# phcavelar/graph-odenet

Measured on AMD Instinct MI355X. Metric: full-graph ODE-GCN forward+backward steps/sec at 64 RK4 evals, higher is better.
Workload: dtype f32; 1 GPU; RMAT scale-20 / 10000000 edges (+self loops, dedup) row-normalised, d=128, ODEGCN3 rk4(3/8) 16 steps = 64 f-evals fwd, adjoint bwd, Adam; one graph per GPU; nodes=1048576, nnz=10758918, nfeat=128, hidden=128, nclass=16, parallelism=dp1 (one graph per rank, 1 gradient all-reduce/step)

## Files before the change

### graph_odenet_amd/csrc/api.hip

```cpp
#include "common.h"

extern "C" int gode_abi_version(void) { return GODE_ABI_VERSION; }

extern "C" const char* gode_error_string(int code) {
    switch (code) {
        case 0: return "success";
        case GODE_E_NULLPTR: return "graphode: required pointer is NULL";
        case GODE_E_SHAPE: return "graphode: invalid shape / leading dimension";
        case GODE_E_ALIGN: return "graphode: operand not 16-byte aligned";
        case GODE_E_RANGE: return "graphode: argument out of range";
        case GODE_E_UNSUPPORTED: return "graphode: unsupported configuration";
        default: break;
    }
    if (code > 0) return hipGetErrorString((hipError_t)code);
    return "graphode: unknown error";
}

#include "options.h"
#include <cstdlib>
#include <cstring>

namespace {
int env_int(const char* name, int dflt) { const char* e = getenv(name); return e ? atoi(e) : dflt; }
int g_gemm_split = -1, g_overlap = -1, g_wgrad_split = -1, g_wgrad_split_small = 0, g_bwd_pc = -1, g_fwd_pc = -1, g_small_fused = -1, g_bwd_wgrad = -1, g_y2_colsum = -1, g_rk_close_once = -1, g_spmm_pipe = -1;
}

int gode_opt_gemm_split() { if (g_gemm_split < 0) { const int v = env_int("GODE_GEMM_SPLIT", 2); g_gemm_split = (v == 1 || v == 2) ? v : 0; } return g_gemm_split; }
int gode_opt_wgrad_split() {
    if (g_wgrad_split < 0) { const int v = env_int("GODE_WGRAD_SPLIT", 8); g_wgrad_split = (v == 6 || v == 8) ? v : 0; }
    return g_wgrad_split;
}
int gode_opt_wgrad_split_small() { return g_wgrad_split_small; }
int gode_opt_bwd_pc() { if (g_bwd_pc < 0) g_bwd_pc = env_int("GODE_BWD_PC", 1) != 0; return g_bwd_pc; }
int gode_opt_fwd_pc() { if (g_fwd_pc < 0) g_fwd_pc = env_int("GODE_FWD_PC", 3) & 3; return g_fwd_pc; }
int gode_opt_small_fused() { if (g_small_fused < 0) g_small_fused = env_int("GODE_SMALL_FUSED", 1) != 0; return g_small_fused; }
int gode_opt_bwd_wgrad() { if (g_bwd_wgrad < 0) g_bwd_wgrad = env_int("GODE_BWD_WGRAD", 1) != 0; return g_bwd_wgrad; }
int gode_opt_y2_colsum() { if (g_y2_colsum < 0) g_y2_colsum = env_int("GODE_Y2_COLSUM", 1) != 0; return g_y2_colsum; }
int gode_opt_rk_close_once() { if (g_rk_close_once < 0) g_rk_close_once = env_int("GODE_RK_CLOSE_ONCE", 1) != 0; return g_rk_close_once; }
int gode_opt_spmm_pipe() { if (g_spmm_pipe < 0) { const int v = env_int("GODE_SPMM_PIPE", 1); g_spmm_pipe = (v < 0 || v > 64) ? 1 : v; } return g_spmm_pipe; }
int gode_opt_overlap() { if (g_overlap < 0) g_overlap = env_int("GODE_OVERLAP", 1) != 0; return g_overlap; }

extern "C" int gode_set_option(const char* name, int value) {
    if (!name) return GODE_E_NULLPTR;
    if (!strcmp(name, "gemm_split")) { if (value < 0 || value > 2) return GODE_E_UNSUPPORTED; g_gemm_split = value; return 0; }
    if (!strcmp(name, "overlap")) { g_overlap = value != 0; return 0; }
    if (!strcmp(name, "wgrad_split_small")) { g_wgrad_split_small = value != 0; return 0; }
    if (!strcmp(name, "bwd_pc")) { g_bwd_pc = value != 0; return 0; }
    if (!strcmp(name, "small_fused")) { g_small_fused = value != 0; return 0; }
    if (!strcmp(name, "bwd_wgrad")) { g_bwd_wgrad = value != 0; return 0; }
    if (!strcmp(name, "y2_colsum")) { g_y2_colsum = value != 0; return 0; }
    if (!strcmp(name, "rk_close_once")) { g_rk_close_once = value != 0; return 0; }
    if (!strcmp(name, "spmm_pipe")) { if (value < 0 || value > 64) return GODE_E_UNSUPPORTED; g_spmm_pipe = value; return 0; }
    if (!strcmp(name, "fwd_pc")) { if (value < 0 || value > 3) return GODE_E_UNSUPPORTED; g_fwd_pc = value; return 0; }
    if (!strcmp(name, "wgrad_split")) { if (value != 0 && value != 6 && value != 8) return GODE_E_UNSUPPORTED; g_wgrad_split = value; return 0; }
    return GODE_E_UNSUPPORTED;
}
extern "C" int gode_get_option(const char* name) {
    if (!name) return GODE_E_NULLPTR;
    if (!strcmp(name, "gemm_split")) return gode_opt_gemm_split();
    if (!strcmp(name, "overlap")) return gode_opt_overlap();
    if (!strcmp(name, "wgrad_split")) return gode_opt_wgrad_split();
    if (!strcmp(name, "wgrad_split_small")) return gode_opt_wgrad_split_small();
    if (!strcmp(name, "bwd_pc")) return gode_opt_bwd_pc();
    if (!strcmp(name, "small_fused")) return gode_opt_small_fused();
    if (!strcmp(name, "bwd_wgrad")) return gode_opt_bwd_wgrad();
    if (!strcmp(name, "y2_colsum")) return gode_opt_y2_colsum();
    if (!strcmp(name, "rk_close_once")) return gode_opt_rk_close_once();
    if (!strcmp(name, "spmm_pipe")) return gode_opt_spmm_pipe();
    if (!strcmp(name, "fwd_pc")) return gode_opt_fwd_pc();
    return GODE_E_UNSUPPORTED;
}
```

### graph_odenet_amd/csrc/dense_pc.h

```cpp
#pragma once
#include "common.h"

int gode_pc_fwd_launch(const LinComb& lc, int64_t n_rows, float eps, const float* gamma, const float* beta,
                       const float* W, int has_time, float t, float* S, float* xout, const float* aux_coef, float* aux,
                       int cg, hipStream_t s);
int gode_pc_bwd_launch(const LinComb& lc, int64_t n_rows, float eps, const float* gamma, const float* W, int has_time,
                       const float* dS, float out_scale, const LinComb& pre, float* dx, float* dgamma_part,
                       float* dbeta_part, int64_t n_part, int cg, hipStream_t s);
int64_t gode_pc_bwd_wgrad_parts(int64_t n_rows);
int gode_pc_bwd_wgrad_launch(const LinComb& lc, int64_t n_rows, float eps, const float* gamma, const float* beta, const float* W,
                             int has_time, const float* dS, float out_scale, const LinComb& pre, float* dx,
                             float* dgamma_part, float* dbeta_part, int64_t n_part, float* dW_part, int cg, hipStream_t s);
```

### graph_odenet_amd/csrc/gemm.hip

```cpp
#include <map>
#include <mutex>
#include <utility>
#include "common.h"
#include "dense_common.h"
#include "dense_pc.h"
#include "options.h"
#include "prof.h"

namespace {

constexpr int kMaxBlocks = 512;
constexpr int64_t kWgradSplitMinRows = 65536;

template <int D, int NTHREADS, bool TRANSPOSE>
__device__ __forceinline__ void fill_w_lds(float* Wl, const float* __restrict__ W, int has_time) {
    constexpr int LDW = D + 4;
    constexpr int N4 = D * D / 4;
    constexpr int IT = (N4 + NTHREADS - 1) / NTHREADS;
    float4 v[IT];
#pragma unroll
    for (int it = 0; it < IT; ++it) {
        const int idx = threadIdx.x + it * NTHREADS;
        v[it] = make_float4(0.f, 0.f, 0.f, 0.f);
        if (idx < N4) v[it] = ld4(W + (int64_t)has_time * D + (int64_t)idx * 4);
// ... 1127 lines not shown
                const float c3 = -c2 * m - bsum * rs * sc;
                dx[(int64_t)row * d_in + c] = out_scale * (rs * (gamma ? gamma[c] : 1.f) * dy[idx] + c2 * xs[idx] + c3) +
                                              (pre.n > 0 ? lc_load1(pre, (int64_t)row * d_in + c) : 0.f);
            }
            if (dgamma_part) {
                const bool first = blk == (int)blockIdx.x;
                for (int c = threadIdx.x; c < d_in; c += 256) {
                    const int gi = c / cg;
                    float sg = 0.f, sb = 0.f;
                    for (int rr = 0; rr < RB; ++rr) {
                        if (blk * RB + rr >= n_rows) break;
                        const float m = stat[(rr * groups + gi) * 2], rs = stat[(rr * groups + gi) * 2 + 1];
                        sg += dy[rr * d_in + c] * (xs[rr * d_in + c] - m) * rs;
                        sb += dy[rr * d_in + c];
                    }
                    float* pg = dgamma_part + (int64_t)blockIdx.x * d_in + c;
                    float* pb = dbeta_part + (int64_t)blockIdx.x * d_in + c;
                    *pg = first ? sg : *pg + sg;
                    *pb = first ? sb : *pb + sb;
                }
            }
        } else {
            for (int idx = threadIdx.x; idx < RB * d_in; idx += 256) {
                const int rr = idx / d_in, c = idx % d_in;
                const int row = blk * RB + rr;
                if (row < n_rows) dx[(int64_t)row * d_in + c] = out_scale * dy[idx] + (pre.n > 0 ? lc_load1(pre, (int64_t)row * d_in + c) : 0.f);
            }
        }
    }
    if (dgamma_part && groups > 0) {
        const int owned = n_blk < (int)gridDim.x ? n_blk : (int)gridDim.x;
        for (int p = owned + blockIdx.x; p < n_part; p += gridDim.x)
            for (int c = threadIdx.x; c < d_in; c += 256) { dgamma_part[(int64_t)p * d_in + c] = 0.f; dbeta_part[(int64_t)p * d_in + c] = 0.f; }
    }
}

__global__ __launch_bounds__(256) void wgrad_generic(LinComb xin, int n_rows, int d_in, int groups, float eps,
                                                     const float* gamma, const float* beta, const float* dS,
                                                     int d_out, int has_time, float* dW_part)
{
    extern __shared__ __attribute__((aligned(16))) float smem[];
    float* xs = smem;
    float* stat = smem + RB * d_in;
    const int n_blk = (n_rows + RB - 1) / RB;
    const int K = d_in + has_time;
    float* out = dW_part + (int64_t)blockIdx.x * K * d_out;
    for (int idx = threadIdx.x; idx < K * d_out; idx += 256) out[idx] = 0.f;
    for (int blk = blockIdx.x; blk < n_blk; blk += gridDim.x) {
        __syncthreads();
        stage_rows_gn(xs, stat, xin, blk * RB, n_rows, d_in, groups, eps, gamma, beta, true);
        const int nr = (n_rows - blk * RB) < RB ? (n_rows - blk * RB) : RB;
        for (int idx = threadIdx.x; idx < K * d_out; idx += 256) {
            const int i = idx / d_out, n = idx % d_out;
            float acc = 0.f;
            for (int rr = 0; rr < nr; ++rr) {
                const float a = (has_time && i == 0) ? 1.0f : xs[rr * d_in + (i - has_time)];
                acc = fmaf(a, dS[(int64_t)(blk * RB + rr) * d_out + n], acc);
            }
            out[idx] += acc;
        }
    }
}

template <typename K>
int set_lds(K kernel, size_t bytes) { return gode_set_lds_once(reinterpret_cast<const void*>(kernel), bytes); }

int fast_cg(int64_t d_in, int64_t d_out, int32_t groups) {
    if (d_in != d_out) return -1;
    if (d_in != 16 && d_in != 32 && d_in != 64 && d_in != 128) return -1;
    if (groups == 0) return 0;
    if (d_in % groups) return -1;
    const int64_t cg = d_in / groups;
    if (cg == 1 || cg == 2 || cg == 4) return (int)cg;
    return -1;
}

int narrow_cg(int64_t d_in, int64_t d_out, int32_t groups) {
    if (d_out != 2) return -1;
    if (d_in != 16 && d_in != 32 && d_in != 64 && d_in != 128) return -1;
    if (groups == 0) return 0;
    if (d_in % groups) return -1;
    const int64_t cg = d_in / groups;
    return (cg == 1 || cg == 2 || cg == 4) ? (int)cg : -1;
}

int64_t fwd_blocks(int64_t n_rows) {
    int64_t b = ((n_rows + 15) / 16 + 3) / 4;
    if (b < 1) b = 1;
    if (b > kMaxBlocks) b = kMaxBlocks;
    return b;
}
int64_t wgrad_blocks(int64_t n_rows) {
    int64_t b = (n_rows + 31) / 32;
    if (b < 1) b = 1;
    if (b > kMaxBlocks) b = kMaxBlocks;
    return b;
}

}

int gode_set_lds_once(const void* fn, size_t bytes) {
    if (bytes <= 64 * 1024) return 0;
    static std::mutex mu;
    static std::map<std::pair<int, const void*>, size_t> done;
    int dev = 0;
    hipError_t e = hipGetDevice(&dev);
    if (e != hipSuccess) return (int)e;
    std::lock_guard<std::mutex> lk(mu);
    auto key = std::make_pair(dev, fn);
    auto it = done.find(key);
    if (it != done.end() && it->second >= bytes) return 0;
    e = hipFuncSetAttribute(fn, hipFuncAttributeMaxDynamicSharedMemorySize, (int)bytes);
    if (e != hipSuccess) return (int)e;
    done[key] = bytes;
    return 0;
}

#define GODE_DISPATCH_NJ_CG(NJV, CGV, MACRO)                                        \
    if (nj == NJV && cg == CGV) { MACRO(NJV, CGV) }

#define GODE_DISPATCH_ALL(MACRO)                                                    \
    GODE_DISPATCH_NJ_CG(1, 0, MACRO) GODE_DISPATCH_NJ_CG(1, 1, MACRO)               \
    GODE_DISPATCH_NJ_CG(2, 0, MACRO) GODE_DISPATCH_NJ_CG(2, 1, MACRO)               \
    GODE_DISPATCH_NJ_CG(4, 0, MACRO) GODE_DISPATCH_NJ_CG(4, 2, MACRO)               \
    GODE_DISPATCH_NJ_CG(8, 0, MACRO) GODE_DISPATCH_NJ_CG(8, 4, MACRO)               \
    GODE_DISPATCH_NJ_CG(1, 2, MACRO) GODE_DISPATCH_NJ_CG(1, 4, MACRO)               \
    GODE_DISPATCH_NJ_CG(2, 2, MACRO) GODE_DISPATCH_NJ_CG(2, 4, MACRO)               \
    GODE_DISPATCH_NJ_CG(4, 1, MACRO) GODE_DISPATCH_NJ_CG(4, 4, MACRO)               \
    GODE_DISPATCH_NJ_CG(8, 1, MACRO) GODE_DISPATCH_NJ_CG(8, 2, MACRO)

static int check_common(const gode_lincomb_t* xin, int64_t n_rows, int64_t d_in, int32_t groups, int64_t d_out) {
    if (n_rows < 0 || d_in <= 0 || d_out <= 0 || groups < 0) return GODE_E_SHAPE;
    if (groups > 0 && d_in % groups) return GODE_E_SHAPE;
    if (n_rows > INT32_MAX || d_in > 2048 || d_out > 65536) return GODE_E_RANGE;
    return check_lincomb(xin, true);
}

extern "C" int gode_gn_time_gemm_f32(const gode_lincomb_t* xin, int64_t n_rows, int64_t d_in, int32_t groups,
                                     float eps, const float* gamma, const float* beta, const float* W,
                                     int64_t d_out, int has_time, float t, float* S, void* stream)
{
    return gode_gn_time_gemm_xout_f32(xin, n_rows, d_in, groups, eps, gamma, beta, W, d_out, has_time, t, S, nullptr,
                                      stream);
}

extern "C" int gode_gn_time_gemm_xout_f32(const gode_lincomb_t* xin, int64_t n_rows, int64_t d_in, int32_t groups,
                                          float eps, const float* gamma, const float* beta, const float* W,
                                          int64_t d_out, int has_time, float t, float* S, float* x_out, void* stream)
{
    return gode_gn_time_gemm_xout_aux_f32(xin, n_rows, d_in, groups, eps, gamma, beta, W, d_out, has_time, t, S, x_out,
                                          nullptr, nullptr, stream);
}

extern "C" int gode_gn_time_gemm_xout_aux_f32(const gode_lincomb_t* xin, int64_t n_rows, int64_t d_in, int32_t groups,
                                              float eps, const float* gamma, const float* beta, const float* W,
                                              int64_t d_out, int has_time, float t, float* S, float* x_out,
                                              const float* aux_coef, float* aux_out, void* stream)
{
    int rc = check_common(xin, n_rows, d_in, groups, d_out); if (rc) return rc;
    if (aux_out && !aux_coef) return GODE_E_NULLPTR;
    if (n_rows == 0) return 0;
    if (!W || !S) return GODE_E_NULLPTR;
    if (x_out && (((uintptr_t)x_out) & 15)) return GODE_E_ALIGN;
    if (aux_out && (((uintptr_t)aux_out) & 15)) return GODE_E_ALIGN;
    if (aux_out) {
        if (aux_out == S || aux_out == x_out) return GODE_E_RANGE;
        for (int j = 0; j < xin->n; ++j) if (aux_out == xin->ptr[j]) return GODE_E_RANGE;
    }
    has_time = has_time ? 1 : 0;
    hipStream_t s = (hipStream_t)stream;
    LinComb lc = make_lincomb(xin);
    AuxCoef ac;
    for (int j = 0; j < GODE_MAX_TERMS; ++j) ac.c[j] = (aux_out && j < lc.n) ? aux_coef[j] : 0.f;
    const int cg = fast_cg(d_in, d_out, groups);
    const bool al = lincomb_aligned16(xin) && !(((uintptr_t)S) & 15) && !(((uintptr_t)W) & 15) &&
                    (!gamma || !(((uintptr_t)gamma) & 15)) && (!beta || !(((uintptr_t)beta) & 15));
    if (aux_out && !(cg >= 0 && al && d_in == 128)) return GODE_E_UNSUPPORTED;
    if (cg >= 0 && al && d_in == 128 && (n_rows >= kWgradSplitMinRows || gode_opt_wgrad_split_small()) &&
        ((lc.n <= 2 && !x_out) ? (gode_opt_fwd_pc() & 1) : (gode_opt_fwd_pc() & 2))) {
        rc = gode_pc_fwd_launch(lc, n_rows, eps, gamma, beta, W, has_time, t, S, x_out, aux_coef, aux_out, cg, s);
        if (rc != GODE_E_UNSUPPORTED) return rc;
        if (aux_out && (cg == 0 || cg == 1 || cg == 2 || cg == 4)) return GODE_E_UNSUPPORTED;
    }
    if (cg >= 0 && al && d_in == 128 && !x_out && (gode_opt_gemm_split() == 1 || (gode_opt_gemm_split() == 2 && lc.n <= 2 && n_rows >= 65536))) {
        if (aux_out) return GODE_E_UNSUPPORTED;
        const size_t lds = (size_t)3 * 128 * (128 + 8) * sizeof(unsigned short) + 3 * 128 * sizeof(float);
        int64_t blocks = ((n_rows + 15) / 16 + 7) / 8; if (blocks < 1) blocks = 1; if (blocks > 256) blocks = 256;
#define GODE_FWDS2(CGV, NXV) { rc = set_lds(gn_gemm_fwd_split_kernel<CGV, NXV>, lds); if (rc) return rc;    \
          const int slot = gode_prof_begin(s, d_in, n_rows, (int64_t)lc.n - 1, GODE_PROF_GEMM_FWD | GODE_PROF_FORM_SPLIT); \
          hipLaunchKernelGGL((gn_gemm_fwd_split_kernel<CGV, NXV>), dim3((unsigned)blocks), dim3(512), lds, s, \
                             lc, (int)n_rows, eps, gamma, beta, W, has_time, t, S);                           \
          gode_prof_end(s, slot);                                                                             \
          GODE_LAUNCH_CHECK(); return 0; }
#define GODE_FWDS(CGV) { if (lc.n == 1) GODE_FWDS2(CGV, 1) else if (lc.n == 2) GODE_FWDS2(CGV, 2) else GODE_FWDS2(CGV, 0) }
        if (cg == 0) GODE_FWDS(0) else if (cg == 1) GODE_FWDS(1) else if (cg == 2) GODE_FWDS(2) else GODE_FWDS(4)
#undef GODE_FWDS
#undef GODE_FWDS2
    }
    if (cg >= 0 && al) {
        const int nj = (int)(d_in / 16);
        const size_t lds = ((size_t)d_in * (d_in + 4) + 3 * d_in) * sizeof(float);
        const int64_t blocks = fwd_blocks(n_rows);
#define GODE_FWD(NJV, CGV)                                                                          \
        { rc = set_lds(gn_gemm_fwd_kernel<NJV, CGV>, lds); if (rc) return rc;                       \
          const int slot = gode_prof_begin(s, d_in, n_rows, (int64_t)lc.n - 1 + (x_out ? 1 : 0), GODE_PROF_GEMM_FWD); \
          hipLaunchKernelGGL((gn_gemm_fwd_kernel<NJV, CGV>), dim3((unsigned)blocks), dim3(256), lds, s, \
                             lc, (int)n_rows, eps, gamma, beta, W, has_time, t, S, x_out,           \
                             (const float*)nullptr, (float*)nullptr, ac, (float*)nullptr);          \
          gode_prof_end(s, slot);                                                                   \
          GODE_LAUNCH_CHECK(); return 0; }
#define GODE_FWDA(NJV, CGV)                                                                         \
        { rc = set_lds(gn_gemm_fwd_kernel<NJV, CGV, true>, lds); if (rc) return rc;                 \
          const int slot = gode_prof_begin(s, d_in, n_rows, (int64_t)lc.n - 1 + (x_out ? 1 : 0) + 1, GODE_PROF_GEMM_FWD); \
          hipLaunchKernelGGL((gn_gemm_fwd_kernel<NJV, CGV, true>), dim3((unsigned)blocks), dim3(256), lds, s, \
                             lc, (int)n_rows, eps, gamma, beta, W, has_time, t, S, x_out,           \
                             (const float*)nullptr, (float*)nullptr, ac, aux_out);                  \
          gode_prof_end(s, slot);                                                                   \
          GODE_LAUNCH_CHECK(); return 0; }
        if (aux_out) {
            GODE_DISPATCH_NJ_CG(8, 0, GODE_FWDA) GODE_DISPATCH_NJ_CG(8, 1, GODE_FWDA)
            GODE_DISPATCH_NJ_CG(8, 2, GODE_FWDA) GODE_DISPATCH_NJ_CG(8, 4, GODE_FWDA)
            return GODE_E_UNSUPPORTED;
        }
        GODE_DISPATCH_ALL(GODE_FWD)
#undef GODE_FWDA
#undef GODE_FWD
    }
    {
        const int cg = narrow_cg(d_in, d_out, groups);
        if (cg >= 0 && al) {
            const int nj = (int)(d_in / 16);
            const int64_t blocks = fwd_blocks(n_rows);
#define GODE_NFWD(NJV, CGV)                                                                                 \
            { hipLaunchKernelGGL((gn_narrow_fwd_kernel<NJV, CGV, 2>), dim3((unsigned)blocks), dim3(256), 0, s, \
                                 lc, (int)n_rows, eps, gamma, beta, W, has_time, t, S, x_out);              \
              GODE_LAUNCH_CHECK(); return 0; }
            GODE_DISPATCH_ALL(GODE_NFWD)
#undef GODE_NFWD
        }
    }
    if (x_out) { rc = gode_lincomb_f32(x_out, xin, n_rows * d_in, stream); if (rc) return rc; }
    const size_t lds = ((size_t)RB * d_in + (size_t)RB * (groups > 0 ? groups : 1) * 2) * sizeof(float);
    rc = set_lds(gn_gemm_fwd_generic, lds); if (rc) return rc;
    int64_t blocks = (n_rows + RB - 1) / RB; if (blocks > 2048) blocks = 2048;
    hipLaunchKernelGGL(gn_gemm_fwd_generic, dim3((unsigned)blocks), dim3(256), lds, s, lc, (int)n_rows, (int)d_in,
                       (int)groups, eps, gamma, beta, W, (int)d_out, has_time, t, S);
    GODE_LAUNCH_CHECK();
    return 0;
}

extern "C" int gode_gn_time_gemm_pair_f32(const gode_lincomb_t* xin, int64_t n_rows, int64_t d, int32_t groups, float eps,
                                          const float* gamma, const float* beta, const float* Wa, const float* Wb,
                                          int has_time, float t, float* Sa, float* Sb, float* x_out, void* stream)
{
    int rc = check_common(xin, n_rows, d, groups, d); if (rc) return rc;
    if (n_rows == 0) return 0;
    if (!Wa || !Wb || !Sa || !Sb) return GODE_E_NULLPTR;
    has_time = has_time ? 1 : 0;
    hipStream_t s = (hipStream_t)stream;
    LinComb lc = make_lincomb(xin);
    const int cg = fast_cg(d, d, groups);
    const bool al = lincomb_aligned16(xin) && !((((uintptr_t)Sa) | ((uintptr_t)Sb) | ((uintptr_t)Wa) | ((uintptr_t)Wb)) & 15) &&
                    (!gamma || !(((uintptr_t)gamma) & 15)) && (!beta || !(((uintptr_t)beta) & 15)) &&
                    (!x_out || !(((uintptr_t)x_out) & 15));
    if (cg >= 0 && al) {
        const int nj = (int)(d / 16);
        const size_t lds = ((size_t)d * (d + 4) + 3 * d) * sizeof(float);
        const int64_t blocks = fwd_blocks(n_rows);
#define GODE_FWDP(NJV, CGV)                                                                         \
        { rc = set_lds(gn_gemm_fwd_kernel<NJV, CGV>, lds); if (rc) return rc;                       \
          hipLaunchKernelGGL((gn_gemm_fwd_kernel<NJV, CGV>), dim3((unsigned)blocks, 2), dim3(256), lds, s, \
                             lc, (int)n_rows, eps, gamma, beta, Wa, has_time, t, Sa, x_out, Wb, Sb, AuxCoef(), (float*)nullptr);  \
          GODE_LAUNCH_CHECK(); return 0; }
        GODE_DISPATCH_ALL(GODE_FWDP)
#undef GODE_FWDP
    }
    rc = gode_gn_time_gemm_xout_f32(xin, n_rows, d, groups, eps, gamma, beta, Wa, d, has_time, t, Sa, x_out, stream);
    if (rc) return rc;
    return gode_gn_time_gemm_f32(xin, n_rows, d, groups, eps, gamma, beta, Wb, d, has_time, t, Sb, stream);
}

extern "C" int64_t gode_gemm_bwd_parts(int64_t n_rows) {
    int64_t a = fwd_blocks(n_rows);
    int64_t b = (n_rows + RB - 1) / RB; if (b > 2048) b = 2048; if (b < 1) b = 1;
    return a > b ? a : b;
}

extern "C" int gode_gn_time_gemm_bwd_f32(const gode_lincomb_t* xin, int64_t n_rows, int64_t d_in, int32_t groups,
                                         float eps, const float* gamma, const float* W, int64_t d_out,
                                         int has_time, const float* dS, float out_scale,
                                         const gode_lincomb_t* pre, float* dx,
                                         float* dgamma_part, float* dbeta_part, void* stream)
{
    int rc = check_common(xin, n_rows, d_in, groups, d_out); if (rc) return rc;
    if (n_rows == 0) return 0;
    if (!W || !dS || !dx) return GODE_E_NULLPTR;
    if ((dgamma_part == nullptr) != (dbeta_part == nullptr)) return GODE_E_NULLPTR;
    if (pre && pre->n > 0) { rc = check_lincomb(pre, true); if (rc) return rc; } else pre = nullptr;
    has_time = has_time ? 1 : 0;
    hipStream_t s = (hipStream_t)stream;
    LinComb lc = make_lincomb(xin);
    LinComb lpre = make_lincomb(pre);
    const int64_t n_part = gode_gemm_bwd_parts(n_rows);
    const int cg = fast_cg(d_in, d_out, groups);
    const bool al = lincomb_aligned16(xin) && lincomb_aligned16(pre) && !(((uintptr_t)dS) & 15) && !(((uintptr_t)dx) & 15) &&
                    (!gamma || !(((uintptr_t)gamma) & 15)) &&
// ... 192 lines not shown
```

### graph_odenet_amd/csrc/gemm_pc.hip

```cpp
#include "common.h"
#include "dense_common.h"
#include "dense_pc.h"
#include "prof.h"

namespace {

constexpr int D = 128;
constexpr int LDK = D + 8;
constexpr int LDX = D + 4;
constexpr int kBlocks = 256;
template <int R> struct Img { static constexpr int PIECE_B = R * LDK * 2, BUF_B = 3 * PIECE_B; };

__device__ __forceinline__ bf16x8 pack8(const unsigned (&u)[8]) {
    const uint2 a = pack_hi16x4(u[0], u[1], u[2], u[3]), b = pack_hi16x4(u[4], u[5], u[6], u[7]);
    typedef unsigned u32x4 __attribute__((ext_vector_type(4)));
    const u32x4 v = {a.x, a.y, b.x, b.y};
    return __builtin_bit_cast(bf16x8, v);
}

template <typename F>
__device__ __forceinline__ void load_weight_pieces(bf16x8 (&A)[4][3], F element) {
    const int l = threadIdx.x & 63, m = l & 15, g = l >> 4;
#pragma unroll
    for (int kb = 0; kb < 4; ++kb) {
        unsigned h[8], md[8], lo[8];
#pragma unroll
        for (int e = 0; e < 8; ++e) split3_trunc(element(m, 32 * kb + 8 * g + e), h[e], md[e], lo[e]);
        A[kb][0] = pack8(h); A[kb][1] = pack8(md); A[kb][2] = pack8(lo);
    }
}

template <int R>
__device__ __forceinline__ void tile_product(const char* img , const bf16x8 (&A)[4][3], f32x4 (&acc)[R / 16]) {
    constexpr int PIECE_B = Img<R>::PIECE_B, NS = (R / 16) * 4;
    bf16x8 b[2][3];
#pragma unroll
    for (int pc = 0; pc < 3; ++pc) b[0][pc] = *reinterpret_cast<const bf16x8*>(img + pc * PIECE_B);
#pragma unroll
    for (int s = 0; s < NS; ++s) {
        const int rt = s >> 2, kb = s & 3;
        if (s + 1 < NS) {
            const int rt2 = (s + 1) >> 2, kb2 = (s + 1) & 3;
#pragma unroll
            for (int pc = 0; pc < 3; ++pc)
                b[(s + 1) & 1][pc] = *reinterpret_cast<const bf16x8*>(img + pc * PIECE_B + rt2 * 16 * LDK * 2 + kb2 * 64);
        }
        const bf16x8 bh = b[s & 1][0], bm = b[s & 1][1], bl = b[s & 1][2];
        f32x4 c = acc[rt];
        c = __builtin_amdgcn_mfma_f32_16x16x32_bf16(A[kb][2], bm, c, 0, 0, 0);
        c = __builtin_amdgcn_mfma_f32_16x16x32_bf16(A[kb][1], bl, c, 0, 0, 0);
        c = __builtin_amdgcn_mfma_f32_16x16x32_bf16(A[kb][2], bh, c, 0, 0, 0);
        c = __builtin_amdgcn_mfma_f32_16x16x32_bf16(A[kb][0], bl, c, 0, 0, 0);
        c = __builtin_amdgcn_mfma_f32_16x16x32_bf16(A[kb][1], bm, c, 0, 0, 0);
        c = __builtin_amdgcn_mfma_f32_16x16x32_bf16(A[kb][1], bh, c, 0, 0, 0);
        c = __builtin_amdgcn_mfma_f32_16x16x32_bf16(A[kb][0], bm, c, 0, 0, 0);
        c = __builtin_amdgcn_mfma_f32_16x16x32_bf16(A[kb][0], bh, c, 0, 0, 0);
        acc[rt] = c;
        __builtin_amdgcn_sched_barrier(0);
    }
}

template <int PIECE_B>
__device__ __forceinline__ void stage_row4(char* dst , const float4 v) {
    unsigned h0, m0, l0, h1, m1, l1, h2, m2, l2, h3, m3, l3;
    split3_trunc(v.x, h0, m0, l0); split3_trunc(v.y, h1, m1, l1); split3_trunc(v.z, h2, m2, l2); split3_trunc(v.w, h3, m3, l3);
    *reinterpret_cast<uint2*>(dst) = pack_hi16x4(h0, h1, h2, h3);
    *reinterpret_cast<uint2*>(dst + PIECE_B) = pack_hi16x4(m0, m1, m2, m3);
    *reinterpret_cast<uint2*>(dst + 2 * PIECE_B) = pack_hi16x4(l0, l1, l2, l3);
}

struct TileWalk {
    int n_tiles, stride, mine;
    __device__ TileWalk(int n_rows, int R) {
        n_tiles = (n_rows + R - 1) / R;
        stride = gridDim.x;
        mine = (int)blockIdx.x < n_tiles ? (n_tiles - 1 - (int)blockIdx.x) / stride + 1 : 0;
    }
    __device__ int tile(int k) const { return blockIdx.x + k * stride; }
    __device__ int clamped(int k) const { return blockIdx.x + (k < mine ? k : (mine > 0 ? mine - 1 : 0)) * stride; }
};

template <int CG, int NX, bool XOUT, int R, bool AUX = false>
__global__ __launch_bounds__(1024, 1) void gn_gemm_fwd_pc_kernel(LinComb xin, int n_rows, float eps,
                                                                const float* __restrict__ gamma,
                                                                const float* __restrict__ beta,
                                                                const float* __restrict__ W, int has_time, float t,
                                                                float* __restrict__ S, float* __restrict__ xout,
                                                                AuxCoef acoef, float* __restrict__ aux)
{
    static_assert(!AUX || NX > 0, "the second combination needs the raw terms");
    constexpr int PIECE_B = Img<R>::PIECE_B, BUF_B = Img<R>::BUF_B;
    constexpr int RPT = R / 8;
    extern __shared__ __attribute__((aligned(16))) float smem[];
    char* lds = reinterpret_cast<char*>(smem);
    const TileWalk tw(n_rows, R);
    if (threadIdx.x >= 512) {
        const int grp = (threadIdx.x - 512) >> 8, pt = (threadIdx.x - 512) & 255;
        const int trow = pt >> 5, tcol = 4 * (pt & 31);
        const float4 gmv = gamma ? ld4(gamma + tcol) : make_float4(1.f, 1.f, 1.f, 1.f);
        const float4 btv = beta ? ld4(beta + tcol) : make_float4(0.f, 0.f, 0.f, 0.f);
        constexpr int NXR = NX > 0 ? NX : 1;
        float4 xr[NXR][RPT];
        auto prefetch = [&](int k) {
            const int tile = tw.clamped(k);
#pragma unroll
            for (int p = 0; p < RPT; ++p) {
                const int row = tile * R + RPT * trow + p;
                const int64_t off = (int64_t)(row < n_rows ? row : n_rows - 1) * D + tcol;
                if (NX > 0) {
#pragma unroll
                    for (int j = 0; j < NXR; ++j) xr[j][p] = ld4(xin.ptr[j] + off);
                } else {
                    xr[0][p] = lc_load4(xin, off);
                }
            }
        };
        auto stage = [&](int k) {
            char* img = lds + (k & 1) * BUF_B + (RPT * trow) * LDK * 2 + tcol * 2;
            const int tile = tw.tile(k);
#pragma unroll
            for (int p = 0; p < RPT; ++p) {
                const int row = tile * R + RPT * trow + p;
                float4 x = xr[0][p];
                if (NX > 0) {
                    x = make_float4(0.f, 0.f, 0.f, 0.f);
#pragma unroll
                    for (int j = 0; j < NXR; ++j) {
                        const float c = xin.coef[j];
                        x.x = fmaf(c, xr[j][p].x, x.x); x.y = fmaf(c, xr[j][p].y, x.y);
                        x.z = fmaf(c, xr[j][p].z, x.z); x.w = fmaf(c, xr[j][p].w, x.w);
                    }
                }
                if (XOUT && row < n_rows) *reinterpret_cast<float4*>(xout + (int64_t)row * D + tcol) = x;
                if (AUX) {
                    float4 a = make_float4(0.f, 0.f, 0.f, 0.f);
#pragma unroll
                    for (int j = 0; j < NXR; ++j) {
                        const float c = acoef.c[j];
                        a.x = fmaf(c, xr[j][p].x, a.x); a.y = fmaf(c, xr[j][p].y, a.y);
                        a.z = fmaf(c, xr[j][p].z, a.z); a.w = fmaf(c, xr[j][p].w, a.w);
                    }
                    if (row < n_rows) *reinterpret_cast<float4*>(aux + (int64_t)row * D + tcol) = a;
                }
                float4 xn = gn_forward_v<CG>(x, eps, gmv, btv);
                if (row >= n_rows) xn = make_float4(0.f, 0.f, 0.f, 0.f);
                stage_row4<PIECE_B>(img + p * LDK * 2, xn);
            }
        };
        prefetch(grp);
        if (grp == 0 && tw.mine > 0) { stage(0); prefetch(2); }
        lds_barrier();
        for (int k = 0; k < tw.mine; ++k) {
            if (((k + 1) & 1) == grp && k + 1 < tw.mine) { stage(k + 1); prefetch(k + 3); }
            lds_barrier();
        }
        return;
    }
    const int wave = threadIdx.x >> 6, l = threadIdx.x & 63, r = l & 15, g = l >> 4;
    const int n0 = 16 * wave;
    bf16x8 A[4][3];
    load_weight_pieces(A, [&](int m, int k) { return W[(int64_t)(k + has_time) * D + n0 + m]; });
    f32x4 t0 = {0.f, 0.f, 0.f, 0.f};
    if (has_time) { const float4 w0 = ld4(W + n0 + 4 * g); t0 = (f32x4){t * w0.x, t * w0.y, t * w0.z, t * w0.w}; }
    const int rd_off = r * LDK * 2 + g * 16;
    lds_barrier();
    for (int k = 0; k < tw.mine; ++k) {
        f32x4 acc[R / 16];
#pragma unroll
        for (int rt = 0; rt < R / 16; ++rt) acc[rt] = t0;
        tile_product<R>(lds + (k & 1) * BUF_B + rd_off, A, acc);
        const int row0 = tw.tile(k) * R + r;
#pragma unroll
        for (int rt = 0; rt < R / 16; ++rt) {
            const int row = row0 + 16 * rt;
            if (row < n_rows)
                *reinterpret_cast<float4*>(S + (int64_t)row * D + n0 + 4 * g) = make_float4(acc[rt][0], acc[rt][1], acc[rt][2], acc[rt][3]);
        }
        lds_barrier();
    }
}

template <int CG, int NX, bool XLDS>
__global__ __launch_bounds__(1024, 1) void gn_gemm_bwd_pc_kernel(LinComb xin, int n_rows, float eps,
                                                                const float* __restrict__ gamma,
                                                                const float* __restrict__ W, int has_time,
                                                                const float* __restrict__ dS, float out_scale,
                                                                LinComb pre, float* __restrict__ dx,
                                                                float* __restrict__ dgamma_part,
                                                                float* __restrict__ dbeta_part, int n_part)
{
    constexpr int R = 32, PIECE_B = Img<R>::PIECE_B;
    constexpr int XT_B = (CG != 0 && XLDS) ? R * LDX * 4 : 0;
    constexpr int BUF_B = Img<R>::BUF_B + XT_B;
    extern __shared__ __attribute__((aligned(16))) float smem[];
    char* lds = reinterpret_cast<char*>(smem);
    const TileWalk tw(n_rows, R);
    if (threadIdx.x >= 512) {
        const int grp = (threadIdx.x - 512) >> 8, pt = (threadIdx.x - 512) & 255;
        const int trow = pt >> 5, tcol = 4 * (pt & 31);
        constexpr int NXR = NX > 0 ? NX : 1;
        float4 gr[4], xr[NXR][4];
        auto prefetch = [&](int k) {
            const int tile = tw.clamped(k);
#pragma unroll
            for (int p = 0; p < 4; ++p) {
                const int row = tile * R + 4 * trow + p;
                const int64_t off = (int64_t)(row < n_rows ? row : n_rows - 1) * D + tcol;
                gr[p] = ld4(dS + off);
                if (CG != 0 && XLDS) {
                    if (NX > 0) {
#pragma unroll
                        for (int j = 0; j < NXR; ++j) xr[j][p] = ld4(xin.ptr[j] + off);
                    } else {
                        xr[0][p] = lc_load4(xin, off);
                    }
                }
            }
        };
        auto stage = [&](int k) {
            char* buf = lds + (k & 1) * BUF_B;
            char* img = buf + (4 * trow) * LDK * 2 + tcol * 2;
            const int tile = tw.tile(k);
#pragma unroll
            for (int p = 0; p < 4; ++p) {
                float4 v = gr[p];
                if (tile * R + 4 * trow + p >= n_rows) v = make_float4(0.f, 0.f, 0.f, 0.f);
                stage_row4<PIECE_B>(img + p * LDK * 2, v);
                if (CG != 0 && XLDS) {
                    float4 x = xr[0][p];
                    if (NX > 0) {
                        x = make_float4(0.f, 0.f, 0.f, 0.f);
#pragma unroll
                        for (int j = 0; j < NXR; ++j) {
                            const float c = xin.coef[j];
                            x.x = fmaf(c, xr[j][p].x, x.x); x.y = fmaf(c, xr[j][p].y, x.y);
                            x.z = fmaf(c, xr[j][p].z, x.z); x.w = fmaf(c, xr[j][p].w, x.w);
                        }
                    }
                    *reinterpret_cast<float4*>(buf + Img<R>::BUF_B + ((4 * trow + p) * LDX + tcol) * 4) = x;
                }
            }
        };
        prefetch(grp);
        if (grp == 0 && tw.mine > 0) { stage(0); prefetch(2); }
        lds_barrier();
        for (int k = 0; k < tw.mine; ++k) {
            if (((k + 1) & 1) == grp && k + 1 < tw.mine) { stage(k + 1); prefetch(k + 3); }
            lds_barrier();
        }
        if (CG != 0 && dgamma_part)
            for (int p = gridDim.x + blockIdx.x; p < n_part; p += gridDim.x)
                for (int c = threadIdx.x - 512; c < D; c += 512) { dgamma_part[(int64_t)p * D + c] = 0.f; dbeta_part[(int64_t)p * D + c] = 0.f; }
        return;
    }
    const int wave = threadIdx.x >> 6, l = threadIdx.x & 63, r = l & 15, g = l >> 4;
    const int i0 = 16 * wave, c0 = i0 + 4 * g;
    bf16x8 A[4][3];
    load_weight_pieces(A, [&](int m, int k) { return W[(int64_t)(i0 + m + has_time) * D + k]; });
    const float4 gm = (CG != 0 && gamma) ? ld4(gamma + c0) : make_float4(1.f, 1.f, 1.f, 1.f);
    float4 dgs = make_float4(0.f, 0.f, 0.f, 0.f), dbs = make_float4(0.f, 0.f, 0.f, 0.f);
    const int rd_off = r * LDK * 2 + g * 16;
    const int xt_off = Img<R>::BUF_B + (r * LDX + c0) * 4;
    lds_barrier();
    for (int k = 0; k < tw.mine; ++k) {
        const char* buf = lds + (k & 1) * BUF_B;
        const int row0 = tw.tile(k) * R + r;
        constexpr int NXC = NX > 0 ? NX : 1;
        float4 xd[2][NXC];
        if (CG != 0 && !XLDS) {
#pragma unroll
            for (int rt = 0; rt < 2; ++rt) {
                const int row = row0 + 16 * rt;
                const int64_t off = (int64_t)(row < n_rows ? row : n_rows - 1) * D + c0;
                if (NX > 0) {
#pragma unroll
                    for (int j = 0; j < NXC; ++j) xd[rt][j] = ld4(xin.ptr[j] + off);
                } else {
                    xd[rt][0] = lc_load4(xin, off);
                }
            }
        }
        f32x4 acc[2] = {{0.f, 0.f, 0.f, 0.f}, {0.f, 0.f, 0.f, 0.f}};
        tile_product<R>(buf + rd_off, A, acc);
#pragma unroll
        for (int rt = 0; rt < 2; ++rt) {
            const int row = row0 + 16 * rt;
            const bool valid = row < n_rows;
            const float4 dy = make_float4(acc[rt][0], acc[rt][1], acc[rt][2], acc[rt][3]);
            float4 out = dy;
            if (CG != 0) {
                float4 x;
                if (XLDS) {
                    x = *reinterpret_cast<const float4*>(buf + xt_off + rt * 16 * LDX * 4);
                } else {
                    x = xd[rt][0];
                    if (NX > 0) {
                        x = make_float4(0.f, 0.f, 0.f, 0.f);
#pragma unroll
                        for (int j = 0; j < NXC; ++j) {
                            const float c = xin.coef[j];
                            x.x = fmaf(c, xd[rt][j].x, x.x); x.y = fmaf(c, xd[rt][j].y, x.y);
                            x.z = fmaf(c, xd[rt][j].z, x.z); x.w = fmaf(c, xd[rt][j].w, x.w);
                        }
                    }
                }
                float4 mean, rstd;
                gn_stats<CG>(x, eps, mean, rstd);
                const float4 xh = make_float4((x.x - mean.x) * rstd.x, (x.y - mean.y) * rstd.y,
                                              (x.z - mean.z) * rstd.z, (x.w - mean.w) * rstd.w);
                const float4 dh = make_float4(dy.x * gm.x, dy.y * gm.y, dy.z * gm.z, dy.w * gm.w);
                if (valid) {
                    dgs.x += dy.x * xh.x; dgs.y += dy.y * xh.y; dgs.z += dy.z * xh.z; dgs.w += dy.w * xh.w;
                    dbs.x += dy.x; dbs.y += dy.y; dbs.z += dy.z; dbs.w += dy.w;
                }
                const float m1 = ((dh.x + dh.y) + (dh.z + dh.w)) * 0.25f;
                const float m2 = ((dh.x * xh.x + dh.y * xh.y) + (dh.z * xh.z + dh.w * xh.w)) * 0.25f;
                const float rs = rstd.x;
                out = make_float4(rs * (dh.x - m1 - xh.x * m2), rs * (dh.y - m1 - xh.y * m2),
                                  rs * (dh.z - m1 - xh.z * m2), rs * (dh.w - m1 - xh.w * m2));
            }
            if (valid) {
                float4 o = make_float4(out_scale * out.x, out_scale * out.y, out_scale * out.z, out_scale * out.w);
                if (pre.n > 0) {
                    const float4 pv = lc_load4(pre, (int64_t)row * D + c0);
                    o.x += pv.x; o.y += pv.y; o.z += pv.z; o.w += pv.w;
                }
                *reinterpret_cast<float4*>(dx + (int64_t)row * D + c0) = o;
            }
        }
// ... 100 lines not shown
            stage(qb, k + 1);
            prefetch(qb, k + 3);
            lds_barrier();
            if (++k >= tw.mine) break;
            stage(qa, k + 1);
            prefetch(qa, k + 3);
            lds_barrier();
            ++k;
        }
        if (has_time) {
            float* red = smem;
            *reinterpret_cast<float4*>(red + trow * D + tcol) = csum;
        }
        __syncthreads();
        if (has_time && pt < D) {
            float sacc = 0.f;
            for (int p = 0; p < 8; ++p) sacc += smem[p * D + pt];
            out[pt] = sacc;
        }
        if (CG != 0 && dgamma_part)
            for (int p = gridDim.x + blockIdx.x; p < n_part; p += gridDim.x)
                for (int c = pt; c < D; c += 256) { dgamma_part[(int64_t)p * D + c] = 0.f; dbeta_part[(int64_t)p * D + c] = 0.f; }
        return;
    }
    const int wave = threadIdx.x >> 6, l = threadIdx.x & 63, r = l & 15, g = l >> 4;
    const int i0 = 16 * wave, c0 = i0 + 4 * g;
    bf16x8 A[4][3];
    load_weight_pieces(A, [&](int m, int k) { return W[(int64_t)(i0 + m + has_time) * D + k]; });
    const float4 gm = (CG != 0 && gamma) ? ld4(gamma + c0) : make_float4(1.f, 1.f, 1.f, 1.f);
    float4 dgs = make_float4(0.f, 0.f, 0.f, 0.f), dbs = make_float4(0.f, 0.f, 0.f, 0.f);
    const int rd_off = r * LDK * 2 + g * 16;
    const int xt_off = 2 * IMG_B + (r * LDX + c0) * 4;
    const int a0 = 4 * (wave >> 2), b0 = 2 * (wave & 3);
    const int tr_off = (8 * g + (r >> 2)) * LDK * 2 + 4 * (r & 3) * 2;
    f32x4 wacc[4][2];
#pragma unroll
    for (int a = 0; a < 4; ++a)
#pragma unroll
        for (int b = 0; b < 2; ++b) wacc[a][b] = (f32x4){0.f, 0.f, 0.f, 0.f};
    lds_barrier();
    for (int k = 0; k < tw.mine; ++k) {
        const char* buf = lds + (k & 1) * BUF_B;
        const int row0 = tw.tile(k) * R + r;
        f32x4 acc[2] = {{0.f, 0.f, 0.f, 0.f}, {0.f, 0.f, 0.f, 0.f}};
        tile_product<R>(buf + rd_off, A, acc);
#pragma unroll
        for (int rt = 0; rt < 2; ++rt) {
            const int row = row0 + 16 * rt;
            const bool valid = row < n_rows;
            const float4 dy = make_float4(acc[rt][0], acc[rt][1], acc[rt][2], acc[rt][3]);
            float4 o4 = dy;
            if (CG != 0) {
                const float4 x = *reinterpret_cast<const float4*>(buf + xt_off + rt * 16 * LDX * 4);
                float4 mean, rstd;
                gn_stats<CG>(x, eps, mean, rstd);
                const float4 xh = make_float4((x.x - mean.x) * rstd.x, (x.y - mean.y) * rstd.y,
                                              (x.z - mean.z) * rstd.z, (x.w - mean.w) * rstd.w);
                const float4 dh = make_float4(dy.x * gm.x, dy.y * gm.y, dy.z * gm.z, dy.w * gm.w);
                if (valid) {
                    dgs.x += dy.x * xh.x; dgs.y += dy.y * xh.y; dgs.z += dy.z * xh.z; dgs.w += dy.w * xh.w;
                    dbs.x += dy.x; dbs.y += dy.y; dbs.z += dy.z; dbs.w += dy.w;
                }
                const float m1 = ((dh.x + dh.y) + (dh.z + dh.w)) * 0.25f;
                const float m2 = ((dh.x * xh.x + dh.y * xh.y) + (dh.z * xh.z + dh.w * xh.w)) * 0.25f;
                const float rs = rstd.x;
                o4 = make_float4(rs * (dh.x - m1 - xh.x * m2), rs * (dh.y - m1 - xh.y * m2),
                                 rs * (dh.z - m1 - xh.z * m2), rs * (dh.w - m1 - xh.w * m2));
            }
            if (valid) {
                float4 o = make_float4(out_scale * o4.x, out_scale * o4.y, out_scale * o4.z, out_scale * o4.w);
                if (pre.n > 0) {
                    const float4 pv = lc_load4(pre, (int64_t)row * D + c0);
                    o.x += pv.x; o.y += pv.y; o.z += pv.z; o.w += pv.w;
                }
                *reinterpret_cast<float4*>(dx + (int64_t)row * D + c0) = o;
            }
        }
        const char* Gp = buf + tr_off;
        const char* Xp = buf + IMG_B + tr_off;
        bf16x8 Bf[2][3];
#pragma unroll
        for (int b = 0; b < 2; ++b)
#pragma unroll
            for (int pc = 0; pc < 3; ++pc) Bf[b][pc] = tr_frag(Gp + pc * PIECE_B, 16 * (b0 + b) * 2);
#pragma unroll
        for (int a = 0; a < 4; ++a) {
            bf16x8 Af[3];
#pragma unroll
            for (int pc = 0; pc < 3; ++pc) Af[pc] = tr_frag(Xp + pc * PIECE_B, 16 * (a0 + a) * 2);
#pragma unroll
            for (int b = 0; b < 2; ++b) {
                f32x4 c = wacc[a][b];
                c = __builtin_amdgcn_mfma_f32_16x16x32_bf16(Af[2], Bf[b][1], c, 0, 0, 0);
                c = __builtin_amdgcn_mfma_f32_16x16x32_bf16(Af[1], Bf[b][2], c, 0, 0, 0);
                c = __builtin_amdgcn_mfma_f32_16x16x32_bf16(Af[2], Bf[b][0], c, 0, 0, 0);
                c = __builtin_amdgcn_mfma_f32_16x16x32_bf16(Af[0], Bf[b][2], c, 0, 0, 0);
                c = __builtin_amdgcn_mfma_f32_16x16x32_bf16(Af[1], Bf[b][1], c, 0, 0, 0);
                c = __builtin_amdgcn_mfma_f32_16x16x32_bf16(Af[1], Bf[b][0], c, 0, 0, 0);
                c = __builtin_amdgcn_mfma_f32_16x16x32_bf16(Af[0], Bf[b][1], c, 0, 0, 0);
                c = __builtin_amdgcn_mfma_f32_16x16x32_bf16(Af[0], Bf[b][0], c, 0, 0, 0);
                wacc[a][b] = c;
            }
        }
        lds_barrier();
    }
#pragma unroll
    for (int a = 0; a < 4; ++a)
#pragma unroll
        for (int b = 0; b < 2; ++b)
#pragma unroll
            for (int q = 0; q < 4; ++q) {
                const int i = 16 * (a0 + a) + 4 * g + q;
                out[(int64_t)(i + has_time) * D + 16 * (b0 + b) + r] = wacc[a][b][q];
            }
    if (CG != 0 && dgamma_part) {
#pragma unroll
        for (int o = 1; o < 16; o <<= 1) {
            dgs.x += __shfl_xor(dgs.x, o, 64); dgs.y += __shfl_xor(dgs.y, o, 64); dgs.z += __shfl_xor(dgs.z, o, 64); dgs.w += __shfl_xor(dgs.w, o, 64);
            dbs.x += __shfl_xor(dbs.x, o, 64); dbs.y += __shfl_xor(dbs.y, o, 64); dbs.z += __shfl_xor(dbs.z, o, 64); dbs.w += __shfl_xor(dbs.w, o, 64);
        }
        if (r == 0) {
            *reinterpret_cast<float4*>(dgamma_part + (int64_t)blockIdx.x * D + c0) = dgs;
            *reinterpret_cast<float4*>(dbeta_part + (int64_t)blockIdx.x * D + c0) = dbs;
        }
    }
    __syncthreads();
}

int64_t pc_blocks(int64_t n_rows, int R) {
    int64_t b = (n_rows + R - 1) / R;
    if (b < 1) b = 1;
    if (b > kBlocks) b = kBlocks;
    return b;
}

template <typename K>
int set_lds_pc(K kernel, size_t bytes) { return gode_set_lds_once(reinterpret_cast<const void*>(kernel), bytes); }

}

int gode_pc_fwd_launch(const LinComb& lc, int64_t n_rows, float eps, const float* gamma, const float* beta,
                       const float* W, int has_time, float t, float* S, float* xout, const float* aux_coef, float* aux,
                       int cg, hipStream_t s)
{
    int rc = 0;
    AuxCoef ac;
    for (int j = 0; j < GODE_MAX_TERMS; ++j) ac.c[j] = (aux && j < lc.n) ? aux_coef[j] : 0.f;
#define GODE_FPC5(CGV, NXV, XO, RV, AX)                                                                           \
    { const size_t lds = 2 * (size_t)Img<RV>::BUF_B;                                                               \
      const int64_t blocks = pc_blocks(n_rows, RV);                                                                \
      rc = set_lds_pc(gn_gemm_fwd_pc_kernel<CGV, NXV, XO, RV, AX>, lds); if (rc) return rc;                        \
      const int slot = gode_prof_begin(s, D, n_rows, (int64_t)lc.n - 1 + (XO ? 1 : 0) + (AX ? 1 : 0), GODE_PROF_GEMM_FWD | GODE_PROF_FORM_PC); \
      hipLaunchKernelGGL((gn_gemm_fwd_pc_kernel<CGV, NXV, XO, RV, AX>), dim3((unsigned)blocks), dim3(1024), lds, s, \
                         lc, (int)n_rows, eps, gamma, beta, W, has_time, t, S, xout, ac, aux);                    \
      gode_prof_end(s, slot);                                                                                      \
      GODE_LAUNCH_CHECK(); return 0; }
#define GODE_FPC2(CGV, NXV, RV) { if (xout) GODE_FPC5(CGV, NXV, true, RV, false) else GODE_FPC5(CGV, NXV, false, RV, false) }
#define GODE_FPC(CGV) { switch (lc.n) { case 1: GODE_FPC2(CGV, 1, 32) case 2: GODE_FPC2(CGV, 2, 32) case 3: GODE_FPC2(CGV, 3, 32) \
                                        case 4: GODE_FPC2(CGV, 4, 32) default: GODE_FPC2(CGV, 0, 32) } }
#define GODE_FPCA(CGV) { if (xout) GODE_FPC5(CGV, 4, true, 32, true) else GODE_FPC5(CGV, 4, false, 32, true) }
    if (aux) {
        if (lc.n != 4) return GODE_E_UNSUPPORTED;
        if (cg == 0) GODE_FPCA(0) else if (cg == 1) GODE_FPCA(1) else if (cg == 2) GODE_FPCA(2) else if (cg == 4) GODE_FPCA(4)
        return GODE_E_UNSUPPORTED;
    }
    if (cg == 0) GODE_FPC(0) else if (cg == 1) GODE_FPC(1) else if (cg == 2) GODE_FPC(2) else if (cg == 4) GODE_FPC(4)
#undef GODE_FPCA
#undef GODE_FPC
#undef GODE_FPC2
#undef GODE_FPC5
    return GODE_E_UNSUPPORTED;
}

int gode_pc_bwd_launch(const LinComb& lc, int64_t n_rows, float eps, const float* gamma, const float* W, int has_time,
                       const float* dS, float out_scale, const LinComb& pre, float* dx, float* dgamma_part,
                       float* dbeta_part, int64_t n_part, int cg, hipStream_t s)
{
    const int64_t blocks = pc_blocks(n_rows, 32);
    int rc = 0;
#define GODE_BPC3(CGV, NXV, XL)                                                                                   \
    { const size_t lds = 2 * ((size_t)Img<32>::BUF_B + ((CGV != 0 && XL) ? 32 * LDX * 4 : 0));                     \
      rc = set_lds_pc(gn_gemm_bwd_pc_kernel<CGV, NXV, XL>, lds); if (rc) return rc;                                \
      const int slot = gode_prof_begin(s, D, n_rows, (int64_t)lc.n - 1 + pre.n, GODE_PROF_GEMM_BWD | GODE_PROF_FORM_PC); \
      hipLaunchKernelGGL((gn_gemm_bwd_pc_kernel<CGV, NXV, XL>), dim3((unsigned)blocks), dim3(1024), lds, s,        \
                         lc, (int)n_rows, eps, gamma, W, has_time, dS, out_scale, pre, dx, dgamma_part, dbeta_part, \
                         (int)n_part);                                                                             \
      gode_prof_end(s, slot);                                                                                      \
      GODE_LAUNCH_CHECK(); return 0; }
#define GODE_BPC(CGV) { if (lc.n == 1) GODE_BPC3(CGV, 1, false) else if (lc.n == 2) GODE_BPC3(CGV, 2, true) else GODE_BPC3(CGV, 0, true) }
    if (cg == 0) GODE_BPC3(0, 1, false) else if (cg == 4) GODE_BPC(4)
#undef GODE_BPC
#undef GODE_BPC3
    return GODE_E_UNSUPPORTED;
}

int64_t gode_pc_bwd_wgrad_parts(int64_t n_rows) { return pc_blocks(n_rows, 32); }

int gode_pc_bwd_wgrad_launch(const LinComb& lc, int64_t n_rows, float eps, const float* gamma, const float* beta, const float* W,
                             int has_time, const float* dS, float out_scale, const LinComb& pre, float* dx,
                             float* dgamma_part, float* dbeta_part, int64_t n_part, float* dW_part, int cg, hipStream_t s)
{
    const int64_t blocks = pc_blocks(n_rows, 32);
    int rc = 0;
#define GODE_BW(CGV, NXV)                                                                                          \
    { const size_t lds = 2 * ((size_t)2 * 3 * Img<32>::PIECE_B + (CGV != 0 ? 32 * LDX * 4 : 0));                     \
      rc = set_lds_pc(gn_gemm_bwd_wgrad_pc_kernel<CGV, NXV>, lds); if (rc) return rc;                               \
      const int slot = gode_prof_begin(s, D, n_rows, (int64_t)lc.n - 1 + pre.n, GODE_PROF_BWD_WGRAD | GODE_PROF_FORM_PC); \
      hipLaunchKernelGGL((gn_gemm_bwd_wgrad_pc_kernel<CGV, NXV>), dim3((unsigned)blocks), dim3(768), lds, s,         \
                         lc, (int)n_rows, eps, gamma, beta, W, has_time, dS, out_scale, pre, dx, dgamma_part,       \
                         dbeta_part, (int)n_part, dW_part);                                                        \
      gode_prof_end(s, slot);                                                                                       \
      GODE_LAUNCH_CHECK(); return 0; }
#define GODE_BWN(CGV) { if (lc.n == 1) GODE_BW(CGV, 1) else if (lc.n == 2) GODE_BW(CGV, 2) else GODE_BW(CGV, 0) }
    if (cg == 0) GODE_BWN(0) else if (cg == 4) GODE_BWN(4)
#undef GODE_BWN
#undef GODE_BW
    return GODE_E_UNSUPPORTED;
}
```

### graph_odenet_amd/csrc/ode_driver.hip

```cpp
#include <map>
#include <mutex>
#include <utility>
#include "rk_driver.h"
#include "options.h"

namespace {

int spmm(const gode_graph_t& g, const float* X, float* Y, int64_t d, const gode_spmm_epilogue_t* ep, void* s) {
    return gode_spmm_csr_f32(g.rowptr, g.col, g.val, g.items, g.n_items, g.long_rows, g.n_long, g.partial,
                             X, d, Y, d, g.n_rows, d, ep, s);
}
gode_spmm_epilogue_t relu_bias_epilogue(const gode_gcn_odefunc_t* f) {
    gode_spmm_epilogue_t ep = {};
    ep.bias = f->b; ep.relu = 1; ep.alpha = 1.f;
    return ep;
}

__global__ void theta_fixup_kernel(float* ktheta, const float* W, float t, int d, int64_t off_at) {
    __shared__ float sm[4];
    float s = 0.f;
    for (int c = threadIdx.x; c < d; c += blockDim.x) s += ktheta[c] * W[c];
    s = wave_sum(s);
    if ((threadIdx.x & 63) == 0) sm[threadIdx.x >> 6] = s;
    __syncthreads();
    if (threadIdx.x == 0) ktheta[off_at] = sm[0] + sm[1] + sm[2] + sm[3];
    __syncthreads();
    for (int c = threadIdx.x; c < d; c += blockDim.x) ktheta[c] *= t;
}

int close_bias(const gode_gcn_odefunc_t* f, const gode_rk4_workspace_t* ws, float* kt, const float* src, int64_t rows,
               void* stream) {
    return gode_colsum_f32(kt + (f->d + 1) * f->d, src, rows, f->d, 1.f, 0, ws->colsum_scratch, stream);
}
int close_weight(const gode_gcn_odefunc_t* f, const gode_rk4_workspace_t* ws, float* kt, int64_t parts, float ts,
                 void* stream) {
    const int64_t d = f->d;
    GODE_TRY(gode_reduce_parts_f32(kt, ws->wpart, parts, (d + 1) * d, 1.f, 0, stream));
    hipLaunchKernelGGL(theta_fixup_kernel, dim3(1), dim3(256), 0, (hipStream_t)stream, kt, f->W, ts, (int)d,
                       gode_gcn_ode_theta_len(d) - 1);
    GODE_LAUNCH_CHECK();
    return 0;
}
int close_affine(const gode_gcn_odefunc_t* f, const gode_rk4_workspace_t* ws, float* kt, void* stream) {
    const int64_t d = f->d;
    float* kg = kt + (d + 1) * d + d;
    if (f->groups <= 0) return gode_zero_f32(kg, 2 * d, stream);
    return gode_reduce_parts2_f32(kg, ws->gpart, kg + d, ws->bpart, gode_gemm_bwd_parts(f->n), d, 1.f, 0, stream);
}

int stage_finish_merged(const gode_gcn_odefunc_t* f, const gode_rk4_workspace_t* ws, float* kt, float ts, void* stream) {
    const int64_t n = f->n, d = f->d, nW = (d + 1) * d, P = gode_gcn_ode_theta_len(d);
    int64_t cparts = 0;
    GODE_TRY(gode_colsum_parts_f32(ws->dZ, n, d, (float*)ws->colsum_scratch, &cparts, stream));
    const int64_t gp = gode_gemm_bwd_parts(n);
    gode_reduce_seg_t sg[4] = {};
    sg[0] = {kt, ws->wpart, gode_wgrad_parts(n), nW, 0, 1, nW, f->W, d};
    sg[1] = {kt + nW, (const float*)ws->colsum_scratch, cparts, d, 0, 1, d, nullptr, 0};
    sg[2] = {kt + nW + d, ws->gpart, gp, d, 0, 1, d, nullptr, 0};
    sg[3] = {kt + nW + 2 * d, ws->bpart, gp, d, 0, 1, d, nullptr, 0};
    GODE_TRY(gode_reduce_segments_f32(sg, f->groups > 0 ? 4 : 2, ts, kt + (P - 1), stream));
    if (f->groups <= 0) GODE_TRY(gode_zero_f32(kt + nW + d, 2 * d, stream));
    return 0;
}

bool fused_small(const gode_gcn_odefunc_t* f) {
    return gode_opt_small_fused() && gode_gcn_small_supported(f->n, f->d, f->groups);
}

bool close_once_route(const gode_gcn_odefunc_t* f) {
    return gode_opt_rk_close_once() && !fused_small(f) && f->n > kMergedFinishMaxRows && f->d == 128;
}

int gf_last_stage(const gode_gcn_odefunc_t* f, const gode_lincomb_t& xin, const gode_lincomb_t& pre, float t, float* S,
                  float* x_out, float* p_out, bool* formed, void* stream) {
    *formed = false;
    bool distinct = p_out != S && p_out != x_out;
    for (int j = 0; j < xin.n; ++j) distinct = distinct && p_out != xin.ptr[j];
    if (distinct && xin.n == pre.n) {
        const int rc = gode_gn_time_gemm_xout_aux_f32(&xin, f->n, f->d, f->groups, f->eps, f->gamma, f->beta, f->W, f->d, 1, t, S,
                                                      x_out, pre.coef, p_out, stream);
        if (rc != GODE_E_UNSUPPORTED) { *formed = rc == 0; return rc; }
    }
    return gode_gn_time_gemm_xout_f32(&xin, f->n, f->d, f->groups, f->eps, f->gamma, f->beta, f->W, f->d, 1, t, S, x_out, stream);
}

struct StepClose { gode_lincomb_t pre; float alpha; bool once; };

int feval_large(const gode_gcn_odefunc_t* f, const gode_lincomb_t& xin, float t, float* S, float* out,
                const StepClose* close, float* k_save, void* stream) {
    const int64_t d = f->d;
    bool p_formed = false;
    if (close && close->once) {
        GODE_TRY(gf_last_stage(f, xin, close->pre, t, S, nullptr, out, &p_formed, stream));
    } else {
        GODE_TRY(gode_gn_time_gemm_f32(&xin, f->n, d, f->groups, f->eps, f->gamma, f->beta, f->W, d, 1, t, S, stream));
    }
    gode_spmm_epilogue_t ep = relu_bias_epilogue(f);
    if (close) { ep.pre = p_formed ? one_term(out) : close->pre; ep.alpha = close->alpha; }
    if (!k_save) return spmm(f->A, S, out, d, &ep, stream);
    const gode_graph_t& g = f->A;
    return gode_spmm_csr_save_f32(g.rowptr, g.col, g.val, g.items, g.n_items, g.long_rows, g.n_long, g.partial,
                                  S, d, out, d, g.n_rows, d, &ep, k_save, stream);
}

int rk4_forward_step(const gode_gcn_odefunc_t* f, const gode_rk4_workspace_t* ws, const float* y, float* const* k,
                     float* ynext, bool keep_k4, double t, double h, bool fused, bool close_once, void* stream) {
    for (int s = 0; s < 4; ++s) {
        const gode_lincomb_t xin = stage_terms(y, k, s, h);
        const float ts = (float)(t + C38[s] * h);
        if (s < 3) {
            if (fused) GODE_TRY(gode_gcn_feval_small_f32(f, &xin, ts, 1.f, nullptr, nullptr, nullptr, k[s], stream));
            else GODE_TRY(feval_large(f, xin, ts, ws->S, k[s], nullptr, nullptr, stream));
            continue;
        }
        const StepClose close = {combine_terms(y, k, h), (float)(h * B38[3]), close_once};
        if (!fused) GODE_TRY(feval_large(f, xin, ts, ws->S, ynext, &close, keep_k4 ? k[3] : nullptr, stream));
        else if (keep_k4) GODE_TRY(gode_gcn_feval_small_save_f32(f, &xin, ts, close.alpha, &close.pre, ynext, k[3], stream));
        else GODE_TRY(gode_gcn_feval_small_f32(f, &xin, ts, close.alpha, &close.pre, nullptr, nullptr, ynext, stream));
    }
    return 0;
}

}

extern "C" int64_t gode_gcn_ode_theta_len(int64_t d) { return (d + 1) * d + 3 * d + 1; }

extern "C" int gode_gcn_ode_rk4_forward(const gode_gcn_odefunc_t* f, float* y, float** result,
                                        const gode_rk4_workspace_t* ws, float t0, float t1, int32_t n_steps,
                                        void* stream)
{
    if (!f || !y || !ws || !result) return GODE_E_NULLPTR;
    if (n_steps <= 0 || f->n <= 0 || f->d <= 0) return GODE_E_SHAPE;
    if (!ws->S || !ws->ky[0] || !ws->ky[1] || !ws->ky[2] || !ws->ky[3]) return GODE_E_NULLPTR;
    const double h = ((double)t1 - (double)t0) / n_steps;
    float* cur = y;
    float* k[4] = {ws->ky[0], ws->ky[1], ws->ky[2], ws->ky[3]};
    const bool fused = fused_small(f);
    const bool close_once = close_once_route(f);
    for (int i = 0; i < n_steps; ++i) {
        GODE_TRY(rk4_forward_step(f, ws, cur, k, k[3], false, (double)t0 + i * h, h, fused, close_once, stream));
        float* tmp = cur; cur = k[3]; k[3] = tmp;
    }
    *result = cur;
    return 0;
}

namespace {

struct Overlap {
    hipStream_t side = nullptr;
    hipEvent_t sp = nullptr, gf = nullptr, spt = nullptr, wg = nullptr;
    bool ok = false;
};
Overlap* overlap_ctx(hipStream_t caller) {
    static std::mutex mu;
    static std::map<std::pair<int, hipStream_t>, Overlap*> ctxs;
    int dev = 0;
    if (hipGetDevice(&dev) != hipSuccess) return nullptr;
    std::lock_guard<std::mutex> lk(mu);
    auto key = std::make_pair(dev, caller);
    auto it = ctxs.find(key);
    if (it != ctxs.end()) return it->second;
    Overlap* c = new Overlap();
    if (hipStreamCreateWithFlags(&c->side, hipStreamNonBlocking) == hipSuccess) {
        bool ok = true;
        for (hipEvent_t* ev : {&c->sp, &c->gf, &c->spt, &c->wg})
            ok = ok && hipEventCreateWithFlags(ev, hipEventDisableTiming) == hipSuccess;
        c->ok = ok;
    }
    ctxs[key] = c;
    return c;
}

int rk4_adjoint_small(const gode_gcn_odefunc_t* f, const gode_rk4_workspace_t* ws, float* y, float* a, float* theta,
                      float** y_result, float** a_result, float t0, double h, int32_t n_steps, void* stream) {
    float* ycur = y; float* acur = a;
    float* ky[4] = {ws->ky[0], ws->ky[1], ws->ky[2], ws->ky[3]};
    float* ka[4] = {ws->ka[0], ws->ka[1], ws->ka[2], ws->ka[3]};
    const int64_t slot = gode_gcn_small_parts(f->n) * gode_gcn_small_part_len(f->d);
    const float hb3 = (float)(h * B38[3]);
    for (int i = 0; i < n_steps; ++i) {
        float stage_t[4];
        const gode_lincomb_t ypre = combine_terms(ycur, ky, h), apre = combine_terms(acur, ka, h);
        for (int s = 0; s < 4; ++s) {
            stage_t[s] = (float)((double)t0 + i * h + C38[s] * h);
            const gode_lincomb_t yin = stage_terms(ycur, ky, s, h);
            const gode_lincomb_t cot = negated(stage_terms(acur, ka, s, h));
            GODE_TRY(gode_gcn_feval_small_f32(f, &yin, stage_t[s], s == 3 ? hb3 : 1.f, s == 3 ? &ypre : nullptr,
                                              &cot, ws->dZ, ky[s], stream));
            GODE_TRY(gode_gcn_vjp_small_f32(f, &yin, ws->dZ, s == 3 ? hb3 : 1.f, s == 3 ? &apre : nullptr,
                                            ka[s], ws->small_part + s * slot, stream));
        }
        const float wb[4] = {(float)(h * B38[0]), (float)(h * B38[1]), (float)(h * B38[2]), hb3};
        GODE_TRY(gode_gcn_small_finish4_f32(f, ws->small_part, theta, wb, stage_t, stream));
        float* tmp = ycur; ycur = ky[3]; ky[3] = tmp;
        tmp = acur; acur = ka[3]; ka[3] = tmp;
    }
    *y_result = ycur;
    *a_result = acur;
    return 0;
}

}

extern "C" int gode_gcn_ode_rk4_adjoint(const gode_gcn_odefunc_t* f, float* y, float* a, float* theta,
                                        float** y_result, float** a_result,
                                        const gode_rk4_workspace_t* ws, float t0, float t1, int32_t n_steps,
                                        void* stream)
{
    if (!f || !y || !a || !theta || !ws || !y_result || !a_result) return GODE_E_NULLPTR;
    if (n_steps <= 0 || f->n <= 0 || f->d <= 0) return GODE_E_SHAPE;
    for (int s = 0; s < 4; ++s) if (!ws->ky[s] || !ws->ka[s] || !ws->ktheta[s]) return GODE_E_NULLPTR;
    if (!ws->S || !ws->dZ || !ws->dS || !ws->wpart || !ws->colsum_scratch) return GODE_E_NULLPTR;
    if (f->groups > 0 && (!ws->gpart || !ws->bpart)) return GODE_E_NULLPTR;
    const int64_t n = f->n, d = f->d;
    const double h = ((double)t1 - (double)t0) / n_steps;
    if (fused_small(f) && ws->small_part != nullptr)
        return rk4_adjoint_small(f, ws, y, a, theta, y_result, a_result, t0, h, n_steps, stream);
    hipStream_t hs = (hipStream_t)stream;
    const bool small = f->n <= kMergedFinishMaxRows;
    Overlap* ov = (!small && ws->S2 != nullptr && gode_opt_overlap()) ? overlap_ctx(hs) : nullptr;
    const bool two = ov != nullptr && ov->ok;
    void* side = two ? (void*)ov->side : stream;
    float* Sbuf[2] = {ws->S, two ? ws->S2 : ws->S};
    float* ycur = y; float* acur = a;
    float* ky[4] = {ws->ky[0], ws->ky[1], ws->ky[2], ws->ky[3]};
    float* ka[4] = {ws->ka[0], ws->ka[1], ws->ka[2], ws->ka[3]};
    const int64_t wparts = gode_wgrad_parts(n);
    const int total = 4 * n_steps;
    const bool bw = !small && gode_bwd_wgrad_supported(n, d, d, f->groups) && gode_bwd_wgrad_parts(n) <= wparts;
    const int64_t y2rows = (bw && ws->y2_colsum && gode_opt_y2_colsum())
        ? gode_spmm_y2_colsum_rows(f->A.items ? f->A.n_items : f->A.n_rows, f->A.items ? f->A.n_long : 0, d) : 0;

    const bool mat = ws->X[0] != nullptr && ws->X[1] != nullptr;
    auto x_out_of = [&](int g) -> float* { return (mat && (g % 4) >= 2) ? ws->X[g & 1] : nullptr; };
    auto stage_time = [&](int g) { return (float)((double)t0 + (g / 4) * h + C38[g % 4] * h); };

    const bool close_once = bw && close_once_route(f);
    bool py_formed = false;
    auto gf = [&](int g, void* st) -> int {
        const gode_lincomb_t yin = stage_terms(ycur, ky, g % 4, h);
        if (g % 4 == 3 && close_once)
            return gf_last_stage(f, yin, combine_terms(ycur, ky, h), stage_time(g), Sbuf[g & 1], x_out_of(g), ky[3], &py_formed, st);
        return gode_gn_time_gemm_xout_f32(&yin, n, d, f->groups, f->eps, f->gamma, f->beta, f->W, d, 1, stage_time(g),
                                          Sbuf[g & 1], x_out_of(g), st);
    };
    GODE_TRY(gf(0, stream));
    bool wg_pending = false;
    for (int g = 0; g < total; ++g) {
        const int s = g % 4;
        const float ts = stage_time(g);
        const gode_lincomb_t yin = x_out_of(g) ? one_term(x_out_of(g)) : stage_terms(ycur, ky, s, h);
        const gode_lincomb_t ain = stage_terms(acur, ka, s, h);
        gode_spmm_epilogue_t ep = relu_bias_epilogue(f);
        ep.cot = negated(ain);
        ep.Y2 = ws->dZ;
        if (y2rows > 0) ep.Y2_colsum = ws->y2_colsum;
        gode_lincomb_t apre; apre.n = 0;
        if (s == 3) {
            ep.pre = py_formed ? one_term(ky[3]) : combine_terms(ycur, ky, h);
            ep.alpha = (float)(h * B38[3]);
            apre = combine_terms(acur, ka, h);
            if (close_once && ain.n == apre.n) {
                ep.cot_out = ka[3];
                for (int j = 0; j < apre.n; ++j) ep.cot_out_coef[j] = apre.coef[j];
                apre = one_term(ka[3]);
            }
            py_formed = false;
        }
        if (two && g > 0) GODE_HIP(hipStreamWaitEvent(hs, ov->gf, 0));
        GODE_TRY(spmm(f->A, Sbuf[g & 1], ky[s], d, &ep, stream));
        if (s == 3) { float* tmp = ycur; ycur = ky[3]; ky[3] = tmp; }
        if (two && wg_pending) GODE_HIP(hipStreamWaitEvent(hs, ov->wg, 0));
        GODE_TRY(spmm(f->AT, ws->dZ, ws->dS, d, nullptr, stream));
        if (two) {
            GODE_HIP(hipEventRecord(ov->spt, hs));
            GODE_HIP(hipStreamWaitEvent(ov->side, ov->spt, 0));
        }
        float* kt = ws->ktheta[s];
        const float out_scale = s == 3 ? (float)(h * B38[3]) : 1.f;
        float* gpart = f->groups > 0 ? ws->gpart : nullptr;
        float* bpart = f->groups > 0 ? ws->bpart : nullptr;
        if (bw) {
            if (two) GODE_HIP(hipStreamWaitEvent(ov->side, ov->spt, 0));
            GODE_TRY(close_bias(f, ws, kt, y2rows > 0 ? ws->y2_colsum : ws->dZ, y2rows > 0 ? y2rows : n, side));
            GODE_TRY(gode_gn_time_gemm_bwd_wgrad_f32(&yin, n, d, f->groups, f->eps, f->gamma, f->beta, f->W, d, 1, ws->dS,
                                                     out_scale, s == 3 ? &apre : nullptr, ka[s], gpart, bpart, ws->wpart, stream));
            if (two) {
                GODE_HIP(hipEventRecord(ov->sp, hs));
                GODE_HIP(hipStreamWaitEvent(ov->side, ov->sp, 0));
            }
            GODE_TRY(close_weight(f, ws, kt, gode_bwd_wgrad_parts(n), ts, side));
            GODE_TRY(close_affine(f, ws, kt, side));
            if (two) { GODE_HIP(hipEventRecord(ov->wg, ov->side)); wg_pending = true; }
            if (g + 1 < total) {
                GODE_TRY(gf(g + 1, stream));
                if (two) GODE_HIP(hipEventRecord(ov->gf, hs));
            }
            if (two) { GODE_HIP(hipStreamWaitEvent(hs, ov->wg, 0)); wg_pending = false; }
        } else {
            GODE_TRY(gode_wgrad_f32(&yin, n, d, f->groups, f->eps, f->gamma, f->beta, ws->dS, d, 1, ws->wpart, side));
            if (!small) GODE_TRY(close_weight(f, ws, kt, wparts, ts, side));
            if (two) { GODE_HIP(hipEventRecord(ov->wg, ov->side)); wg_pending = true; }
            if (g + 1 < total) {
                GODE_TRY(gf(g + 1, side));
                if (two) GODE_HIP(hipEventRecord(ov->gf, ov->side));
            }
            GODE_TRY(gode_gn_time_gemm_bwd_f32(&yin, n, d, f->groups, f->eps, f->gamma, f->W, d, 1, ws->dS, out_scale,
                                               s == 3 ? &apre : nullptr, ka[s], gpart, bpart, stream));
            if (small) {
                GODE_TRY(stage_finish_merged(f, ws, kt, ts, stream));
            } else {
                GODE_TRY(close_bias(f, ws, kt, ws->dZ, n, stream));
                GODE_TRY(close_affine(f, ws, kt, stream));
            }
        }
        if (s == 3) {
            if (two) { GODE_HIP(hipStreamWaitEvent(hs, ov->wg, 0)); wg_pending = false; }
            gode_lincomb_t tc = one_term(theta);
            tc.n = 5;
            for (int q = 0; q < 4; ++q) { tc.coef[1 + q] = (float)(h * B38[q]); tc.ptr[1 + q] = ws->ktheta[q]; }
            GODE_TRY(gode_lincomb_f32(theta, &tc, gode_gcn_ode_theta_len(d), stream));
            float* tmp = acur; acur = ka[3]; ka[3] = tmp;
        }
    }
    if (two) {
        GODE_HIP(hipEventRecord(ov->gf, ov->side));
        GODE_HIP(hipStreamWaitEvent(hs, ov->gf, 0));
    }
    *y_result = ycur;
    *a_result = acur;
    return 0;
}

namespace {

int dp_eval_forward(const gode_gcn_odefunc_t* f, const gode_rk4_workspace_t* ws, const gode_lincomb_t* yin, float t,
                    float* k_out, const gode_lincomb_t* next, float* x_next, void* stream) {
    if (fused_small(f)) return gode_gcn_feval_small_next_f32(f, yin, t, 1.f, nullptr, nullptr, nullptr, k_out, next, x_next, stream);
    return feval_large(f, *yin, t, ws->S, k_out, nullptr, nullptr, stream);
}

int dp_eval_adjoint(const gode_gcn_odefunc_t* f, const gode_rk4_workspace_t* ws, gode_lincomb_t yin,
                    const gode_lincomb_t& ain, float t, float* ky, float* ka, float* kth, const gode_lincomb_t* next,
                    float* x_next, int part_slot, void* stream) {
    const int64_t n = f->n, d = f->d;
    if (fused_small(f) && ws->small_part) {
        const gode_lincomb_t cot = negated(ain);
        GODE_TRY(gode_gcn_feval_small_next_f32(f, &yin, t, 1.f, nullptr, &cot, ws->dZ, ky, next, x_next, stream));
        float* part = ws->small_part + (part_slot > 0 ? part_slot : 0) * gode_gcn_small_parts(n) * gode_gcn_small_part_len(d);
        GODE_TRY(gode_gcn_vjp_small_f32(f, &yin, ws->dZ, 1.f, nullptr, ka, part, stream));
        if (part_slot >= 0) return 0;
        return gode_gcn_small_finish_f32(f, part, kth, t, stream);
    }
    float* xo = (yin.n >= 3 && ws->X[0]) ? ws->X[0] : nullptr;
    GODE_TRY(gode_gn_time_gemm_xout_f32(&yin, n, d, f->groups, f->eps, f->gamma, f->beta, f->W, d, 1, t, ws->S, xo, stream));
    if (xo) yin = one_term(xo);
    gode_spmm_epilogue_t ep = relu_bias_epilogue(f);
    ep.cot = negated(ain);
    ep.Y2 = ws->dZ;
    GODE_TRY(spmm(f->A, ws->S, ky, d, &ep, stream));
    GODE_TRY(spmm(f->AT, ws->dZ, ws->dS, d, nullptr, stream));
    GODE_TRY(gode_gn_time_gemm_bwd_f32(&yin, n, d, f->groups, f->eps, f->gamma, f->W, d, 1, ws->dS, 1.f, nullptr, ka,
                                       f->groups > 0 ? ws->gpart : nullptr, f->groups > 0 ? ws->bpart : nullptr, stream));
    GODE_TRY(gode_wgrad_f32(&yin, n, d, f->groups, f->eps, f->gamma, f->beta, ws->dS, d, 1, ws->wpart, stream));
    if (n <= kMergedFinishMaxRows) return stage_finish_merged(f, ws, kth, t, stream);
    GODE_TRY(close_weight(f, ws, kth, gode_wgrad_parts(n), t, stream));
    GODE_TRY(close_bias(f, ws, kth, ws->dZ, n, stream));
    return close_affine(f, ws, kth, stream);
}

}

extern "C" int gode_gcn_ode_dopri5_step_forward(const gode_gcn_odefunc_t* f, const float* y, float* const* k, float* y1,
                                                const gode_rk4_workspace_t* ws, double t, double h, float rtol,
                                                float atol, double* sums, void* err_scratch, void* stream)
{
    if (!f || !y || !k || !y1 || !ws || !sums || !err_scratch) return GODE_E_NULLPTR;
    if (f->n <= 0 || f->d <= 0) return GODE_E_SHAPE;
    for (int s = 0; s < 7; ++s) if (!k[s]) return GODE_E_NULLPTR;
    if (!ws->S) return GODE_E_NULLPTR;
    const int64_t nd = f->n * f->d;
    const bool chain = fused_small(f) && ws->X[0] && ws->X[1];
    for (int s = 1; s < 7; ++s) {
        gode_lincomb_t yin = dp_terms(y, k, DPA[s], s, h, true);
        if (chain && s >= 2) yin = one_term(ws->X[s & 1]);
        gode_lincomb_t nxt; nxt.n = 0;
        if (chain && s < 6) nxt = dp_terms(y, k, DPA[s + 1], s + 1, h, true);
        GODE_TRY(dp_eval_forward(f, ws, &yin, (float)(t + DPC[s] * h), k[s], nxt.n > 0 ? &nxt : nullptr,
                                 nxt.n > 0 ? ws->X[(s + 1) & 1] : nullptr, stream));
    }
    gode_lincomb_t sol = dp_terms(y, k, DPB, 7, h, true);
    GODE_TRY(gode_lincomb_f32(y1, &sol, nd, stream));
    gode_lincomb_t err = dp_terms(nullptr, k, DPE, 7, h, false);
    return gode_rk_errnorm_f32(sums, y, y1, &err, rtol, atol, nd, err_scratch, stream);
}

extern "C" int gode_gcn_ode_dopri5_step_adjoint(const gode_gcn_odefunc_t* f, const float* y, const float* a,
                                                const float* theta, float* const* ky, float* const* ka,
                                                float* const* kth, float* y1, float* a1, float* theta1,
                                                const gode_rk4_workspace_t* ws, double t, double h, float rtol,
                                                float atol, double* sums , void* err_scratch, void* stream)
{
    if (!f || !y || !a || !theta || !ky || !ka || !kth || !y1 || !a1 || !theta1 || !ws || !sums || !err_scratch)
        return GODE_E_NULLPTR;
    if (f->n <= 0 || f->d <= 0) return GODE_E_SHAPE;
    for (int s = 0; s < 7; ++s) if (!ky[s] || !ka[s] || !kth[s]) return GODE_E_NULLPTR;
    if (!ws->S || !ws->dZ || !ws->dS || !ws->wpart || !ws->colsum_scratch) return GODE_E_NULLPTR;
    if (f->groups > 0 && (!ws->gpart || !ws->bpart)) return GODE_E_NULLPTR;
    const int64_t nd = f->n * f->d, P = gode_gcn_ode_theta_len(f->d);
    const bool fused = fused_small(f) && ws->small_part;
    const bool chain = fused && ws->X[0] && ws->X[1];
    for (int s = 1; s < 7; ++s) {
        gode_lincomb_t yin = dp_terms(y, ky, DPA[s], s, h, true);
        if (chain && s >= 2) yin = one_term(ws->X[s & 1]);
        gode_lincomb_t ain = dp_terms(a, ka, DPA[s], s, h, true);
        gode_lincomb_t nxt; nxt.n = 0;
        if (chain && s < 6) nxt = dp_terms(y, ky, DPA[s + 1], s + 1, h, true);
        GODE_TRY(dp_eval_adjoint(f, ws, yin, ain, (float)(t + DPC[s] * h), ky[s], ka[s], kth[s], nxt.n > 0 ? &nxt : nullptr,
                                 nxt.n > 0 ? ws->X[(s + 1) & 1] : nullptr, fused ? s - 1 : -1, stream));
    }
    if (fused) {
        float* kout[6]; float tsv[6];
        for (int s = 1; s < 7; ++s) { kout[s - 1] = kth[s]; tsv[s - 1] = (float)(t + DPC[s] * h); }
        GODE_TRY(gode_gcn_small_finish_multi_f32(f, ws->small_part, 6, kout, tsv, stream));
    }
// ... 228 lines not shown
```

### graph_odenet_amd/csrc/options.h

```cpp
#pragma once
int gode_opt_gemm_split();
int gode_opt_overlap();
int gode_opt_wgrad_split();
int gode_opt_wgrad_split_small();
int gode_opt_bwd_pc();
int gode_opt_fwd_pc();
int gode_opt_small_fused();
int gode_opt_bwd_wgrad();
int gode_opt_y2_colsum();
int gode_opt_rk_close_once();
int gode_opt_spmm_pipe();
```

### graph_odenet_amd/csrc/spmm.hip

```cpp
#include "common.h"
#include "prof.h"
#include "options.h"
#include <algorithm>

namespace {

constexpr int SPMM_PIPE_TILES = 4;
constexpr int SPMM_PIPE_MIN_BLOCKS = 4096;

struct Epilogue {
    const float* bias;
    int relu;
    float alpha;
    LinComb pre;
    LinComb cot;
    float* Y2;
    float* colpart;
    int64_t colpart_row0;
    float* K;
    float* Y3;
    float c3[GODE_MAX_TERMS];
};

template <int LPR, bool OUT3 = false, bool COT = true>
__device__ __forceinline__ float4 epilogue_store4(const Epilogue& ep, float4 z, int row, int lane,
                                                  int64_t d, float* Y, int64_t ldy) {
    if (ep.bias) {
        const float4 b = *reinterpret_cast<const float4*>(ep.bias + lane * 4);
        z.x += b.x; z.y += b.y; z.z += b.z; z.w += b.w;
    }
    float4 y = z;
    if (ep.relu) { y.x = fmaxf(z.x, 0.f); y.y = fmaxf(z.y, 0.f); y.z = fmaxf(z.z, 0.f); y.w = fmaxf(z.w, 0.f); }
    if (ep.K) *reinterpret_cast<float4*>(ep.K + (int64_t)row * d + lane * 4) = y;
    if (ep.pre.n > 0) {
        const float4 p = lc_load4(ep.pre, (int64_t)row * d + lane * 4);
        y.x = fmaf(ep.alpha, y.x, p.x); y.y = fmaf(ep.alpha, y.y, p.y);
        y.z = fmaf(ep.alpha, y.z, p.z); y.w = fmaf(ep.alpha, y.w, p.w);
    } else if (ep.alpha != 1.f) {
        y.x *= ep.alpha; y.y *= ep.alpha; y.z *= ep.alpha; y.w *= ep.alpha;
    }
    *reinterpret_cast<float4*>(Y + (int64_t)row * ldy + lane * 4) = y;
    if (COT && ep.Y2) {
        const int64_t o = (int64_t)row * d + lane * 4;
        float4 g;
        if (OUT3) {
            float4 g3;
            lc_load4_pair(ep.cot, ep.c3, o, g, g3);
            *reinterpret_cast<float4*>(ep.Y3 + o) = g3;
        } else {
            g = lc_load4(ep.cot, o);
        }
        g.x = z.x > 0.f ? g.x : 0.f; g.y = z.y > 0.f ? g.y : 0.f;
        g.z = z.z > 0.f ? g.z : 0.f; g.w = z.w > 0.f ? g.w : 0.f;
        *reinterpret_cast<float4*>(ep.Y2 + o) = g;
        return g;
    }
    return make_float4(0.f, 0.f, 0.f, 0.f);
}

template <int LPR>
__device__ __forceinline__ void block_colsum_store(const float4 g, float* __restrict__ colpart_row) {
    __shared__ float4 cs[256];
    cs[threadIdx.x] = g;
    __syncthreads();
    if (threadIdx.x < LPR) {
        float4 t = cs[threadIdx.x];
#pragma unroll
        for (int r = 1; r < 256 / LPR; ++r) {
            const float4 a = cs[r * LPR + threadIdx.x];
            t.x += a.x; t.y += a.y; t.z += a.z; t.w += a.w;
        }
        *reinterpret_cast<float4*>(colpart_row + 4 * threadIdx.x) = t;
    }
}

template <int LPR, bool OUT3 = false>
__global__ __launch_bounds__(256) void spmm_vec4_kernel(
    const int* __restrict__ rowptr, const int* __restrict__ col, const float* __restrict__ val,
    const int4* __restrict__ items, int n_items, float* __restrict__ partial,
    const float* __restrict__ X, int64_t ldx, float* __restrict__ Y, int64_t ldy, Epilogue ep)
{
    constexpr int U = 4;
    const int64_t tid = (int64_t)blockIdx.x * blockDim.x + threadIdx.x;
    const int gid = (int)(tid / LPR);
    const int lane = threadIdx.x & (LPR - 1);
    const bool active = gid < n_items;
    int row = 0, b = 0, e = 0, slot = -1;
    if (active) {
        if (items) { const int4 it = items[gid]; row = it.x; b = it.y; e = it.z; slot = it.w; }
        else { row = gid; b = rowptr[gid]; e = rowptr[gid + 1]; }
    }
    const int len = e - b;
    float4 acc = make_float4(0.f, 0.f, 0.f, 0.f);
    const float* Xl = X + lane * 4;

    for (int base = 0; __any(base < len); base += LPR) {
        int c = 0; float v = 0.f;
        if (base + lane < len) {
            c = col[b + base + lane];
            v = val ? val[b + base + lane] : 1.f;
        }
        const int cnt = len - base;
        for (int k = 0; k < LPR; k += U) {
            if (!__any(k < cnt)) break;
            int cc[U]; float vv[U]; float4 xv[U];
#pragma unroll
            for (int u = 0; u < U; ++u) {
                cc[u] = __shfl(c, k + u, LPR);
                vv[u] = __shfl(v, k + u, LPR);
            }
#pragma unroll
            for (int u = 0; u < U; ++u) {
                xv[u] = make_float4(0.f, 0.f, 0.f, 0.f);
                if (k + u < cnt && k + u < LPR)
                    xv[u] = *reinterpret_cast<const float4*>(Xl + (int64_t)cc[u] * ldx);
            }
#pragma unroll
            for (int u = 0; u < U; ++u) {
                acc.x = fmaf(vv[u], xv[u].x, acc.x); acc.y = fmaf(vv[u], xv[u].y, acc.y);
                acc.z = fmaf(vv[u], xv[u].z, acc.z); acc.w = fmaf(vv[u], xv[u].w, acc.w);
            }
        }
    }
    if (ep.colpart) {
        float4 g = make_float4(0.f, 0.f, 0.f, 0.f);
        if (active) {
            if (slot < 0) g = epilogue_store4<LPR, OUT3>(ep, acc, row, lane, (int64_t)LPR * 4, Y, ldy);
            else *reinterpret_cast<float4*>(partial + (int64_t)slot * (LPR * 4) + lane * 4) = acc;
        }
        block_colsum_store<LPR>(g, ep.colpart + (int64_t)blockIdx.x * (LPR * 4));
        return;
    }
    if (!active) return;
    if (slot < 0) epilogue_store4<LPR, OUT3>(ep, acc, row, lane, (int64_t)LPR * 4, Y, ldy);
    else *reinterpret_cast<float4*>(partial + (int64_t)slot * (LPR * 4) + lane * 4) = acc;
}

constexpr int SPMM_PIPE_RECS = 1024;
constexpr int spmm_pipe_max_tiles(int lpr) { return std::min(64, SPMM_PIPE_RECS / (256 / lpr)); }

template <bool REC>
__device__ __forceinline__ int4 pipe_load_rec(const int4* __restrict__ items, const int* __restrict__ rowptr, int gid, int n_items) {
    const int g = min(gid, n_items - 1);
    if (REC) return items[g];
    return make_int4(g, rowptr[g], rowptr[g + 1], -1);
}

__device__ __forceinline__ void pipe_load_chunk(const int* __restrict__ col, const float* __restrict__ val,
                                                const int* __restrict__ safe, int b, int len, int lane, int& c, float& v) {
    const int64_t i = (int64_t)b + min(lane, len - 1);
    const int* cp = len > 0 ? col + i : safe;
    const float* vp = (len > 0 && val) ? val + i : reinterpret_cast<const float*>(safe);
    const int cl = *cp;
    const float vl = *vp;
    c = lane < len ? cl : 0;
    v = lane < len ? (val ? vl : 1.f) : 0.f;
}

template <int LPR, bool REC>
__global__ __launch_bounds__(256) __attribute__((amdgpu_waves_per_eu((LPR == 4 || LPR == 64) ? 7 : 8, 8)))
void spmm_vec4_pipe_kernel(
    const int* __restrict__ rowptr, const int* __restrict__ col, const float* __restrict__ val,
    const int4* __restrict__ items, int n_items, float* __restrict__ partial,
    const float* __restrict__ X, int64_t ldx, float* __restrict__ Y, int64_t ldy, Epilogue ep,
    int tiles)
{
    constexpr int U = 4;
    constexpr int GPT = 256 / LPR;
    constexpr int NQ = (spmm_pipe_max_tiles(LPR) * GPT + 255) / 256;
    __shared__ int4 recs[SPMM_PIPE_RECS];
    const int lane = threadIdx.x & (LPR - 1);
    const int grp = threadIdx.x / LPR;
    const float* Xl = X + lane * 4;
    const int t0 = (int)blockIdx.x, step = (int)gridDim.x;
    const int n_here = (tiles - t0 + step - 1) / step;
    {
        const int cnt = n_here * GPT;
        int4 r[NQ]; int gid[NQ];
#pragma unroll
        for (int q = 0; q < NQ; ++q) {
            const int i = min((int)threadIdx.x + 256 * q, cnt - 1);
            gid[q] = (t0 + (i / GPT) * step) * GPT + (i % GPT);
            r[q] = pipe_load_rec<REC>(items, rowptr, gid[q], n_items);
        }
#pragma unroll
        for (int q = 0; q < NQ; ++q) {
            const bool in = gid[q] < n_items;
            if ((int)threadIdx.x + 256 * q < cnt)
                recs[threadIdx.x + 256 * q] = make_int4(r[q].w < 0 ? r[q].x : ~r[q].w, r[q].y, in ? r[q].z - r[q].y : 0, in ? 1 : 0);
        }
    }
    __syncthreads();

    int c; float v;
    pipe_load_chunk(col, val, rowptr, recs[grp].y, recs[grp].z, lane, c, v);
    for (int j = 0; j < n_here; ++j) {
        const int4 nx = recs[min(j + 1, n_here - 1) * GPT + grp];
        int nc; float nv;
        pipe_load_chunk(col, val, rowptr, nx.y, j + 1 < n_here ? nx.z : 0, lane, nc, nv);

        const int4 cur = recs[j * GPT + grp];
        const int dst = cur.x, b = cur.y, len = cur.z;
        float4 acc = make_float4(0.f, 0.f, 0.f, 0.f);
        for (int base = 0; __any(base < len); base += LPR) {
            if (base > 0) {
                c = 0; v = 0.f;
                if (base + lane < len) {
                    c = col[b + base + lane];
                    v = val ? val[b + base + lane] : 1.f;
                }
            }
            const int cnt = len - base;
            for (int k = 0; k < LPR; k += U) {
                if (!__any(k < cnt)) break;
                int cc[U]; float vv[U]; float4 xv[U];
#pragma unroll
                for (int u = 0; u < U; ++u) {
                    cc[u] = __shfl(c, k + u, LPR);
                    vv[u] = __shfl(v, k + u, LPR);
                }
#pragma unroll
                for (int u = 0; u < U; ++u) {
                    xv[u] = make_float4(0.f, 0.f, 0.f, 0.f);
                    if (k + u < cnt && k + u < LPR)
                        xv[u] = *reinterpret_cast<const float4*>(Xl + (int64_t)cc[u] * ldx);
                }
#pragma unroll
                for (int u = 0; u < U; ++u) {
                    acc.x = fmaf(vv[u], xv[u].x, acc.x); acc.y = fmaf(vv[u], xv[u].y, acc.y);
                    acc.z = fmaf(vv[u], xv[u].z, acc.z); acc.w = fmaf(vv[u], xv[u].w, acc.w);
                }
            }
        }
        asm volatile("" : "+v"(nc), "+v"(nv));
        if (cur.w) {
            if (dst >= 0) epilogue_store4<LPR, false, false>(ep, acc, dst, lane, (int64_t)LPR * 4, Y, ldy);
            else *reinterpret_cast<float4*>(partial + (int64_t)(~dst) * (LPR * 4) + lane * 4) = acc;
        }
        c = nc; v = nv;
    }
}

template <int LPR, bool OUT3 = false>
__global__ __launch_bounds__(256) void spmm_vec4_wave_kernel(
    const int* __restrict__ rowptr, const int* __restrict__ col, const float* __restrict__ val,
    const int4* __restrict__ items, int n_items, float* __restrict__ partial,
    const float* __restrict__ X, int64_t ldx, float* __restrict__ Y, int64_t ldy, Epilogue ep)
{
    const int gid = (int)(((int64_t)blockIdx.x * blockDim.x + threadIdx.x) >> 6);
    const int wl = threadIdx.x & 63;
    const int lane = wl & (LPR - 1), sub = wl / LPR;
    if (gid >= n_items) return;
    int row, b, e, slot = -1;
    if (items) { const int4 it = items[gid]; row = it.x; b = it.y; e = it.z; slot = it.w; }
    else { row = gid; b = rowptr[gid]; e = rowptr[gid + 1]; }
    const int len = e - b;
    float4 acc = make_float4(0.f, 0.f, 0.f, 0.f);
    const float* Xl = X + lane * 4;
    for (int base = sub * LPR; base - sub * LPR < len; base += 64) {
        int c = 0; float v = 0.f;
        if (base + lane < len) {
            c = col[b + base + lane];
            v = val ? val[b + base + lane] : 1.f;
        }
        const int cnt = len - base;
        constexpr int U = LPR < 4 ? LPR : 4;
        for (int k = 0; k < LPR; k += U) {
            if (!__any(k < cnt)) break;
            int cc[U]; float vv[U]; float4 xv[U];
#pragma unroll
            for (int u = 0; u < U; ++u) { cc[u] = __shfl(c, k + u, LPR); vv[u] = __shfl(v, k + u, LPR); }
#pragma unroll
            for (int u = 0; u < U; ++u) {
                xv[u] = make_float4(0.f, 0.f, 0.f, 0.f);
                if (k + u < cnt) xv[u] = *reinterpret_cast<const float4*>(Xl + (int64_t)cc[u] * ldx);
            }
#pragma unroll
            for (int u = 0; u < U; ++u) {
                acc.x = fmaf(vv[u], xv[u].x, acc.x); acc.y = fmaf(vv[u], xv[u].y, acc.y);
                acc.z = fmaf(vv[u], xv[u].z, acc.z); acc.w = fmaf(vv[u], xv[u].w, acc.w);
            }
        }
    }
#pragma unroll
    for (int off = LPR; off < 64; off <<= 1) {
        acc.x += __shfl_xor(acc.x, off, 64); acc.y += __shfl_xor(acc.y, off, 64);
        acc.z += __shfl_xor(acc.z, off, 64); acc.w += __shfl_xor(acc.w, off, 64);
    }
    if (sub != 0) return;
    if (slot < 0) epilogue_store4<LPR, OUT3>(ep, acc, row, lane, (int64_t)LPR * 4, Y, ldy);
    else *reinterpret_cast<float4*>(partial + (int64_t)slot * (LPR * 4) + lane * 4) = acc;
}

template <int LPR, bool OUT3 = false>
__global__ __launch_bounds__(256) void spmm_finish_vec4_kernel(
    const int4* __restrict__ long_rows, int n_long, const float* __restrict__ partial,
    float* __restrict__ Y, int64_t ldy, Epilogue ep)
{
    const int64_t tid = (int64_t)blockIdx.x * blockDim.x + threadIdx.x;
    const int gid = (int)(tid / LPR);
    const int lane = threadIdx.x & (LPR - 1);
    const bool active = gid < n_long;
    if (!active && !ep.colpart) return;
    const int4 lr = active ? long_rows[gid] : make_int4(0, 0, 0, 0);
    float4 acc = make_float4(0.f, 0.f, 0.f, 0.f);
    int s = lr.y;
    for (; s + 3 < lr.z; s += 4) {
        const float4 p0 = *reinterpret_cast<const float4*>(partial + (int64_t)s * (LPR * 4) + lane * 4);
        const float4 p1 = *reinterpret_cast<const float4*>(partial + (int64_t)(s + 1) * (LPR * 4) + lane * 4);
        const float4 p2 = *reinterpret_cast<const float4*>(partial + (int64_t)(s + 2) * (LPR * 4) + lane * 4);
        const float4 p3 = *reinterpret_cast<const float4*>(partial + (int64_t)(s + 3) * (LPR * 4) + lane * 4);
        acc.x += p0.x; acc.y += p0.y; acc.z += p0.z; acc.w += p0.w;
        acc.x += p1.x; acc.y += p1.y; acc.z += p1.z; acc.w += p1.w;
        acc.x += p2.x; acc.y += p2.y; acc.z += p2.z; acc.w += p2.w;
        acc.x += p3.x; acc.y += p3.y; acc.z += p3.z; acc.w += p3.w;
    }
    for (; s < lr.z; ++s) {
        const float4 p = *reinterpret_cast<const float4*>(partial + (int64_t)s * (LPR * 4) + lane * 4);
        acc.x += p.x; acc.y += p.y; acc.z += p.z; acc.w += p.w;
    }
    if (ep.colpart) {
        float4 g = make_float4(0.f, 0.f, 0.f, 0.f);
        if (active) g = epilogue_store4<LPR, OUT3>(ep, acc, lr.x, lane, (int64_t)LPR * 4, Y, ldy);
        block_colsum_store<LPR>(g, ep.colpart + (ep.colpart_row0 + blockIdx.x) * (LPR * 4));
        return;
    }
    epilogue_store4<LPR, OUT3>(ep, acc, lr.x, lane, (int64_t)LPR * 4, Y, ldy);
}

__device__ __forceinline__ void epilogue_store1(const Epilogue& ep, float z, int row, int c, int64_t d,
                                                float* Y, int64_t ldy) {
    if (ep.bias) z += ep.bias[c];
    float y = ep.relu ? fmaxf(z, 0.f) : z;
    if (ep.K) ep.K[(int64_t)row * d + c] = y;
    if (ep.pre.n > 0) y = fmaf(ep.alpha, y, lc_load1(ep.pre, (int64_t)row * d + c));
    else y *= ep.alpha;
    Y[(int64_t)row * ldy + c] = y;
    if (ep.Y2) {
        const int64_t o = (int64_t)row * d + c;
        const float g = lc_load1(ep.cot, o);
        ep.Y2[o] = z > 0.f ? g : 0.f;
        if (ep.Y3) {
            float g3 = 0.f;
#pragma unroll
            for (int j = 0; j < GODE_MAX_TERMS; ++j)
                if (j < ep.cot.n) g3 = fmaf(ep.c3[j], ep.cot.ptr[j][o], g3);
            ep.Y3[o] = g3;
        }
    }
}

__global__ __launch_bounds__(256) void spmm_generic_kernel(
    const int* __restrict__ rowptr, const int* __restrict__ col, const float* __restrict__ val,
    const int4* __restrict__ items, int n_items, float* __restrict__ partial,
    const float* __restrict__ X, int64_t ldx, float* __restrict__ Y, int64_t ldy, int d, int G, Epilogue ep)
{
    const int64_t tid = (int64_t)blockIdx.x * blockDim.x + threadIdx.x;
    const int gid = (int)(tid / G);
    const int lane = threadIdx.x & (G - 1);
    if (gid >= n_items) return;
    int row, b, e, slot = -1;
    if (items) { const int4 it = items[gid]; row = it.x; b = it.y; e = it.z; slot = it.w; }
    else { row = gid; b = rowptr[gid]; e = rowptr[gid + 1]; }
    for (int c = lane; c < d; c += G) {
        float acc = 0.f;
        int j = b;
        for (; j + 4 <= e; j += 4) {
            const int c0 = col[j], c1 = col[j + 1], c2 = col[j + 2], c3 = col[j + 3];
            const float x0 = X[(int64_t)c0 * ldx + c], x1 = X[(int64_t)c1 * ldx + c], x2 = X[(int64_t)c2 * ldx + c],
                        x3 = X[(int64_t)c3 * ldx + c];
            float v0 = 1.f, v1 = 1.f, v2 = 1.f, v3 = 1.f;
            if (val) { v0 = val[j]; v1 = val[j + 1]; v2 = val[j + 2]; v3 = val[j + 3]; }
            acc = fmaf(v0, x0, acc); acc = fmaf(v1, x1, acc); acc = fmaf(v2, x2, acc); acc = fmaf(v3, x3, acc);
        }
        for (; j < e; ++j) {
            const float v = val ? val[j] : 1.f;
            acc = fmaf(v, X[(int64_t)col[j] * ldx + c], acc);
        }
        if (slot < 0) epilogue_store1(ep, acc, row, c, d, Y, ldy);
        else partial[(int64_t)slot * d + c] = acc;
    }
}

__global__ __launch_bounds__(256) void spmv_wave_kernel(
    const int* __restrict__ rowptr, const int* __restrict__ col, const float* __restrict__ val,
    const int4* __restrict__ items, int n_items, float* __restrict__ partial,
    const float* __restrict__ X, int64_t ldx, float* __restrict__ Y, int64_t ldy, Epilogue ep)
{
    const int gid = (int)(((int64_t)blockIdx.x * blockDim.x + threadIdx.x) >> 6);
    const int lane = threadIdx.x & 63;
    if (gid >= n_items) return;
    int row, b, e, slot = -1;
    if (items) { const int4 it = items[gid]; row = it.x; b = it.y; e = it.z; slot = it.w; }
    else { row = gid; b = rowptr[gid]; e = rowptr[gid + 1]; }
    float acc = 0.f;
    for (int j = b + lane; j < e; j += 64) acc = fmaf(val ? val[j] : 1.f, X[(int64_t)col[j] * ldx], acc);
    acc = wave_sum(acc);
    if (lane == 0) {
        if (slot < 0) epilogue_store1(ep, acc, row, 0, 1, Y, ldy);
        else partial[slot] = acc;
    }
}

__global__ __launch_bounds__(256) void spmm_finish_generic_kernel(
    const int4* __restrict__ long_rows, int n_long, const float* __restrict__ partial,
    float* __restrict__ Y, int64_t ldy, int d, int G, Epilogue ep)
{
    const int64_t tid = (int64_t)blockIdx.x * blockDim.x + threadIdx.x;
    const int gid = (int)(tid / G);
    const int lane = threadIdx.x & (G - 1);
    if (gid >= n_long) return;
    const int4 lr = long_rows[gid];
    for (int c = lane; c < d; c += G) {
        float acc = 0.f;
        for (int s = lr.y; s < lr.z; ++s) acc += partial[(int64_t)s * d + c];
        epilogue_store1(ep, acc, lr.x, c, d, Y, ldy);
    }
}

template <int LPR, bool OUT3>
int launch_vec4(const int* rowptr, const int* col, const float* val, const int4* items, int n_items,
                const int4* long_rows, int n_long, float* partial, const float* X, int64_t ldx,
                float* Y, int64_t ldy, const Epilogue& ep, hipStream_t s) {
    if (LPR < 64 && n_items > 0 && n_items <= 65536) {
        if (ep.colpart) return GODE_E_UNSUPPORTED;
        const int64_t wb = ((int64_t)n_items * 64 + 255) / 256;
        const int slot = gode_prof_begin(s, (int64_t)LPR * 4, n_items, (int64_t)ep.pre.n + ep.cot.n + (ep.Y2 ? 1 : 0) + (ep.Y3 ? 1 : 0));
        hipLaunchKernelGGL((spmm_vec4_wave_kernel<LPR, OUT3>), dim3((unsigned)wb), dim3(256), 0, s,
                           rowptr, col, val, items, n_items, partial, X, ldx, Y, ldy, ep);
        gode_prof_end(s, slot);
        GODE_LAUNCH_CHECK();
        if (n_long > 0) {
            const int64_t b2 = ((int64_t)n_long * LPR + 255) / 256;
            hipLaunchKernelGGL((spmm_finish_vec4_kernel<LPR, OUT3>), dim3((unsigned)b2), dim3(256), 0, s,
                               long_rows, n_long, partial, Y, ldy, ep);
            GODE_LAUNCH_CHECK();
        }
        return 0;
    }
    const int64_t threads = (int64_t)n_items * LPR;
    const int64_t blocks = (threads + 255) / 256;
    if (blocks > 0) {
        const int slot = gode_prof_begin(s, (int64_t)LPR * 4, n_items, (int64_t)ep.pre.n + ep.cot.n + (ep.Y2 ? 1 : 0) + (ep.Y3 ? 1 : 0));
        const int pipe = gode_opt_spmm_pipe();
        if (pipe != 0 && !ep.Y2) {
            int64_t per = pipe == 1 ? std::max<int64_t>(1, std::min<int64_t>(SPMM_PIPE_TILES, blocks / SPMM_PIPE_MIN_BLOCKS)) : pipe;
            per = std::min<int64_t>(per, spmm_pipe_max_tiles(LPR));
            const int64_t grid = (blocks + per - 1) / per;
            if (items)
                hipLaunchKernelGGL((spmm_vec4_pipe_kernel<LPR, true>), dim3((unsigned)grid), dim3(256), 0, s,
                                   rowptr, col, val, items, n_items, partial, X, ldx, Y, ldy, ep, (int)blocks);
            else
                hipLaunchKernelGGL((spmm_vec4_pipe_kernel<LPR, false>), dim3((unsigned)grid), dim3(256), 0, s,
                                   rowptr, col, val, items, n_items, partial, X, ldx, Y, ldy, ep, (int)blocks);
        } else
        hipLaunchKernelGGL((spmm_vec4_kernel<LPR, OUT3>), dim3((unsigned)blocks), dim3(256), 0, s,
                           rowptr, col, val, items, n_items, partial, X, ldx, Y, ldy, ep);
        gode_prof_end(s, slot);
        GODE_LAUNCH_CHECK();
    }
    if (n_long > 0) {
        const int64_t b2 = ((int64_t)n_long * LPR + 255) / 256;
        Epilogue ep2 = ep;
        ep2.colpart_row0 = blocks;
        hipLaunchKernelGGL((spmm_finish_vec4_kernel<LPR, OUT3>), dim3((unsigned)b2), dim3(256), 0, s,
                           long_rows, n_long, partial, Y, ldy, ep2);
        GODE_LAUNCH_CHECK();
    }
    return 0;
}

}

extern "C" int64_t gode_spmm_y2_colsum_rows(int64_t n_items, int64_t n_long, int64_t d)
{
    if (n_items <= 0 || n_long < 0 || d <= 0 || d % 4) return 0;
    const int64_t lpr = d / 4;
    if (lpr > 64 || (lpr & (lpr - 1))) return 0;
    if (lpr < 64 && n_items <= 65536) return 0;
    return (n_items * lpr + 255) / 256 + (n_long * lpr + 255) / 256;
}

namespace {

int spmm_csr_impl(const int32_t* rowptr, const int32_t* col, const float* val,
                  const int32_t* items, int64_t n_items,
                  const int32_t* long_rows, int64_t n_long, float* partial,
                  const float* X, int64_t ldx, float* Y, int64_t ldy,
                  int64_t n_rows, int64_t d,
                  const gode_spmm_epilogue_t* epi, float* K, void* stream)
{
    if (n_rows < 0 || d <= 0 || ldx < d || ldy < d) return GODE_E_SHAPE;
    if (n_rows == 0) return 0;
    if (!rowptr || !col || !X || !Y) return GODE_E_NULLPTR;
    if (n_rows > INT32_MAX || d > (1 << 20)) return GODE_E_RANGE;
    if (!items) { n_items = n_rows; n_long = 0; }
    if (n_items < 0 || n_items > INT32_MAX || n_long < 0 || n_long > INT32_MAX) return GODE_E_RANGE;
    if (n_long > 0 && (!long_rows || !partial)) return GODE_E_NULLPTR;
    if (n_items * 64 >= ((int64_t)1 << 32)) return GODE_E_RANGE;
    const float* bias = epi ? epi->bias : nullptr;
    float* Y2 = epi ? epi->Y2 : nullptr;
    const gode_lincomb_t* cot = (epi && Y2) ? &epi->cot : nullptr;
    const gode_lincomb_t* pre = (epi && epi->pre.n > 0) ? &epi->pre : nullptr;
    if (Y2) { int rc = check_lincomb(cot, true); if (rc) return rc; }
    if (pre) { int rc = check_lincomb(pre, true); if (rc) return rc; }
    hipStream_t s = (hipStream_t)stream;

    Epilogue ep;
    ep.bias = bias; ep.relu = epi ? epi->relu : 0; ep.alpha = epi ? epi->alpha : 1.f;
    ep.pre = make_lincomb(pre); ep.cot = make_lincomb(cot); ep.Y2 = Y2;
    ep.colpart = (epi && Y2) ? epi->Y2_colsum : nullptr; ep.colpart_row0 = 0;
    ep.K = K;
    ep.Y3 = (epi && Y2) ? epi->cot_out : nullptr;
    for (int j = 0; j < GODE_MAX_TERMS; ++j) ep.c3[j] = (ep.Y3 && j < ep.cot.n) ? epi->cot_out_coef[j] : 0.f;
    if (ep.Y3) {
        if (ep.Y3 == Y || ep.Y3 == Y2 || ep.Y3 == K) return GODE_E_RANGE;
        for (int j = 0; j < ep.cot.n; ++j) if (ep.Y3 == ep.cot.ptr[j]) return GODE_E_RANGE;
    }
    if (ep.colpart && ((((uintptr_t)ep.colpart) & 15) || gode_spmm_y2_colsum_rows(n_items, n_long, d) == 0)) return GODE_E_UNSUPPORTED;

    const bool al = !(((uintptr_t)X) & 15) && !(((uintptr_t)Y) & 15) && (ldx % 4 == 0) && (ldy % 4 == 0) &&
                    (!bias || !(((uintptr_t)bias) & 15)) && (!partial || !(((uintptr_t)partial) & 15)) &&
                    (!Y2 || (!(((uintptr_t)Y2) & 15) && lincomb_aligned16(cot))) && lincomb_aligned16(pre) &&
                    !(((uintptr_t)K) & 15) && !(((uintptr_t)ep.Y3) & 15);
    const int4* it4 = reinterpret_cast<const int4*>(items);
    const int4* lr4 = reinterpret_cast<const int4*>(long_rows);
    if (al && d % 4 == 0) {
        switch (d / 4) {
#define GODE_CASE(L) case L: return ep.Y3 ? launch_vec4<L, true>(rowptr, col, val, it4, (int)n_items, lr4, (int)n_long, partial, X, ldx, Y, ldy, ep, s) \
                                        : launch_vec4<L, false>(rowptr, col, val, it4, (int)n_items, lr4, (int)n_long, partial, X, ldx, Y, ldy, ep, s);
            GODE_CASE(1) GODE_CASE(2) GODE_CASE(4) GODE_CASE(8) GODE_CASE(16) GODE_CASE(32) GODE_CASE(64)
#undef GODE_CASE
            default: break;
        }
    }
    if (ep.colpart) return GODE_E_UNSUPPORTED;
    int G = 1; while (G < d && G < 64) G <<= 1;
    if (d == 1 && it4 != nullptr) {
        const int64_t blocks = ((int64_t)n_items * 64 + 255) / 256;
        const int slot = gode_prof_begin(s, 1, n_items, (int64_t)ep.pre.n + ep.cot.n + (ep.Y2 ? 1 : 0) + (ep.Y3 ? 1 : 0));
        hipLaunchKernelGGL(spmv_wave_kernel, dim3((unsigned)blocks), dim3(256), 0, s,
                           rowptr, col, val, it4, (int)n_items, partial, X, ldx, Y, ldy, ep);
        gode_prof_end(s, slot);
        GODE_LAUNCH_CHECK();
    } else {
        const int64_t blocks = ((int64_t)n_items * G + 255) / 256;
        hipLaunchKernelGGL(spmm_generic_kernel, dim3((unsigned)blocks), dim3(256), 0, s,
                           rowptr, col, val, it4, (int)n_items, partial, X, ldx, Y, ldy, (int)d, G, ep);
        GODE_LAUNCH_CHECK();
    }
    if (n_long > 0) {
        const int64_t b2 = ((int64_t)n_long * G + 255) / 256;
        hipLaunchKernelGGL(spmm_finish_generic_kernel, dim3((unsigned)b2), dim3(256), 0, s,
                           lr4, (int)n_long, partial, Y, ldy, (int)d, G, ep);
        GODE_LAUNCH_CHECK();
    }
    return 0;
}

}

extern "C" int gode_spmm_csr_f32(const int32_t* rowptr, const int32_t* col, const float* val,
                                 const int32_t* items, int64_t n_items,
                                 const int32_t* long_rows, int64_t n_long, float* partial,
                                 const float* X, int64_t ldx, float* Y, int64_t ldy,
                                 int64_t n_rows, int64_t d,
                                 const gode_spmm_epilogue_t* epi, void* stream)
{
    return spmm_csr_impl(rowptr, col, val, items, n_items, long_rows, n_long, partial, X, ldx, Y, ldy, n_rows, d, epi,
                         nullptr, stream);
}

extern "C" int gode_spmm_csr_save_f32(const int32_t* rowptr, const int32_t* col, const float* val,
                                      const int32_t* items, int64_t n_items,
                                      const int32_t* long_rows, int64_t n_long, float* partial,
                                      const float* X, int64_t ldx, float* Y, int64_t ldy,
                                      int64_t n_rows, int64_t d,
                                      const gode_spmm_epilogue_t* epi, float* K, void* stream)
{
    if (n_rows < 0 || d <= 0 || ldx < d || ldy < d) return GODE_E_SHAPE;
    if (n_rows > 0 && !K) return GODE_E_NULLPTR;
    return spmm_csr_impl(rowptr, col, val, items, n_items, long_rows, n_long, partial, X, ldx, Y, ldy, n_rows, d, epi,
                         K, stream);
}
```

### graph_odenet_amd/gcn_ode.py

```python
import ctypes

import torch

from . import _lib, ops
from .graph import as_graph
from .solver import Field


def _graph_struct(g, d):
    gs = _lib.Graph()
    gs.rowptr, gs.col = g.rowptr.data_ptr(), g.col.data_ptr()
    gs.val = g.val.data_ptr() if g.val is not None else None
    gs.items, gs.n_items = (g.items.data_ptr() if g.items is not None else None), g.n_items
    gs.long_rows = g.long_rows.data_ptr() if g.long_rows is not None else None
    gs.n_long = g.n_long
    part = g.partial(d)
    gs.partial = part.data_ptr() if part is not None else None
    gs.n_rows, gs.nnz = g.n_rows, g.nnz
    return gs


class _Shared:

    def __init__(self, graph, d, device):
        n = graph.n_rows
        self.S = torch.empty(n, d, dtype=torch.float32, device=device)
        self.dZ = None
        self.dS = None
        self.n = n
        self.d = d
        self.device = device
        self._ky = self._ka = self._kt = None
        self._parts = None
        self.y2_rows = 0
        if not getattr(graph, "is_partitioned", False) and hasattr(graph, "n_items"):
            self.y2_rows = _lib.load().gode_spmm_y2_colsum_rows(graph.n_items if graph.items is not None else n, graph.n_long, d)
        self._y2_colsum = None
        self._X2 = None

    @property
    def X2(self):
        if self._X2 is None:
            self._X2 = [torch.empty_like(self.S), torch.empty_like(self.S)]
        return self._X2

    def bwd(self):
        if self.dZ is None:
            self.dZ = torch.empty_like(self.S)
            self.dS = torch.empty_like(self.S)
        return self.dZ, self.dS

    def stage_buffers(self, adjoint):
        if self._ky is None:
            self._ky = [torch.empty_like(self.S) for _ in range(4)]
        if adjoint and self._ka is None:
            lib = _lib.load()
            P = lib.gode_gcn_ode_theta_len(self.d)
            self._ka = [torch.empty_like(self.S) for _ in range(4)]
            self._kt = [torch.empty(P, dtype=torch.float32, device=self.device) for _ in range(4)]
            nW = (self.d + 1) * self.d
            self._parts = (torch.empty(lib.gode_wgrad_parts(self.n) * nW, dtype=torch.float32, device=self.device),
                           torch.empty(lib.gode_gemm_bwd_parts(self.n) * self.d, dtype=torch.float32, device=self.device),
                           torch.empty(lib.gode_gemm_bwd_parts(self.n) * self.d, dtype=torch.float32, device=self.device),
                           torch.empty(max(lib.gode_colsum_scratch_bytes(self.n, self.d), 16), dtype=torch.uint8,
                                       device=self.device))
        return self._ky, self._ka, self._kt, self._parts

    def workspace_struct(self, adjoint, groups=0):
        ky, ka, kt, parts = self.stage_buffers(adjoint)
        ws = _lib.Rk4Workspace()
        ws.S = self.S.data_ptr()
        for i in range(4):
            ws.ky[i] = ky[i].data_ptr()
        if not adjoint and _lib.load().gode_gcn_small_supported(self.n, self.d, int(groups)):
            ws.X[0], ws.X[1] = self.X2[0].data_ptr(), self.X2[1].data_ptr()
        if adjoint:
            dZ, dS = self.bwd()
            ws.dZ, ws.dS = dZ.data_ptr(), dS.data_ptr()
            if getattr(self, "S2", None) is None:
                self.S2 = torch.empty_like(self.S)
            ws.S2 = self.S2.data_ptr()
            for i in range(4):
                ws.ka[i] = ka[i].data_ptr()
                ws.ktheta[i] = kt[i].data_ptr()
            ws.wpart, ws.gpart, ws.bpart, ws.colsum_scratch = (p.data_ptr() for p in parts)
            ws.X[0], ws.X[1] = self.X2[0].data_ptr(), self.X2[1].data_ptr()
            sp = self.small_part(groups)
            ws.small_part = sp.data_ptr() if sp is not None else None
            if self.y2_rows > 0:
                if self._y2_colsum is None:
                    self._y2_colsum = torch.empty(self.y2_rows, self.d, dtype=torch.float32, device=self.device)
                ws.y2_colsum = self._y2_colsum.data_ptr()
        return ws

    def cot_colpart(self):
        rows = _lib.load().gode_masked_cot_parts(self.n, self.d)
        if rows <= 0:
            return None
        if getattr(self, "_cot_colpart", None) is None:
            self._cot_colpart = torch.empty(rows, self.d, dtype=torch.float32, device=self.device)
        return self._cot_colpart

    def small_part(self, groups):
        lib = _lib.load()
        if not lib.gode_gcn_small_supported(self.n, self.d, int(groups)):
            return None
        if getattr(self, "_small_part", None) is None:
            self._small_part = torch.empty(7 * lib.gode_gcn_small_parts(self.n) * lib.gode_gcn_small_part_len(self.d),
                                           dtype=torch.float32, device=self.device)
        return self._small_part


def _func_struct(spec):
    fs = _lib.GcnOdeFunc()
    fs.A = _graph_struct(spec.graph, spec.d)
    fs.AT = _graph_struct(spec.graph.transpose(), spec.d)
    fs.n, fs.d, fs.groups, fs.eps = spec.graph.n_rows, spec.d, spec.groups, spec.eps
    fs.W, fs.b = spec.W.data_ptr(), spec.b.data_ptr()
    fs.gamma, fs.beta = spec.gamma.data_ptr(), spec.beta.data_ptr()
    return fs


def _by_ptr(ptr_value, candidates):
    for t in candidates:
        if t.data_ptr() == ptr_value:
            return t
    raise RuntimeError("rk4 driver returned an unknown buffer")


RELABEL_MIN_OPERAND_BYTES = 64 << 20
RELABEL_MIN_NNZ = 1 << 21
RELABEL_MIN_IMBALANCE = 2.0
NODE_ORDERS = ("auto", "given", "degree")


def gather_imbalance(graph, d, inverse=None):
    m = max(8, min(4096, (32 << 10) // (4 * d)))
    col = graph.col.to(torch.int64)
    rp = graph.rowptr.to(torch.int64)
    deg = rp[1:] - rp[:-1]
    rows = torch.arange(graph.n_rows, device=col.device)
    if inverse is not None:
        col, rows = inverse[col], inverse
    h_a = torch.bincount(col % m, minlength=m)
    h_t = torch.zeros(m, dtype=torch.int64, device=col.device).index_add_(0, rows % m, deg)
    h = torch.stack([h_a, h_t]).tolist()
    return max(max(hh) * m / max(sum(hh), 1) for hh in h)


def tuned_graph(graph, d, node_order="auto"):
    if node_order not in NODE_ORDERS:
        raise ValueError("node_order must be one of %s, got %r" % (NODE_ORDERS, node_order))
    cache = graph.__dict__.setdefault("_tuned", {})
    hit = cache.get((d, node_order))
    if hit is not None:
        return hit
    res = (graph, None, None)
    info = {"node_order": node_order, "renumbered": False}
    square = graph.n_rows == graph.n_cols and not getattr(graph, "is_partitioned", False)
    big = graph.n_rows * d * 4 >= RELABEL_MIN_OPERAND_BYTES and graph.nnz >= RELABEL_MIN_NNZ
    if square and node_order != "given" and (node_order == "degree" or big) \
            and not torch.cuda.is_current_stream_capturing():
        order = graph.degree_order()
        inverse = torch.empty_like(order)
        inverse[order] = torch.arange(graph.n_rows, device=graph.device)
        take = node_order == "degree"
        if not take:
            given, hubs = gather_imbalance(graph, d), gather_imbalance(graph, d, inverse)
            info.update(imbalance_given=round(given, 4), imbalance_hubs_first=round(hubs, 4))
            take = given >= RELABEL_MIN_IMBALANCE and hubs <= 0.5 * given
        if take:
            res = (graph.relabel(order), order, inverse)
            info["renumbered"] = True
    graph.__dict__.setdefault("_tuned_info", {})[(d, node_order)] = info
    cache[(d, node_order)] = res
    return res


class GcnOdeSpec:

    def __init__(self, graph, W, b, gamma, beta, groups, eps):
        self.graph, self.W, self.b, self.gamma, self.beta = graph, W, b, gamma, beta
        self.groups, self.eps = int(groups), float(eps)
        self.d = W.shape[1]
        if W.shape[0] != self.d + 1:
            raise ValueError("GcnOdeSpec: weight must be (d+1) x d, got %s" % (tuple(W.shape),))
        if graph.n_rows != graph.n_cols:
            raise ValueError("GcnOdeSpec: adjacency must be square")


def small_fused(spec):
    lib = _lib.load()
    return bool(lib.gode_get_option(b"small_fused") == 1 and not getattr(spec.graph, "is_partitioned", False)
                and lib.gode_gcn_small_supported(spec.graph.n_rows, spec.d, spec.groups))


def _feval_small(spec, t, terms, out, pre=None, alpha=1.0, cot=None, out2=None, next_terms=None, x_next=None):
    lib = _lib.load()
    fs = _func_struct(spec)
    lx = _lib.lincomb(terms)
    lp = _lib.lincomb(pre) if pre is not None else None
    lc = _lib.lincomb(cot) if cot is not None else None
    ln = _lib.lincomb(next_terms) if next_terms is not None else None
    _lib.check(lib.gode_gcn_feval_small_next_f32(ctypes.byref(fs), ctypes.byref(lx), float(t), float(alpha),
                                                 ctypes.byref(lp) if lp is not None else None,
                                                 ctypes.byref(lc) if lc is not None else None,
                                                 _lib.ptr(out2) if cot is not None else None, _lib.ptr(out),
                                                 ctypes.byref(ln) if ln is not None else None,
                                                 _lib.ptr(x_next) if ln is not None else None, _lib.stream_ptr()),
               "gode_gcn_feval_small_next_f32")


def _byref(lc):
    return ctypes.byref(lc) if lc is not None else None


def _feval_small_save(spec, t, terms, out, k, pre=None, alpha=1.0):
    lib = _lib.load()
    fs = _func_struct(spec)
    lx = _lib.lincomb(terms)
    lp = _lib.lincomb(pre) if pre is not None else None
    _lib.check(lib.gode_gcn_feval_small_save_f32(ctypes.byref(fs), ctypes.byref(lx), float(t), float(alpha), _byref(lp),
                                                 _lib.ptr(out), _lib.ptr(k), _lib.stream_ptr()),
               "gode_gcn_feval_small_save_f32")


def _vjp_small(spec, terms, dZ, ka, part, pre=None, out_scale=1.0, fs=None):
    lib = _lib.load()
    fs = _func_struct(spec) if fs is None else fs
    lx = _lib.lincomb(terms)
    lp = _lib.lincomb(pre) if pre is not None else None
    _lib.check(lib.gode_gcn_vjp_small_f32(ctypes.byref(fs), ctypes.byref(lx), _lib.ptr(dZ), float(out_scale), _byref(lp),
                                          _lib.ptr(ka), _lib.ptr(part), _lib.stream_ptr()), "gode_gcn_vjp_small_f32")


def _vjp_small_next(spec, terms, dZ, ka, part, cot_next, k_next, dZ_next, pre=None, out_scale=1.0):
    lib = _lib.load()
    fs = _func_struct(spec)
    lx = _lib.lincomb(terms)
    lp = _lib.lincomb(pre) if pre is not None else None
    ln = _lib.lincomb(cot_next)
    _lib.check(lib.gode_gcn_vjp_small_next_f32(ctypes.byref(fs), ctypes.byref(lx), _lib.ptr(dZ), float(out_scale), _byref(lp),
                                               _lib.ptr(ka), _lib.ptr(part), ctypes.byref(ln), _lib.ptr(k_next),
                                               _lib.ptr(dZ_next), _lib.stream_ptr()), "gode_gcn_vjp_small_next_f32")


def _finish_small(spec, part, ktheta, t, fs=None):
    lib = _lib.load()
    fs = _func_struct(spec) if fs is None else fs
    _lib.check(lib.gode_gcn_small_finish_f32(ctypes.byref(fs), _lib.ptr(part), _lib.ptr(ktheta), float(t),
                                             _lib.stream_ptr()), "gode_gcn_small_finish_f32")


def _finish_small_multi(spec, part, kthetas, ts):
    lib = _lib.load()
    fs = _func_struct(spec)
    n = len(kthetas)
    _lib.check(lib.gode_gcn_small_finish_multi_f32(ctypes.byref(fs), _lib.ptr(part), n,
                                                   (ctypes.c_void_p * n)(*[k.data_ptr() for k in kthetas]),
                                                   (ctypes.c_float * n)(*[float(t) for t in ts]), _lib.stream_ptr()),
               "gode_gcn_small_finish_multi_f32")


def _finish_small4(spec, part, theta, wb, ts):
    lib = _lib.load()
    fs = _func_struct(spec)
    wbh, tsh = (ctypes.c_float * 4)(*[float(v) for v in wb]), (ctypes.c_float * 4)(*[float(v) for v in ts])
    _lib.check(lib.gode_gcn_small_finish4_f32(ctypes.byref(fs), _lib.ptr(part), _lib.ptr(theta), wbh, tsh, _lib.stream_ptr()),
               "gode_gcn_small_finish4_f32")


class _PackedParams:

    def _theta_len(self):
        return (self.s.d + 1) * self.s.d + 3 * self.s.d + 1

    def _packed_state(self, th, y, a):
        d = self.s.d
        nW = (d + 1) * d
        comps = [y, a, th[nW + 3 * d:], th[:nW].view(d + 1, d), th[nW:nW + d], th[nW + d:nW + 2 * d],
                 th[nW + 2 * d:nW + 3 * d]]
        comps[2]._gode_packed = th
        return comps

    def _in_params_order(self, comps):
        m = {"W": comps[3], "b": comps[4], "gamma": comps[5], "beta": comps[6]}
        return [m[k] for k in self.params_order]

    def packed_grads(self, device):
        return torch.zeros(self._theta_len(), dtype=torch.float32, device=device)

    def packed_param_grads(self, theta):
        return self._in_params_order(self._packed_state(theta, None, None))


class GcnOdeField(_PackedParams, Field):
    n_components = 1
    fused = True

    def __init__(self, spec, shared, params_order):
        self.s, self.w = spec, shared
        self.params_order = params_order
        self.token = ("gcn", id(spec.graph))

    def eval(self, t, terms, out):
        s, w = self.s, self.w
        if small_fused(s):
            return _feval_small(s, t, terms[0], out[0])
        ops.gn_time_gemm(terms[0], w.n, s.d, s.groups, s.eps, s.gamma, s.beta, s.W, True, t, out=w.S)
        ops.spmm(s.graph, w.S, bias=s.b, relu=True, out=out[0])

    def rk4_native(self, comps, t0, t1, n_steps):
        lib = _lib.load()
        s, w = self.s, self.w
        ky = w.stage_buffers(False)[0]
        fs, ws = _func_struct(s), w.workspace_struct(False, s.groups)
        res = ctypes.c_void_p()
        _lib.check(lib.gode_gcn_ode_rk4_forward(ctypes.byref(fs), _lib.ptr(comps[0]), ctypes.byref(res), ctypes.byref(ws),
                                                float(t0), float(t1), int(n_steps), _lib.stream_ptr()),
                   "gode_gcn_ode_rk4_forward")
        out = _by_ptr(res.value, [comps[0]] + ky)
        if out is not comps[0]:
            comps[0].copy_(out)
        return 4 * n_steps

    def rk4_forward_save(self, y0, y_end, save, t0, t1, n_steps, i0, i1):
# ... 267 lines not shown
```

### graph_odenet_amd/graph.py

```python
import weakref

import torch

DEFAULT_SPLIT = None


def auto_split(nnz):
    return 256 if nnz >= (1 << 20) else 1024


class CSRGraph:

    def __init__(self, rowptr, col, val, n_rows, n_cols, split=DEFAULT_SPLIT, records=True):
        self.rowptr = rowptr.to(torch.int32).contiguous()
        self.col = col.to(torch.int32).contiguous()
        self.val = None if val is None else val.to(torch.float32).contiguous()
        self.n_rows = int(n_rows)
        self.n_cols = int(n_cols)
        self.nnz = int(self.col.numel())
        self.device = self.col.device
        self.split = int(split) if split is not None else auto_split(self.nnz)
        if records:
            self._build_items()
        else:
            self.items, self.n_items, self.long_rows, self.n_long, self.n_slots = None, self.n_rows, None, 0, 0
        self._partial = {}
        self._T = None

    def _build_items(self):
        dev = self.device
        n = self.n_rows
        rp = self.rowptr.to(torch.int64)
        deg = rp[1:] - rp[:-1]
        L = self.split
        nseg = torch.clamp((deg + L - 1) // L, min=1)
        total = int(nseg.sum().item()) if n > 0 else 0
        rows = torch.repeat_interleave(torch.arange(n, device=dev, dtype=torch.int64), nseg)
        first = torch.cumsum(nseg, 0) - nseg
        k = torch.arange(total, device=dev, dtype=torch.int64) - first[rows]
        begin = rp[rows] + k * L
        end = torch.minimum(begin + L, rp[rows + 1])
        is_long = nseg[rows] > 1
        slot = torch.where(is_long, torch.cumsum(is_long.to(torch.int64), 0) - 1,
                           torch.full_like(rows, -1))
        self.n_slots = int(is_long.sum().item()) if total > 0 else 0
        items = torch.stack([rows, begin, end, slot], 1)
        order = torch.argsort(end - begin, descending=True, stable=True)
        self.items = items[order].to(torch.int32).contiguous()
        self.n_items = total
        long_rows = torch.nonzero(nseg > 1).flatten()
        self.n_long = int(long_rows.numel())
        if self.n_long:
            long_first = torch.cumsum(nseg[long_rows], 0) - nseg[long_rows]
            lr = torch.stack([long_rows, long_first, long_first + nseg[long_rows],
                              torch.zeros_like(long_rows)], 1)
            self.long_rows = lr.to(torch.int32).contiguous()
        else:
            self.long_rows = None

    def partial(self, d):
        if self.n_slots == 0:
            return None
        buf = self._partial.get(d)
        if buf is None:
            buf = torch.empty(self.n_slots * d, dtype=torch.float32, device=self.device)
            self._partial[d] = buf
        return buf

    def transpose(self):
        if self._T is None:
            rp = self.rowptr.to(torch.int64)
            rows = torch.repeat_interleave(torch.arange(self.n_rows, device=self.device), rp[1:] - rp[:-1])
            self._T = from_coo(self.col.to(torch.int64), rows, self.val, self.n_cols, self.n_rows,
                               split=self.split, coalesce=False)
            self._T._T = self
        return self._T

    def degree_order(self):
        rp = self.rowptr.to(torch.int64)
        deg = rp[1:] - rp[:-1]
        deg = deg + torch.bincount(self.col.to(torch.int64), minlength=self.n_cols)[: self.n_rows]
        return torch.argsort(deg, descending=True, stable=True)

    def relabel(self, order):
        if self.n_rows != self.n_cols:
            raise ValueError("relabel: square matrices only")
        order = order.to(torch.int64)
        new_id = torch.empty_like(order)
        new_id[order] = torch.arange(self.n_rows, device=self.device)

        def one(g):
            rp = g.rowptr.to(torch.int64)
            deg = (rp[1:] - rp[:-1])[order]
            rowptr = torch.zeros(g.n_rows + 1, dtype=torch.int64, device=g.device)
            rowptr[1:] = torch.cumsum(deg, 0)
            idx = torch.repeat_interleave(rp[order] - rowptr[:-1], deg) + torch.arange(g.nnz, device=g.device)
            return CSRGraph(rowptr, new_id[g.col.to(torch.int64)[idx]], None if g.val is None else g.val[idx],
                            g.n_rows, g.n_cols, split=g.split)
        out, out_t = one(self), one(self.transpose())
        out._T, out_t._T = out_t, out
        return out

    def to_dense(self):
        rp = self.rowptr.to(torch.int64)
        rows = torch.repeat_interleave(torch.arange(self.n_rows, device=self.device), rp[1:] - rp[:-1])
        out = torch.zeros(self.n_rows, self.n_cols, dtype=torch.float32, device=self.device)
        v = self.val if self.val is not None else torch.ones(self.nnz, device=self.device)
        out.index_put_((rows, self.col.to(torch.int64)), v, accumulate=True)
        return out

    def algorithmic_bytes(self, d):
        per = 4 + (4 if self.val is not None else 0) + 4 * d
        return self.nnz * per + (self.n_rows + 1) * 4 + self.n_rows * d * 4


def from_coo(rows, cols, vals, n_rows, n_cols, split=DEFAULT_SPLIT, coalesce=True):
    rows = rows.to(torch.int64)
    cols = cols.to(torch.int64)
    key = rows * n_cols + cols
    if coalesce:
        ukey, inv = torch.unique(key, sorted=True, return_inverse=True)
        if ukey.numel() != key.numel():
            if vals is None:
                vals = torch.ones(key.numel(), dtype=torch.float32, device=key.device)
            vals = torch.zeros(ukey.numel(), dtype=torch.float32, device=key.device).index_add_(0, inv, vals.float())
        elif vals is not None:
            vals = torch.empty_like(vals, dtype=torch.float32).index_copy_(0, inv, vals.float())
        key = ukey
    else:
        order = torch.argsort(key, stable=True)
        key = key[order]
        if vals is not None:
            vals = vals[order]
    r = key // n_cols
    c = key % n_cols
    counts = torch.bincount(r, minlength=n_rows)
    rowptr = torch.zeros(n_rows + 1, dtype=torch.int64, device=key.device)
    rowptr[1:] = torch.cumsum(counts, 0)
    return CSRGraph(rowptr, c, vals, n_rows, n_cols, split=split)


_cache = {}


def _evict(key):
    _cache.pop(key, None)


def as_graph(adj, split=DEFAULT_SPLIT):
    if isinstance(adj, CSRGraph) or getattr(adj, "is_partitioned", False):
        return adj
    if not torch.is_tensor(adj):
        raise TypeError("adjacency must be a torch tensor (sparse COO or dense) or CSRGraph")
    key = id(adj)
    hit = _cache.get(key)
    if hit is not None and hit[0]() is adj and hit[2] == adj._version:
        return hit[1]
    if adj.dim() != 2:
        raise ValueError("adjacency must be 2-D, got shape %s" % (tuple(adj.shape),))
    if adj.is_sparse:
        idx = adj._indices()
        vals = adj._values()
        g = from_coo(idx[0], idx[1], vals, adj.shape[0], adj.shape[1], split=split)
    elif adj.layout == torch.sparse_csr:
        g = CSRGraph(adj.crow_indices(), adj.col_indices(), adj.values(), adj.shape[0], adj.shape[1], split=split)
    else:
        nz = torch.nonzero(adj)
        g = from_coo(nz[:, 0], nz[:, 1], adj[nz[:, 0], nz[:, 1]], adj.shape[0], adj.shape[1], split=split)
    try:
        ref = weakref.ref(adj, lambda _r, k=key: _evict(k))
        _cache[key] = (ref, g, adj._version)
    except TypeError:
        pass
    return g


RECORDS_MIN_NNZ = 1 << 16


def csr_from_assignment(index, n_rows, vals=None, split=DEFAULT_SPLIT, records=None):
    idx = index.to(torch.int64)
    e = idx.numel()
    if records is None:
        records = e >= RECORDS_MIN_NNZ
    if idx.is_cuda and not records and n_rows > 0:
        from . import _lib
        lib = _lib.load()
        if lib.gode_assign_csr_supported(e, n_rows):
            idx = idx.contiguous()
            rowptr = torch.empty(n_rows + 1, dtype=torch.int32, device=idx.device)
            order = torch.empty(e, dtype=torch.int32, device=idx.device)
            v_in = None if vals is None else vals.to(torch.float32).contiguous()
            v = None if vals is None else torch.empty(e, dtype=torch.float32, device=idx.device)
            _lib.check(lib.gode_assign_csr_i32(_lib.ptr(idx), e, n_rows, _lib.ptr(rowptr), _lib.ptr(order), _lib.ptr(v_in),
                                               _lib.ptr(v), _lib.stream_ptr()), "gode_assign_csr_i32")
            return CSRGraph(rowptr, order, v, n_rows, e, split=split, records=False)
    order = torch.argsort(idx, stable=True)
    counts = torch.zeros(n_rows, dtype=torch.int64, device=idx.device).index_add_(
        0, idx, torch.ones(e, dtype=torch.int64, device=idx.device))
    rowptr = torch.zeros(n_rows + 1, dtype=torch.int64, device=idx.device)
    rowptr[1:] = torch.cumsum(counts, 0)
    v = None if vals is None else vals.to(torch.float32)[order]
    return CSRGraph(rowptr, order, v, n_rows, e, split=split, records=records)


def incidence_from_index(index, n_rows, split=DEFAULT_SPLIT):
    return csr_from_assignment(index, n_rows, None, split=split)
```

### include/graphode.h

```cpp
#ifndef GRAPHODE_H
#define GRAPHODE_H

#include <stdint.h>

#ifdef __cplusplus
extern "C" {
#endif

#define GODE_ABI_VERSION 1

#define GODE_E_NULLPTR  (-1)
#define GODE_E_SHAPE    (-2)
#define GODE_E_ALIGN    (-3)
#define GODE_E_RANGE    (-4)
#define GODE_E_UNSUPPORTED (-5)

#define GODE_MAX_TERMS 8

typedef struct gode_lincomb {
    int32_t      n;
    float        coef[GODE_MAX_TERMS];
    const float* ptr[GODE_MAX_TERMS];
} gode_lincomb_t;

int         gode_abi_version(void);
int         gode_set_option(const char* name, int value);
int         gode_get_option(const char* name);
const char* gode_error_string(int code);

typedef struct gode_spmm_epilogue {
    const float*   bias;
    int32_t        relu;
    float          alpha;
    gode_lincomb_t pre;
    gode_lincomb_t cot;
    float*         Y2;
    float*         Y2_colsum;
    float*         cot_out;
    float          cot_out_coef[GODE_MAX_TERMS];
} gode_spmm_epilogue_t;

int64_t gode_spmm_y2_colsum_rows(int64_t n_items, int64_t n_long, int64_t d);

int gode_spmm_csr_f32(const int32_t* rowptr, const int32_t* col, const float* val,
                      const int32_t* items, int64_t n_items,
                      const int32_t* long_rows, int64_t n_long, float* partial,
                      const float* X, int64_t ldx, float* Y, int64_t ldy,
                      int64_t n_rows, int64_t d,
                      const gode_spmm_epilogue_t* epi ,
                      void* stream);
int gode_spmm_csr_save_f32(const int32_t* rowptr, const int32_t* col, const float* val,
                           const int32_t* items, int64_t n_items,
                           const int32_t* long_rows, int64_t n_long, float* partial,
                           const float* X, int64_t ldx, float* Y, int64_t ldy,
                           int64_t n_rows, int64_t d,
                           const gode_spmm_epilogue_t* epi , float* K,
                           void* stream);

int64_t gode_masked_cot_parts(int64_t n_rows, int64_t d);
int gode_masked_cot_f32(const gode_lincomb_t* cot , const float* k, float* dZ, int64_t n_rows, int64_t d,
                        float* colpart , void* stream);

int gode_lincomb_f32(float* out, const gode_lincomb_t* lc , int64_t n, void* stream);
int gode_lincomb_multi_f32(float* const* outs , const gode_lincomb_t* lcs ,
                           const int64_t* ns , int32_t count, void* stream);

int64_t gode_rk_errnorm_scratch_bytes(void);
int gode_rk_errnorm_f32(double* out, const float* y0, const float* y1,
                        const gode_lincomb_t* elc , float rtol, float atol,
                        int64_t n, void* scratch, void* stream);
int gode_rk_errnorm_multi_f32(double* out, const float* const* y0 , const float* const* y1,
                              const gode_lincomb_t* elcs , const int64_t* ns, int32_t count, float rtol,
                              float atol, void* scratch, void* stream);

int gode_rk_scaled_sumsq_f32(double* out, const gode_lincomb_t* lc , const float* y,
                             float rtol, float atol, int64_t n, void* scratch, void* stream);

int gode_gn_time_gemm_f32(const gode_lincomb_t* xin , int64_t n_rows, int64_t d_in,
                          int32_t groups, float eps, const float* gamma, const float* beta,
                          const float* W, int64_t d_out, int has_time, float t,
                          float* S, void* stream);
int gode_gn_time_gemm_xout_f32(const gode_lincomb_t* xin , int64_t n_rows, int64_t d_in,
                               int32_t groups, float eps, const float* gamma, const float* beta,
                               const float* W, int64_t d_out, int has_time, float t,
                               float* S, float* x_out, void* stream);
int gode_gn_time_gemm_xout_aux_f32(const gode_lincomb_t* xin , int64_t n_rows, int64_t d_in,
                                   int32_t groups, float eps, const float* gamma, const float* beta,
                                   const float* W, int64_t d_out, int has_time, float t,
                                   float* S, float* x_out , const float* aux_coef ,
                                   float* aux_out, void* stream);

int gode_gn_time_gemm_pair_f32(const gode_lincomb_t* xin , int64_t n_rows, int64_t d, int32_t groups, float eps,
                               const float* gamma, const float* beta, const float* Wa, const float* Wb,
                               int has_time, float t, float* Sa, float* Sb, float* x_out, void* stream);

int64_t gode_gemm_bwd_parts(int64_t n_rows);
int gode_gn_time_gemm_bwd_f32(const gode_lincomb_t* xin , int64_t n_rows, int64_t d_in,
                              int32_t groups, float eps, const float* gamma,
                              const float* W, int64_t d_out, int has_time,
                              const float* dS, float out_scale,
                              const gode_lincomb_t* pre , float* dx,
                              float* dgamma_part, float* dbeta_part, void* stream);

int gode_bwd_wgrad_supported(int64_t n_rows, int64_t d_in, int64_t d_out, int32_t groups);
int64_t gode_bwd_wgrad_parts(int64_t n_rows);
int gode_gn_time_gemm_bwd_wgrad_f32(const gode_lincomb_t* xin , int64_t n_rows, int64_t d_in, int32_t groups,
                                    float eps, const float* gamma, const float* beta, const float* W, int64_t d_out,
                                    int has_time, const float* dS, float out_scale, const gode_lincomb_t* pre ,
                                    float* dx, float* dgamma_part, float* dbeta_part, float* dW_part, void* stream);

#define GODE_MAX_REDUCE_SEGS 8
typedef struct gode_reduce_seg {
    float* out; const float* part;
    int64_t n_part, ld, col0, col_stride, len;
    const float* w_row0; int64_t time_len;
} gode_reduce_seg_t;
int gode_reduce_segments_f32(const gode_reduce_seg_t* segs, int32_t n_segs, float t, float* at , void* stream);
int gode_colsum_parts_f32(const float* X, int64_t n_rows, int64_t d, float* scratch, int64_t* n_parts , void* stream);

int64_t gode_group_norm_parts(int64_t n_rows);
int gode_group_norm_f32_fwd(const float* x, int64_t n_rows, int64_t d, int32_t groups, float eps,
                            const float* gamma , const float* beta , float* y, void* stream);
int gode_group_norm_f32_bwd(const float* x, int64_t n_rows, int64_t d, int32_t groups, float eps,
                            const float* gamma , const float* dy, float* dx,
                            float* dgamma_part , float* dbeta_part , void* stream);

int64_t gode_wgrad_parts(int64_t n_rows);
int gode_wgrad_f32(const gode_lincomb_t* xin , int64_t n_rows, int64_t d_in,
                   int32_t groups, float eps, const float* gamma, const float* beta,
                   const float* dS, int64_t d_out, int has_time,
                   float* dW_part, void* stream);

int gode_rect_gemm_f32(const float* X, int64_t ldx, int64_t n_rows, int64_t K, const float* W, int64_t M,
                       float* S, int64_t lds, void* stream);
int gode_rect_gemm_nt_f32(const float* dS, int64_t ldds, int64_t n_rows, int64_t M, const float* W, int64_t K,
                          float* dX, int64_t lddx, void* stream);
int64_t gode_rect_wgrad_parts(int64_t n_rows);
int gode_rect_wgrad_f32(const float* X, int64_t ldx, int64_t n_rows, int64_t K, const float* dS, int64_t ldds,
                        int64_t M, float* part, void* stream);
int gode_rect_wgrad_sum_f32(const float* X, int64_t ldx, int64_t n_rows, int64_t K, const float* dS, int64_t ldds, int64_t M,
                            float* part, float* dW, void* stream);

int gode_gemm_f32(int trans_a, int trans_b, int64_t M, int64_t N, int64_t K, const float* A, int64_t lda,
                  const float* B, int64_t ldb, float* C, int64_t ldc, const float* bias, int relu,
                  const float* mask, int64_t ldmask, void* stream);
int64_t gode_gemm_splitk_parts(int64_t M, int64_t N, int64_t K);
int gode_gemm_splitk_f32(int trans_a, int trans_b, int64_t M, int64_t N, int64_t K, const float* A, int64_t lda,
                         const float* B, int64_t ldb, float* part, float* C , void* stream);

int64_t gode_cut_pad(int64_t n);
int gode_cut_bf16x3_f32(const float* X, int64_t ld, int64_t R, int64_t C, void* planes, void* stream);
int64_t gode_pgemm_workspace_bytes(int64_t M, int64_t N, int64_t K);
int gode_pgemm_bf16x3(int trans_a, int trans_b, int64_t M, int64_t N, int64_t K, const void* A_planes,
                      const void* B_planes, float* C, int64_t ldc, const float* bias, int relu,
                      const float* mask, int64_t ldmask, int products, void* workspace, void* stream);

#define GODE_ADAM_MAX_TENSORS 64
typedef struct gode_adam_args {
    float*       param[GODE_ADAM_MAX_TENSORS];
    const float* grad[GODE_ADAM_MAX_TENSORS];
    float*       exp_avg[GODE_ADAM_MAX_TENSORS];
    float*       exp_avg_sq[GODE_ADAM_MAX_TENSORS];
    int64_t      len[GODE_ADAM_MAX_TENSORS];
} gode_adam_args_t;
int64_t gode_adam_chunk(void);
int gode_adam_tick_f32(float* state, float beta1, float beta2, void* stream);
int gode_adam_f32(const gode_adam_args_t* args , int32_t n_tensors, const void* chunks, int64_t n_chunks,
                  const float* state, float lr, float beta1, float beta2, float eps, float weight_decay, void* stream);

int gode_reduce_parts_f32(float* out, const float* part, int64_t n_part, int64_t len,
                          float scale, int accumulate, void* stream);
int gode_reduce_parts2_f32(float* out_a, const float* part_a, float* out_b, const float* part_b,
                           int64_t n_part, int64_t len, float scale, int accumulate, void* stream);

int gode_colsum_f32(float* out, const float* X, int64_t n_rows, int64_t d, float scale,
                    int accumulate, float* scratch , void* stream);
int64_t gode_colsum_scratch_bytes(int64_t n_rows, int64_t d);

int64_t gode_gat_logits_scratch_bytes(int64_t n_edges);

typedef struct gode_graph {
    const int32_t* rowptr; const int32_t* col; const float* val;
    const int32_t* items;  int64_t n_items;
    const int32_t* long_rows; int64_t n_long; float* partial;
    int64_t n_rows; int64_t nnz;
} gode_graph_t;

typedef struct gode_gat_proj {
    const float* ps; int64_t ld_s;
    const float* pt; int64_t ld_t;
    const float* as; const float* at;
    int64_t ld_a;
} gode_gat_proj_t;
int gode_gat_logits_f32(const gode_gat_proj_t* proj, const float* bw, const int32_t* src, const int32_t* tgt,
                        int64_t n_edges, float* a, float* amax, float* scratch, void* stream);
int gode_gat_agg_f32_fwd(const gode_graph_t* mt, const int32_t* src, const int32_t* tgt,
                         const gode_gat_proj_t* proj, int64_t o, const float* bf, const float* a, const float* amax,
                         float eps, float* out, float* w_out, float* den_out, void* stream);
int gode_gat_agg_f32_bwd(const gode_graph_t* mt, const int32_t* src, const int32_t* tgt,
                         const gode_gat_proj_t* proj, int64_t o, const float* bf, const float* w, const float* den,
                         const float* out, const float* dout, const gode_lincomb_t* cot, float cot_scale,
                         float* dz, float* da, float* dpt, int64_t ld_dpt, float* dat, int64_t ld_dat,
                         int32_t* did_target_sums, void* stream);
int64_t gode_gat_maxpath_scratch_bytes(int64_t n_edges);
int gode_gat_maxpath_f32(const float* a, const float* amax, float* da, int64_t n_edges, const int32_t* tgt,
                         float* dat, int64_t ld_dat, void* scratch, void* stream);
int64_t gode_gat_heads_scratch_bytes(int64_t n_edges, int64_t heads);
int gode_gat_logits_heads_f32(const gode_gat_proj_t* proj, const float* bw ,
                              const int32_t* src, const int32_t* tgt, int64_t n_edges, int64_t heads, float* a,
                              float* hmax, void* scratch, void* stream);
int gode_gat_maxpath_heads_f32(const float* a, float* da, int64_t n_edges, int64_t heads, const int32_t* tgt,
                               float* dat, int64_t ld_dat, void* scratch, void* stream);
int64_t gode_gat_heads_parts(int64_t n_edges);
int gode_gat_logits_heads_raw_f32(const gode_gat_proj_t* proj, const float* bw, const int32_t* src, const int32_t* tgt,
                                  int64_t n_edges, int64_t heads, float* a, void* scratch, void* stream);
int gode_gat_agg_heads_f32_fwd(const gode_graph_t* mt, const int32_t* src, const int32_t* tgt, const gode_gat_proj_t* proj,
                               int64_t o, const float* bf, const float* a, const void* scratch, int64_t n_edges,
                               int64_t heads, float eps, float* out, float* w_out, float* den_out, void* stream);
int gode_gat_maxpath_heads_raw_f32(const float* a, float* da, int64_t n_edges, int64_t heads, const int32_t* tgt,
                                   float* dat, int64_t ld_dat, void* scratch, void* stream);
int gode_gat_maxpath_heads_part_f32(const float* a, const float* da, int64_t n_edges, int64_t heads, const int32_t* tgt,
                                    void* scratch, void* stream);
int64_t gode_gat_heads_block_cap(void);
int gode_gat_scatter_f32(const int32_t* rowptr_src, const int32_t* eid_src, const int32_t* rowptr_tgt,
                         const int32_t* eid_tgt, const float* dz, const float* da, int64_t o, int64_t n_rows,
                         float* dps, int64_t ld_s, float* dpt, int64_t ld_t, float* das, float* dat, int64_t ld_a,
                         void* stream);
int gode_time_row_fixup_f32(float* g_row0, const float* w_row0, int64_t len, float t, float* at, int accumulate,
                            void* stream);
int gode_time_row_fixup3_f32(float* g0, const float* w0, int64_t l0, float* g1, const float* w1, int64_t l1,
                             float* g2, const float* w2, int64_t l2, float t, float* at, void* stream);

int gode_edge_matvec_f32_fwd(const int32_t* rowptr, const int32_t* eid, const float* val,
                             const int32_t* src, const float* A, const float* X, int64_t ldx,
                             int64_t h, int64_t n_rows, float* out, int64_t ldo, void* stream);
int gode_edge_matvec_msg_f32(const int32_t* src, const float* A, const float* X, int64_t ldx, int64_t h,
                             int64_t n_edges, float* msg, void* stream);
int gode_edge_matvec_f32_bwd(const int32_t* edge_row, const float* edge_val, const int32_t* src,
                             const float* A, const float* X, int64_t ldx, const float* dM, int64_t ldm,
                             int64_t h, int64_t n_edges, float* dA, float* dxe, void* stream);
int gode_edge_outer_sum_f32(const int32_t* edge_row, const float* edge_val , const int32_t* src, int32_t n_terms,
                            const float* const* dM , const float* const* X , int64_t ldx, int64_t ldm,
                            int64_t h, int64_t n_edges, float* dA, void* stream);

int gode_segment_attention_f32_fwd(const int32_t* segptr, const int32_t* perm, const float* x, int64_t ldx,
                                   const float* q, int64_t n_seg, int64_t h, float* a, float* r, void* stream);
int gode_segment_attention_f32_bwd(const int32_t* segptr, const int32_t* perm, const float* x, int64_t ldx,
                                   const float* q, const float* a, const float* dr, int64_t n_seg, int64_t h,
                                   float* dx, float* dq, void* stream);
int gode_assign_csr_supported(int64_t n_entries, int64_t n_rows);
int gode_dense_first_nonzero_f32(const float* M, int64_t ld, int64_t n_rows, int64_t n_cols, int64_t* index, void* stream);
int gode_assign_csr_i32(const int64_t* index, int64_t n_entries, int64_t n_rows, int32_t* rowptr, int32_t* order,
                        const float* vals, float* vals_out, void* stream);

int gode_set2set_supported(int64_t H);
int gode_set2set_f32_fwd(const int32_t* segptr, const int32_t* perm, const float* x, int64_t ldx, const float* Wt,
                         const float* b_ih, const float* b_hh, int64_t n_graphs, int64_t H, int64_t steps, int64_t n_nodes,
                         float* qs, float* cs, float* gates, float* att, void* stream);
int gode_set2set_f32_bwd(const int32_t* segptr, const int32_t* perm, const float* x, int64_t ldx, const float* w_ih,
                         const float* w_hh, int64_t n_graphs, int64_t H, int64_t steps, int64_t n_nodes, const float* qs,
                         const float* cs, const float* gates, const float* att, const float* dq_final, float* dx,
                         float* DG, void* stream);


typedef struct gode_gcn_odefunc {
    gode_graph_t A, AT;
    int64_t n, d;
    int32_t groups; float eps;
    const float* W;
    const float* b; const float* gamma; const float* beta;
} gode_gcn_odefunc_t;

typedef struct gode_rk4_workspace {
    float* S; float* dZ; float* dS;
    float* S2;
    float* ky[4]; float* ka[4];
    float* ktheta[4];
    float* wpart;
    float* gpart; float* bpart;
    float* colsum_scratch;
    float* X[2];
    float* small_part;
    float* y2_colsum;
} gode_rk4_workspace_t;

int     gode_gcn_small_supported(int64_t n_rows, int64_t d, int32_t groups);
int64_t gode_gcn_small_parts(int64_t n_rows);
int64_t gode_gcn_small_part_len(int64_t d);
int gode_gcn_feval_small_f32(const gode_gcn_odefunc_t* f, const gode_lincomb_t* xin , float t, float alpha,
                             const gode_lincomb_t* pre , const gode_lincomb_t* cot ,
                             float* Y2 , float* out, void* stream);
int gode_gcn_feval_small_next_f32(const gode_gcn_odefunc_t* f, const gode_lincomb_t* xin , float t, float alpha,
                                  const gode_lincomb_t* pre , const gode_lincomb_t* cot ,
                                  float* Y2 , float* out, const gode_lincomb_t* next , float* x_next,
                                  void* stream);
int gode_gcn_vjp_small_f32(const gode_gcn_odefunc_t* f, const gode_lincomb_t* xin , const float* dZ,
                           float out_scale, const gode_lincomb_t* pre , float* ka, float* part,
                           void* stream);
int gode_gcn_vjp_small_next_f32(const gode_gcn_odefunc_t* f, const gode_lincomb_t* xin , const float* dZ,
                                float out_scale, const gode_lincomb_t* pre , float* ka, float* part,
                                const gode_lincomb_t* cot_next , const float* k_next, float* dZ_next,
                                void* stream);
int gode_gcn_feval_small_save_f32(const gode_gcn_odefunc_t* f, const gode_lincomb_t* xin , float t, float alpha,
                                  const gode_lincomb_t* pre , float* out, float* k, void* stream);
int gode_gcn_small_finish_f32(const gode_gcn_odefunc_t* f, const float* part, float* ktheta, float t, void* stream);
int gode_gcn_small_finish_multi_f32(const gode_gcn_odefunc_t* f, const float* part, int32_t n_stages,
                                    float* const* ktheta , const float* ts , void* stream);
int gode_gcn_small_finish4_f32(const gode_gcn_odefunc_t* f, const float* part, float* theta, const float* wb ,
                               const float* ts , void* stream);

int64_t gode_gcn_ode_theta_len(int64_t d);
int gode_gcn_ode_rk4_forward(const gode_gcn_odefunc_t* f, float* y, float** result,
                             const gode_rk4_workspace_t* ws, float t0, float t1, int32_t n_steps, void* stream);
int gode_gcn_ode_rk4_adjoint(const gode_gcn_odefunc_t* f, float* y, float* a, float* theta,
                             float** y_result, float** a_result,
                             const gode_rk4_workspace_t* ws, float t0, float t1, int32_t n_steps, void* stream);

int gode_gcn_ode_rk4_forward_save(const gode_gcn_odefunc_t* f, const float* y0, float* y_end, float* save,
                                  const gode_rk4_workspace_t* ws, float t0, float t1, int32_t n_steps,
                                  int32_t step_begin, int32_t step_end, void* stream);
int gode_gcn_ode_rk4_backprop(const gode_gcn_odefunc_t* f, const float* save, float* a, float* theta, float** a_result,
                              const gode_rk4_workspace_t* ws, float* cot_colpart , float t0, float t1,
                              int32_t n_steps, int32_t step_begin, int32_t step_end, void* stream);

int gode_gcn_ode_dopri5_step_forward(const gode_gcn_odefunc_t* f, const float* y, float* const* k , float* y1,
                                     const gode_rk4_workspace_t* ws, double t, double h, float rtol, float atol,
                                     double* sums, void* err_scratch, void* stream);
int gode_gcn_ode_dopri5_step_adjoint(const gode_gcn_odefunc_t* f, const float* y, const float* a, const float* theta,
                                     float* const* ky , float* const* ka , float* const* ktheta ,
                                     float* y1, float* a1, float* theta1, const gode_rk4_workspace_t* ws,
                                     double t, double h, float rtol, float atol, double* sums ,
                                     void* err_scratch, void* stream);

int gode_gcn_ode_dopri5_step_backprop(const gode_gcn_odefunc_t* f, const float* y, float* const* k ,
                                      const float* g, const float* kbar7 , double wy,
                                      const double* wk , double t, double h, int32_t first,
                                      float* const* ybar , float* ybar_n, float* kbar1, float* theta,
                                      float* const* ktheta , const gode_rk4_workspace_t* ws,
                                      float* cot_colpart , void* stream);

typedef struct gode_gat_odefunc {
    gode_graph_t mt;
    gode_graph_t ms_inc, mt_inc;
    const int32_t* src; const int32_t* tgt; int64_t n_edges;
    int64_t n, d; int32_t groups; float eps_gn; float eps;
    const float* Wsrc; const float* Wtgt; const float* Wlog;
    const float* bf; const float* bw; const float* gamma; const float* beta;
    int32_t heads;
    const float* Wpacked;
} gode_gat_odefunc_t;

typedef struct gode_gat_workspace {
    float* X; float* Ps; float* Pt; float* A2;
    float* a; float* amax; float* wgt; float* den;
    void* logits_scratch;
    float* dz; float* da;
    float* dPs; float* dPt; float* dA2; float* pair;
    float* gp; float* bp;
    float* wp[3];
    void* maxpath_scratch; void* colsum_scratch;
    const float* zeros; void* heads_scratch;
    void* colsum_scratch2;
    float* small_part;
} gode_gat_workspace_t;

int     gode_gat_small_supported(int64_t n_rows, int64_t d, int32_t groups, int64_t heads);
int64_t gode_gat_small_parts(int64_t n_rows, int64_t d);
int64_t gode_gat_small_part_len(int64_t d, int64_t heads);
int gode_gat_project_small_f32(const gode_lincomb_t* xin, int64_t n_rows, int64_t d, int32_t groups, float eps,
                               const float* gamma, const float* beta, const float* Wsrc, const float* Wtgt,
                               const float* Wlog, int64_t heads, const float* pt_bias, float t, float* Ps, float* Pt,
                               float* A2, float* x_out, const float* packed , void* stream);
int gode_gat_dense_vjp_small_f32(const gode_lincomb_t* xin, int64_t n_rows, int64_t d, int32_t groups, float eps,
                                 const float* gamma, const float* beta, const float* Wsrc, const float* Wtgt,
                                 const float* Wlog, int64_t heads, const float* dPs, const float* dPt, const float* dA2,
                                 float out_scale, const gode_lincomb_t* pre, float* ka, float* part,
                                 const void* maxpath_scratch , const int32_t* esrc, const int32_t* etgt, int64_t n_edges,
                                 const float* packed , void* stream);
int gode_gat_small_finish_f32(const float* part, int64_t n_rows, int64_t d, int64_t heads, float t, float* ktheta,
                              float* kat, void* stream);
int gode_gat_small_finish_step_f32(const float* part, int64_t n_rows, int64_t d, int64_t heads, int32_t n_slots,
                                   const float* ts , const float* w , float* theta, float* at,
                                   void* stream);
int64_t gode_gat_small_pack_len(int64_t d, int64_t heads);
int gode_gat_small_pack_f32(const float* Wsrc, const float* Wtgt, const float* Wlog, int64_t d, int64_t heads, float* packed,
                            void* stream);

int64_t gode_gat_ode_theta_len(int64_t d);
int64_t gode_gat_ode_theta_len_heads(int64_t d, int64_t heads);
int gode_gat_ode_dopri5_step_forward(const gode_gat_odefunc_t* f, const float* y, float* const* k , float* y1,
                                     const gode_gat_workspace_t* ws, double t, double h, float rtol, float atol,
                                     double* sums, void* err_scratch, void* stream);
int gode_gat_ode_dopri5_step_adjoint(const gode_gat_odefunc_t* f, const float* y, const float* a, const float* a_t,
                                     const float* theta, float* const* ky, float* const* ka, float* const* ka_t,
                                     float* const* ktheta, float* y1, float* a1, float* a_t1, float* theta1,
                                     const gode_gat_workspace_t* ws, double t, double h, float rtol, float atol,
                                     double* sums , void* err_scratch, void* stream);

int gode_lstm_cell_supported(int64_t B, int64_t I, int64_t H);
int gode_lstm_cell_f32_fwd(const float* x, const float* h, const float* c, const float* w_ih, const float* w_hh,
                           const float* b_ih, const float* b_hh, int64_t B, int64_t I, int64_t H, float* h_out,
                           float* c_out, float* gates, void* stream);
int gode_lstm_cell_f32_bwd(const float* x, const float* h, const float* c, const float* w_ih, const float* w_hh,
                           const float* gates, const float* c_out, const float* dh_out, const float* dc_out, int64_t B,
                           int64_t I, int64_t H, float* dx, float* dh, float* dc, float* dw_ih, float* dw_hh,
                           float* db_ih, float* db_hh, void* stream);
int64_t gode_gru_wgrad_parts(int64_t n);
int gode_gru_cell_f32_fwd(const float* x, const float* m, const float* w_ih, const float* w_hh, const float* b_ih,
                          const float* b_hh, int64_t n, int64_t h, float* out, float* gates, void* stream);
int gode_gru_cell_f32_bwd(const float* x, const float* m, const float* w_ih, const float* w_hh, const float* gates,
                          const float* dout, int64_t n, int64_t h, float* dx, float* dm, float* dgi, float* dgh,
                          float* part, float* dw_ih, float* dw_hh, float* db_ih, float* db_hh, void* stream);
int gode_gru_wreduce_f32(const float* part, int64_t n_part, int64_t h, float* dw_ih, float* dw_hh, float* db_ih,
                         float* db_hh, void* stream);

int gode_edge_ode_supported(int64_t h);
int gode_edge_ode_feval_f32(const int32_t* rowptr, const int32_t* eid, const float* val, const int32_t* src,
                            const float* A, const float* S, int64_t h, int64_t n_rows, const float* bias,
                            const gode_lincomb_t* pre , float alpha, float* out, void* stream);
int gode_edge_ode_vjp_f32(const int32_t* ms_rowptr, const int32_t* ms_eid, const int32_t* edge_row,
                          const float* edge_val, const float* A, const gode_lincomb_t* cot , float cot_scale,
                          const float* fout, int64_t h, int64_t n_rows, int64_t n_edges, float* dM, float* dS,
                          float* dxe, void* stream);
// ... 49 lines not shown
```

Baseline: 4.240 steps/s.

## Handle self-loop-only rows in GEMM epilogue and skip them in SpMM

Finds rows whose only nonzero is the diagonal (isolated nodes after adding self loops) and builds reduced SpMM item lists without them. In the forward pass the GEMM kernel writes relu(diag*S+b) straight into the output for these rows, and skips storing S for rows that A^T never reads. In the backward pass the A^T SpMM runs over the core list only, and the A SpMM epilogue writes the scaled diagonal rows. This removes SpMM traffic for many isolated RMAT rows, but adds extra per-row loads in the GEMM, new epilogue paths and a one-time host-side preprocessing step.

```diff
diff --git a/graph_odenet_amd/csrc/api.hip b/graph_odenet_amd/csrc/api.hip
--- a/graph_odenet_amd/csrc/api.hip
+++ b/graph_odenet_amd/csrc/api.hip
@@ -22,7 +22,7 @@
 
 namespace {
 int env_int(const char* name, int dflt) { const char* e = getenv(name); return e ? atoi(e) : dflt; }
-int g_gemm_split = -1, g_overlap = -1, g_wgrad_split = -1, g_wgrad_split_small = 0, g_bwd_pc = -1, g_fwd_pc = -1, g_small_fused = -1, g_bwd_wgrad = -1, g_y2_colsum = -1, g_rk_close_once = -1, g_spmm_pipe = -1;
+int g_gemm_split = -1, g_overlap = -1, g_wgrad_split = -1, g_wgrad_split_small = 0, g_bwd_pc = -1, g_fwd_pc = -1, g_small_fused = -1, g_bwd_wgrad = -1, g_y2_colsum = -1, g_rk_close_once = -1, g_spmm_pipe = -1, g_diag_rows = -1;
 }
 
 int gode_opt_gemm_split() { if (g_gemm_split < 0) { const int v = env_int("GODE_GEMM_SPLIT", 2); g_gemm_split = (v == 1 || v == 2) ? v : 0; } return g_gemm_split; }
@@ -38,6 +38,7 @@
 int gode_opt_y2_colsum() { if (g_y2_colsum < 0) g_y2_colsum = env_int("GODE_Y2_COLSUM", 1) != 0; return g_y2_colsum; }
 int gode_opt_rk_close_once() { if (g_rk_close_once < 0) g_rk_close_once = env_int("GODE_RK_CLOSE_ONCE", 1) != 0; return g_rk_close_once; }
 int gode_opt_spmm_pipe() { if (g_spmm_pipe < 0) { const int v = env_int("GODE_SPMM_PIPE", 1); g_spmm_pipe = (v < 0 || v > 64) ? 1 : v; } return g_spmm_pipe; }
+int gode_opt_diag_rows() { if (g_diag_rows < 0) g_diag_rows = env_int("GODE_DIAG_ROWS", 1) != 0; return g_diag_rows; }
 int gode_opt_overlap() { if (g_overlap < 0) g_overlap = env_int("GODE_OVERLAP", 1) != 0; return g_overlap; }
 
 extern "C" int gode_set_option(const char* name, int value) {
@@ -51,6 +52,7 @@
     if (!strcmp(name, "y2_colsum")) { g_y2_colsum = value != 0; return 0; }
     if (!strcmp(name, "rk_close_once")) { g_rk_close_once = value != 0; return 0; }
     if (!strcmp(name, "spmm_pipe")) { if (value < 0 || value > 64) return GODE_E_UNSUPPORTED; g_spmm_pipe = value; return 0; }
+    if (!strcmp(name, "diag_rows")) { g_diag_rows = value != 0; return 0; }
     if (!strcmp(name, "fwd_pc")) { if (value < 0 || value > 3) return GODE_E_UNSUPPORTED; g_fwd_pc = value; return 0; }
     if (!strcmp(name, "wgrad_split")) { if (value != 0 && value != 6 && value != 8) return GODE_E_UNSUPPORTED; g_wgrad_split = value; return 0; }
     return GODE_E_UNSUPPORTED;
@@ -67,6 +69,7 @@
     if (!strcmp(name, "y2_colsum")) return gode_opt_y2_colsum();
     if (!strcmp(name, "rk_close_once")) return gode_opt_rk_close_once();
     if (!strcmp(name, "spmm_pipe")) return gode_opt_spmm_pipe();
+    if (!strcmp(name, "diag_rows")) return gode_opt_diag_rows();
     if (!strcmp(name, "fwd_pc")) return gode_opt_fwd_pc();
     return GODE_E_UNSUPPORTED;
 }
diff --git a/graph_odenet_amd/csrc/dense_pc.h b/graph_odenet_amd/csrc/dense_pc.h
--- a/graph_odenet_amd/csrc/dense_pc.h
+++ b/graph_odenet_amd/csrc/dense_pc.h
@@ -4,6 +4,9 @@
 int gode_pc_fwd_launch(const LinComb& lc, int64_t n_rows, float eps, const float* gamma, const float* beta,
                        const float* W, int has_time, float t, float* S, float* xout, const float* aux_coef, float* aux,
                        int cg, hipStream_t s);
+struct FwdDiag { const float* diag; const float* skip; const float* bias; float* K; };
+int gode_pc_fwd_diag_launch(const LinComb& lc, int64_t n_rows, float eps, const float* gamma, const float* beta,
+                            const float* W, int has_time, float t, float* S, const FwdDiag& dg, int cg, hipStream_t s);
 int gode_pc_bwd_launch(const LinComb& lc, int64_t n_rows, float eps, const float* gamma, const float* W, int has_time,
                        const float* dS, float out_scale, const LinComb& pre, float* dx, float* dgamma_part,
                        float* dbeta_part, int64_t n_part, int cg, hipStream_t s);
diff --git a/graph_odenet_amd/csrc/gemm.hip b/graph_odenet_amd/csrc/gemm.hip
--- a/graph_odenet_amd/csrc/gemm.hip
+++ b/graph_odenet_amd/csrc/gemm.hip
@@ -1303,6 +1303,33 @@
                                           nullptr, nullptr, stream);
 }
 
+extern "C" int gode_gn_time_gemm_diag_f32(const gode_lincomb_t* xin, int64_t n_rows, int64_t d_in, int32_t groups,
+                                          float eps, const float* gamma, const float* beta, const float* W,
+                                          int64_t d_out, int has_time, float t, float* S, const float* diag,
+                                          const float* skip, const float* bias, float* K, int32_t* taken, void* stream)
+{
+    if (!taken) return GODE_E_NULLPTR;
+    *taken = 0;
+    int rc = check_common(xin, n_rows, d_in, groups, d_out); if (rc) return rc;
+    if (n_rows == 0) return 0;
+    if (!W || !S) return GODE_E_NULLPTR;
+    const int cg = fast_cg(d_in, d_out, groups);
+    const bool al = lincomb_aligned16(xin) && !(((uintptr_t)S) & 15) && !(((uintptr_t)W) & 15) &&
+                    (!gamma || !(((uintptr_t)gamma) & 15)) && (!beta || !(((uintptr_t)beta) & 15)) &&
+                    !(((uintptr_t)bias) & 15) && !(((uintptr_t)K) & 15);
+    bool distinct = diag && skip && bias && K && K != S;
+    for (int j = 0; distinct && j < xin->n; ++j) distinct = K != xin->ptr[j];
+    if (distinct && cg >= 0 && al && d_in == 128 && xin->n <= 3 && (n_rows >= kWgradSplitMinRows || gode_opt_wgrad_split_small()) &&
+        (xin->n <= 2 ? (gode_opt_fwd_pc() & 1) : (gode_opt_fwd_pc() & 2))) {
+        const FwdDiag dg = {diag, skip, bias, K};
+        rc = gode_pc_fwd_diag_launch(make_lincomb(xin), n_rows, eps, gamma, beta, W, has_time ? 1 : 0, t, S, dg, cg,
+                                     (hipStream_t)stream);
+        if (rc == 0) *taken = 1;
+        if (rc != GODE_E_UNSUPPORTED) return rc;
+    }
+    return gode_gn_time_gemm_f32(xin, n_rows, d_in, groups, eps, gamma, beta, W, d_out, has_time, t, S, stream);
+}
+
 extern "C" int gode_gn_time_gemm_xout_aux_f32(const gode_lincomb_t* xin, int64_t n_rows, int64_t d_in, int32_t groups,
                                               float eps, const float* gamma, const float* beta, const float* W,
                                               int64_t d_out, int has_time, float t, float* S, float* x_out,
diff --git a/graph_odenet_amd/csrc/gemm_pc.hip b/graph_odenet_amd/csrc/gemm_pc.hip
--- a/graph_odenet_amd/csrc/gemm_pc.hip
+++ b/graph_odenet_amd/csrc/gemm_pc.hip
@@ -80,13 +80,13 @@
     __device__ int clamped(int k) const { return blockIdx.x + (k < mine ? k : (mine > 0 ? mine - 1 : 0)) * stride; }
 };
 
-template <int CG, int NX, bool XOUT, int R, bool AUX = false>
+template <int CG, int NX, bool XOUT, int R, bool AUX = false, bool DIAG = false>
 __global__ __launch_bounds__(1024, 1) void gn_gemm_fwd_pc_kernel(LinComb xin, int n_rows, float eps,
                                                                 const float* __restrict__ gamma,
                                                                 const float* __restrict__ beta,
                                                                 const float* __restrict__ W, int has_time, float t,
                                                                 float* __restrict__ S, float* __restrict__ xout,
-                                                                AuxCoef acoef, float* __restrict__ aux)
+                                                                AuxCoef acoef, float* __restrict__ aux, FwdDiag dg)
 {
     static_assert(!AUX || NX > 0, "the second combination needs the raw terms");
     constexpr int PIECE_B = Img<R>::PIECE_B, BUF_B = Img<R>::BUF_B;
@@ -163,18 +163,41 @@
     f32x4 t0 = {0.f, 0.f, 0.f, 0.f};
     if (has_time) { const float4 w0 = ld4(W + n0 + 4 * g); t0 = (f32x4){t * w0.x, t * w0.y, t * w0.z, t * w0.w}; }
     const int rd_off = r * LDK * 2 + g * 16;
+    float4 bv = make_float4(0.f, 0.f, 0.f, 0.f);
+    if (DIAG) bv = ld4(dg.bias + n0 + 4 * g);
     lds_barrier();
     for (int k = 0; k < tw.mine; ++k) {
         f32x4 acc[R / 16];
 #pragma unroll
         for (int rt = 0; rt < R / 16; ++rt) acc[rt] = t0;
+        const int row0 = tw.tile(k) * R + r;
+        float dsc[R / 16], skp[R / 16];
+        if (DIAG) {
+#pragma unroll
+            for (int rt = 0; rt < R / 16; ++rt) {
+                const int rc = min(row0 + 16 * rt, n_rows - 1);
+                dsc[rt] = dg.diag[rc];
+                skp[rt] = dg.skip[rc];
+            }
+        }
         tile_product<R>(lds + (k & 1) * BUF_B + rd_off, A, acc);
-        const int row0 = tw.tile(k) * R + r;
 #pragma unroll
         for (int rt = 0; rt < R / 16; ++rt) {
             const int row = row0 + 16 * rt;
-            if (row < n_rows)
-                *reinterpret_cast<float4*>(S + (int64_t)row * D + n0 + 4 * g) = make_float4(acc[rt][0], acc[rt][1], acc[rt][2], acc[rt][3]);
+            if (row < n_rows) {
+                if (!DIAG || skp[rt] == 0.f)
+                    *reinterpret_cast<float4*>(S + (int64_t)row * D + n0 + 4 * g) = make_float4(acc[rt][0], acc[rt][1], acc[rt][2], acc[rt][3]);
+                if (DIAG && dsc[rt] != 0.f) {
+                    float m[4];
+#pragma unroll
+                    for (int c = 0; c < 4; ++c) {
+                        m[c] = fmaf(dsc[rt], acc[rt][c], 0.f);
+                        asm volatile("" : "+v"(m[c]));
+                    }
+                    *reinterpret_cast<float4*>(dg.K + (int64_t)row * D + n0 + 4 * g) =
+                        make_float4(fmaxf(m[0] + bv.x, 0.f), fmaxf(m[1] + bv.y, 0.f), fmaxf(m[2] + bv.z, 0.f), fmaxf(m[3] + bv.w, 0.f));
+                }
+            }
         }
         lds_barrier();
     }
@@ -581,7 +604,7 @@
       rc = set_lds_pc(gn_gemm_fwd_pc_kernel<CGV, NXV, XO, RV, AX>, lds); if (rc) return rc;                        \
       const int slot = gode_prof_begin(s, D, n_rows, (int64_t)lc.n - 1 + (XO ? 1 : 0) + (AX ? 1 : 0), GODE_PROF_GEMM_FWD | GODE_PROF_FORM_PC); \
       hipLaunchKernelGGL((gn_gemm_fwd_pc_kernel<CGV, NXV, XO, RV, AX>), dim3((unsigned)blocks), dim3(1024), lds, s, \
-                         lc, (int)n_rows, eps, gamma, beta, W, has_time, t, S, xout, ac, aux);                    \
+                         lc, (int)n_rows, eps, gamma, beta, W, has_time, t, S, xout, ac, aux, FwdDiag{});         \
       gode_prof_end(s, slot);                                                                                      \
       GODE_LAUNCH_CHECK(); return 0; }
 #define GODE_FPC2(CGV, NXV, RV) { if (xout) GODE_FPC5(CGV, NXV, true, RV, false) else GODE_FPC5(CGV, NXV, false, RV, false) }
@@ -598,6 +621,29 @@
 #undef GODE_FPC
 #undef GODE_FPC2
 #undef GODE_FPC5
+    return GODE_E_UNSUPPORTED;
+}
+
+int gode_pc_fwd_diag_launch(const LinComb& lc, int64_t n_rows, float eps, const float* gamma, const float* beta,
+                            const float* W, int has_time, float t, float* S, const FwdDiag& dg, int cg, hipStream_t s)
+{
+    int rc = 0;
+    AuxCoef ac;
+    for (int j = 0; j < GODE_MAX_TERMS; ++j) ac.c[j] = 0.f;
+#define GODE_FPCD(CGV, NXV)                                                                                        \
+    { const size_t lds = 2 * (size_t)Img<32>::BUF_B;                                                               \
+      const int64_t blocks = pc_blocks(n_rows, 32);                                                                \
+      rc = set_lds_pc(gn_gemm_fwd_pc_kernel<CGV, NXV, false, 32, false, true>, lds); if (rc) return rc;            \
+      const int slot = gode_prof_begin(s, D, n_rows, (int64_t)lc.n - 1, GODE_PROF_GEMM_FWD | GODE_PROF_FORM_PC);   \
+      hipLaunchKernelGGL((gn_gemm_fwd_pc_kernel<CGV, NXV, false, 32, false, true>), dim3((unsigned)blocks), dim3(1024), lds, s, \
+                         lc, (int)n_rows, eps, gamma, beta, W, has_time, t, S, (float*)nullptr, ac, (float*)nullptr, dg); \
+      gode_prof_end(s, slot);                                                                                      \
+      GODE_LAUNCH_CHECK(); return 0; }
+#define GODE_FPCDN(CGV) { if (lc.n == 1) GODE_FPCD(CGV, 1) else if (lc.n == 2) GODE_FPCD(CGV, 2) else if (lc.n == 3) GODE_FPCD(CGV, 3) }
+    if (!dg.diag || !dg.skip || !dg.bias || !dg.K) return GODE_E_UNSUPPORTED;
+    if (cg == 0) GODE_FPCDN(0) else if (cg == 4) GODE_FPCDN(4)
+#undef GODE_FPCDN
+#undef GODE_FPCD
     return GODE_E_UNSUPPORTED;
 }
 
diff --git a/graph_odenet_amd/csrc/ode_driver.hip b/graph_odenet_amd/csrc/ode_driver.hip
--- a/graph_odenet_amd/csrc/ode_driver.hip
+++ b/graph_odenet_amd/csrc/ode_driver.hip
@@ -87,9 +87,20 @@
 struct StepClose { gode_lincomb_t pre; float alpha; bool once; };
 
 int feval_large(const gode_gcn_odefunc_t* f, const gode_lincomb_t& xin, float t, float* S, float* out,
-                const StepClose* close, float* k_save, void* stream) {
+                const StepClose* close, float* k_save, void* stream, bool diag_ok = false) {
     const int64_t d = f->d;
     bool p_formed = false;
+    if (diag_ok && !close && !k_save) {
+        int32_t taken = 0;
+        GODE_TRY(gode_gn_time_gemm_diag_f32(&xin, f->n, d, f->groups, f->eps, f->gamma, f->beta, f->W, d, 1, t, S, f->a_diag,
+                                            f->at_diag, f->b, out, &taken, stream));
+        gode_spmm_epilogue_t ep = relu_bias_epilogue(f);
+        if (!taken) return spmm(f->A, S, out, d, &ep, stream);
+        ep.n_items_full = f->A.n_items;
+        const gode_graph_t& g = f->A;
+        return gode_spmm_csr_f32(g.rowptr, g.col, g.val, f->a_core_items, f->a_n_core, g.long_rows, g.n_long, g.partial,
+                                 S, d, out, d, g.n_rows, d, &ep, stream);
+    }
     if (close && close->once) {
         GODE_TRY(gf_last_stage(f, xin, close->pre, t, S, nullptr, out, &p_formed, stream));
     } else {
@@ -104,13 +115,14 @@
 }
 
 int rk4_forward_step(const gode_gcn_odefunc_t* f, const gode_rk4_workspace_t* ws, const float* y, float* const* k,
-                     float* ynext, bool keep_k4, double t, double h, bool fused, bool close_once, void* stream) {
+                     float* ynext, bool keep_k4, double t, double h, bool fused, bool close_once, void* stream,
+                     bool diag_ok = false) {
     for (int s = 0; s < 4; ++s) {
         const gode_lincomb_t xin = stage_terms(y, k, s, h);
         const float ts = (float)(t + C38[s] * h);
         if (s < 3) {
             if (fused) GODE_TRY(gode_gcn_feval_small_f32(f, &xin, ts, 1.f, nullptr, nullptr, nullptr, k[s], stream));
-            else GODE_TRY(feval_large(f, xin, ts, ws->S, k[s], nullptr, nullptr, stream));
+            else GODE_TRY(feval_large(f, xin, ts, ws->S, k[s], nullptr, nullptr, stream, diag_ok));
             continue;
         }
         const StepClose close = {combine_terms(y, k, h), (float)(h * B38[3]), close_once};
@@ -137,8 +149,10 @@
     float* k[4] = {ws->ky[0], ws->ky[1], ws->ky[2], ws->ky[3]};
     const bool fused = fused_small(f);
     const bool close_once = close_once_route(f);
+    const bool diag_ok = gode_opt_diag_rows() && !fused && f->n > kMergedFinishMaxRows && f->d == 128 && f->a_core_items &&
+                         f->a_diag && f->at_diag && f->A.items && f->a_n_core > 0 && f->a_n_core <= f->A.n_items;
     for (int i = 0; i < n_steps; ++i) {
-        GODE_TRY(rk4_forward_step(f, ws, cur, k, k[3], false, (double)t0 + i * h, h, fused, close_once, stream));
+        GODE_TRY(rk4_forward_step(f, ws, cur, k, k[3], false, (double)t0 + i * h, h, fused, close_once, stream, diag_ok));
         float* tmp = cur; cur = k[3]; k[3] = tmp;
     }
     *result = cur;
@@ -238,6 +252,8 @@
 
     const bool close_once = bw && close_once_route(f);
     bool py_formed = false;
+    const bool at_core = bw && y2rows > 0 && gode_opt_diag_rows() && f->at_core_items && f->at_diag && f->AT.items &&
+                         f->at_n_core > 0 && f->at_n_core <= f->AT.n_items;
     auto gf = [&](int g, void* st) -> int {
         const gode_lincomb_t yin = stage_terms(ycur, ky, g % 4, h);
         if (g % 4 == 3 && close_once)
@@ -268,10 +284,21 @@
             }
             py_formed = false;
         }
+        if (at_core) {
+            ep.Y2_scale = f->at_diag;
+            ep.Y2_scaled = ws->dS;
+        }
         if (two && g > 0) GODE_HIP(hipStreamWaitEvent(hs, ov->gf, 0));
         GODE_TRY(spmm(f->A, Sbuf[g & 1], ky[s], d, &ep, stream));
         if (s == 3) { float* tmp = ycur; ycur = ky[3]; ky[3] = tmp; }
         if (two && wg_pending) GODE_HIP(hipStreamWaitEvent(hs, ov->wg, 0));
+        if (at_core) {
+            gode_spmm_epilogue_t pt = {};
+            pt.alpha = 1.f;
+            pt.n_items_full = f->AT.n_items;
+            GODE_TRY(gode_spmm_csr_f32(f->AT.rowptr, f->AT.col, f->AT.val, f->at_core_items, f->at_n_core, f->AT.long_rows,
+                                       f->AT.n_long, f->AT.partial, ws->dZ, d, ws->dS, d, f->AT.n_rows, d, &pt, stream));
+        } else
         GODE_TRY(spmm(f->AT, ws->dZ, ws->dS, d, nullptr, stream));
         if (two) {
             GODE_HIP(hipEventRecord(ov->spt, hs));
diff --git a/graph_odenet_amd/csrc/options.h b/graph_odenet_amd/csrc/options.h
--- a/graph_odenet_amd/csrc/options.h
+++ b/graph_odenet_amd/csrc/options.h
@@ -10,3 +10,4 @@
 int gode_opt_y2_colsum();
 int gode_opt_rk_close_once();
 int gode_opt_spmm_pipe();
+int gode_opt_diag_rows();
diff --git a/graph_odenet_amd/csrc/spmm.hip b/graph_odenet_amd/csrc/spmm.hip
--- a/graph_odenet_amd/csrc/spmm.hip
+++ b/graph_odenet_amd/csrc/spmm.hip
@@ -20,9 +20,11 @@
     float* K;
     float* Y3;
     float c3[GODE_MAX_TERMS];
+    const float* y2_scale;
+    float* y2_dst;
 };
 
-template <int LPR, bool OUT3 = false, bool COT = true>
+template <int LPR, bool OUT3 = false, bool COT = true, bool SCALE = false>
 __device__ __forceinline__ float4 epilogue_store4(const Epilogue& ep, float4 z, int row, int lane,
                                                   int64_t d, float* Y, int64_t ldy) {
     if (ep.bias) {
@@ -42,6 +44,7 @@
     *reinterpret_cast<float4*>(Y + (int64_t)row * ldy + lane * 4) = y;
     if (COT && ep.Y2) {
         const int64_t o = (int64_t)row * d + lane * 4;
+        const float sc = (SCALE && ep.y2_scale) ? ep.y2_scale[row] : 0.f;
         float4 g;
         if (OUT3) {
             float4 g3;
@@ -52,7 +55,9 @@
         }
         g.x = z.x > 0.f ? g.x : 0.f; g.y = z.y > 0.f ? g.y : 0.f;
         g.z = z.z > 0.f ? g.z : 0.f; g.w = z.w > 0.f ? g.w : 0.f;
-        *reinterpret_cast<float4*>(ep.Y2 + o) = g;
+        const bool scaled = SCALE && sc != 0.f;
+        const float4 st = scaled ? make_float4(fmaf(sc, g.x, 0.f), fmaf(sc, g.y, 0.f), fmaf(sc, g.z, 0.f), fmaf(sc, g.w, 0.f)) : g;
+        *reinterpret_cast<float4*>((scaled ? ep.y2_dst : ep.Y2) + o) = st;
         return g;
     }
     return make_float4(0.f, 0.f, 0.f, 0.f);
@@ -125,14 +130,14 @@
     if (ep.colpart) {
         float4 g = make_float4(0.f, 0.f, 0.f, 0.f);
         if (active) {
-            if (slot < 0) g = epilogue_store4<LPR, OUT3>(ep, acc, row, lane, (int64_t)LPR * 4, Y, ldy);
+            if (slot < 0) g = epilogue_store4<LPR, OUT3, true, true>(ep, acc, row, lane, (int64_t)LPR * 4, Y, ldy);
             else *reinterpret_cast<float4*>(partial + (int64_t)slot * (LPR * 4) + lane * 4) = acc;
         }
         block_colsum_store<LPR>(g, ep.colpart + (int64_t)blockIdx.x * (LPR * 4));
         return;
     }
     if (!active) return;
-    if (slot < 0) epilogue_store4<LPR, OUT3>(ep, acc, row, lane, (int64_t)LPR * 4, Y, ldy);
+    if (slot < 0) epilogue_store4<LPR, OUT3, true, true>(ep, acc, row, lane, (int64_t)LPR * 4, Y, ldy);
     else *reinterpret_cast<float4*>(partial + (int64_t)slot * (LPR * 4) + lane * 4) = acc;
 }
 
@@ -421,11 +426,11 @@
 template <int LPR, bool OUT3>
 int launch_vec4(const int* rowptr, const int* col, const float* val, const int4* items, int n_items,
                 const int4* long_rows, int n_long, float* partial, const float* X, int64_t ldx,
-                float* Y, int64_t ldy, const Epilogue& ep, hipStream_t s) {
-    if (LPR < 64 && n_items > 0 && n_items <= 65536) {
-        if (ep.colpart) return GODE_E_UNSUPPORTED;
+                float* Y, int64_t ldy, const Epilogue& ep, int64_t full_items, hipStream_t s) {
+    if (LPR < 64 && n_items > 0 && full_items <= 65536) {
+        if (ep.colpart || ep.y2_scale) return GODE_E_UNSUPPORTED;
         const int64_t wb = ((int64_t)n_items * 64 + 255) / 256;
-        const int slot = gode_prof_begin(s, (int64_t)LPR * 4, n_items, (int64_t)ep.pre.n + ep.cot.n + (ep.Y2 ? 1 : 0) + (ep.Y3 ? 1 : 0));
+        const int slot = gode_prof_begin(s, (int64_t)LPR * 4, full_items, (int64_t)ep.pre.n + ep.cot.n + (ep.Y2 ? 1 : 0) + (ep.Y3 ? 1 : 0));
         hipLaunchKernelGGL((spmm_vec4_wave_kernel<LPR, OUT3>), dim3((unsigned)wb), dim3(256), 0, s,
                            rowptr, col, val, items, n_items, partial, X, ldx, Y, ldy, ep);
         gode_prof_end(s, slot);
@@ -441,7 +446,7 @@
     const int64_t threads = (int64_t)n_items * LPR;
     const int64_t blocks = (threads + 255) / 256;
     if (blocks > 0) {
-        const int slot = gode_prof_begin(s, (int64_t)LPR * 4, n_items, (int64_t)ep.pre.n + ep.cot.n + (ep.Y2 ? 1 : 0) + (ep.Y3 ? 1 : 0));
+        const int slot = gode_prof_begin(s, (int64_t)LPR * 4, full_items, (int64_t)ep.pre.n + ep.cot.n + (ep.Y2 ? 1 : 0) + (ep.Y3 ? 1 : 0));
         const int pipe = gode_opt_spmm_pipe();
         if (pipe != 0 && !ep.Y2) {
             int64_t per = pipe == 1 ? std::max<int64_t>(1, std::min<int64_t>(SPMM_PIPE_TILES, blocks / SPMM_PIPE_MIN_BLOCKS)) : pipe;
@@ -517,24 +522,34 @@
         if (ep.Y3 == Y || ep.Y3 == Y2 || ep.Y3 == K) return GODE_E_RANGE;
         for (int j = 0; j < ep.cot.n; ++j) if (ep.Y3 == ep.cot.ptr[j]) return GODE_E_RANGE;
     }
+    ep.y2_scale = (epi && Y2) ? epi->Y2_scale : nullptr;
+    ep.y2_dst = ep.y2_scale ? epi->Y2_scaled : nullptr;
+    if (epi && !Y2 && (epi->Y2_scale || epi->Y2_scaled)) return GODE_E_NULLPTR;
+    if (ep.y2_scale) {
+        if (!ep.y2_dst) return GODE_E_NULLPTR;
+        if (ep.y2_dst == Y || ep.y2_dst == Y2 || ep.y2_dst == K || ep.y2_dst == ep.Y3 || ep.y2_dst == X) return GODE_E_RANGE;
+        for (int j = 0; j < ep.cot.n; ++j) if (ep.y2_dst == ep.cot.ptr[j]) return GODE_E_RANGE;
+        for (int j = 0; j < ep.pre.n; ++j) if (ep.y2_dst == ep.pre.ptr[j]) return GODE_E_RANGE;
+    }
+    const int64_t full_items = (epi && epi->n_items_full > n_items) ? epi->n_items_full : n_items;
     if (ep.colpart && ((((uintptr_t)ep.colpart) & 15) || gode_spmm_y2_colsum_rows(n_items, n_long, d) == 0)) return GODE_E_UNSUPPORTED;
 
     const bool al = !(((uintptr_t)X) & 15) && !(((uintptr_t)Y) & 15) && (ldx % 4 == 0) && (ldy % 4 == 0) &&
                     (!bias || !(((uintptr_t)bias) & 15)) && (!partial || !(((uintptr_t)partial) & 15)) &&
                     (!Y2 || (!(((uintptr_t)Y2) & 15) && lincomb_aligned16(cot))) && lincomb_aligned16(pre) &&
-                    !(((uintptr_t)K) & 15) && !(((uintptr_t)ep.Y3) & 15);
+                    !(((uintptr_t)K) & 15) && !(((uintptr_t)ep.Y3) & 15) && !(((uintptr_t)ep.y2_dst) & 15);
     const int4* it4 = reinterpret_cast<const int4*>(items);
     const int4* lr4 = reinterpret_cast<const int4*>(long_rows);
     if (al && d % 4 == 0) {
         switch (d / 4) {
-#define GODE_CASE(L) case L: return ep.Y3 ? launch_vec4<L, true>(rowptr, col, val, it4, (int)n_items, lr4, (int)n_long, partial, X, ldx, Y, ldy, ep, s) \
-                                        : launch_vec4<L, false>(rowptr, col, val, it4, (int)n_items, lr4, (int)n_long, partial, X, ldx, Y, ldy, ep, s);
+#define GODE_CASE(L) case L: return ep.Y3 ? launch_vec4<L, true>(rowptr, col, val, it4, (int)n_items, lr4, (int)n_long, partial, X, ldx, Y, ldy, ep, full_items, s) \
+                                        : launch_vec4<L, false>(rowptr, col, val, it4, (int)n_items, lr4, (int)n_long, partial, X, ldx, Y, ldy, ep, full_items, s);
             GODE_CASE(1) GODE_CASE(2) GODE_CASE(4) GODE_CASE(8) GODE_CASE(16) GODE_CASE(32) GODE_CASE(64)
 #undef GODE_CASE
             default: break;
         }
     }
-    if (ep.colpart) return GODE_E_UNSUPPORTED;
+    if (ep.colpart || ep.y2_scale) return GODE_E_UNSUPPORTED;
     int G = 1; while (G < d && G < 64) G <<= 1;
     if (d == 1 && it4 != nullptr) {
         const int64_t blocks = ((int64_t)n_items * 64 + 255) / 256;
diff --git a/graph_odenet_amd/gcn_ode.py b/graph_odenet_amd/gcn_ode.py
--- a/graph_odenet_amd/gcn_ode.py
+++ b/graph_odenet_amd/gcn_ode.py
@@ -118,6 +118,11 @@
     fs.n, fs.d, fs.groups, fs.eps = spec.graph.n_rows, spec.d, spec.groups, spec.eps
     fs.W, fs.b = spec.W.data_ptr(), spec.b.data_ptr()
     fs.gamma, fs.beta = spec.gamma.data_ptr(), spec.beta.data_ptr()
+    core = getattr(spec.graph, "_at_core", None)
+    if core is not None:
+        fs.at_core_items, fs.at_n_core, fs.at_diag = core.items.data_ptr(), core.n_items, core.diag.data_ptr()
+        a = spec.graph.__dict__["_a_core"]
+        fs.a_core_items, fs.a_n_core, fs.a_diag = a.items.data_ptr(), a.n_items, a.diag.data_ptr()
     return fs
 
 
@@ -146,6 +151,25 @@
     h_t = torch.zeros(m, dtype=torch.int64, device=col.device).index_add_(0, rows % m, deg)
     h = torch.stack([h_a, h_t]).tolist()
     return max(max(hh) * m / max(sum(hh), 1) for hh in h)
+
+
+CORE_LIST_MIN_ROWS = 65536
+CORE_LIST_MIN_SHARE_INV = 8
+
+
+def _hand_core_list(g, info):
+    if getattr(g, "items", None) is None or g.n_rows <= CORE_LIST_MIN_ROWS or g.transpose().items is None:
+        return
+    if "_at_core" not in g.__dict__:
+        iso = g.transpose().isolated_rows()
+        take = CORE_LIST_MIN_SHARE_INV * iso.n_flagged >= g.n_rows and iso.n_items > 0
+        if take:
+            iso.items
+            g.diag_rows().items
+        g.__dict__["_at_core"] = iso if take else None
+        g.__dict__["_a_core"] = g.diag_rows() if take else None
+        g.__dict__["_isolated_count"] = iso.n_flagged
+    info.update(isolated_rows=g.__dict__["_isolated_count"], core_lists=g.__dict__["_at_core"] is not None)
 
 
 def tuned_graph(graph, d, node_order="auto"):
@@ -172,6 +196,8 @@
         if take:
             res = (graph.relabel(order), order, inverse)
             info["renumbered"] = True
+    if square and not (res[0].device.type == "cuda" and torch.cuda.is_current_stream_capturing()):
+        _hand_core_list(res[0], info)
     graph.__dict__.setdefault("_tuned_info", {})[(d, node_order)] = info
     cache[(d, node_order)] = res
     return res
diff --git a/graph_odenet_amd/graph.py b/graph_odenet_amd/graph.py
--- a/graph_odenet_amd/graph.py
+++ b/graph_odenet_amd/graph.py
@@ -26,6 +26,8 @@
             self.items, self.n_items, self.long_rows, self.n_long, self.n_slots = None, self.n_rows, None, 0, 0
         self._partial = {}
         self._T = None
+        self._diag_rows = None
+        self._isolated_rows = None
 
     def _build_items(self):
         dev = self.device
@@ -67,6 +69,20 @@
             self._partial[d] = buf
         return buf
 
+    def diag_rows(self):
+        if self._diag_rows is None:
+            if self.items is None:
+                raise ValueError("diag_rows: the graph has no record list")
+            self._diag_rows = DiagRows(self)
+        return self._diag_rows
+
+    def isolated_rows(self):
+        if self._isolated_rows is None:
+            if self.n_rows != self.n_cols or self.items is None:
+                raise ValueError("isolated_rows: square matrices with a record list only")
+            self._isolated_rows = DiagRows(self, among=self.transpose().diag_rows().diag)
+        return self._isolated_rows
+
     def transpose(self):
         if self._T is None:
             rp = self.rowptr.to(torch.int64)
@@ -112,6 +128,35 @@
     def algorithmic_bytes(self, d):
         per = 4 + (4 if self.val is not None else 0) + 4 * d
         return self.nnz * per + (self.n_rows + 1) * 4 + self.n_rows * d * 4
+
+
+class DiagRows:
+
+    def __init__(self, g, among=None):
+        n = g.n_rows
+        rp = g.rowptr.to(torch.int64)
+        self.diag = torch.zeros(n, dtype=torch.float32, device=g.device)
+        if n > 0 and g.nnz > 0:
+            first = torch.clamp(rp[:-1], max=g.nnz - 1)
+            rows = torch.arange(n, device=g.device, dtype=torch.int64)
+            v = g.val[first] if g.val is not None else torch.ones(n, dtype=torch.float32, device=g.device)
+            flag = ((rp[1:] - rp[:-1]) == 1) & (g.col.to(torch.int64)[first] == rows) & (v != 0)
+            if among is not None:
+                flag = flag & (among != 0)
+            self.diag = torch.where(flag, v, self.diag)
+        self.n_flagged = int((self.diag != 0).sum())
+        self.n_items = g.n_items - self.n_flagged
+        self._g, self._items = g, None
+
+    @property
+    def items(self):
+        if self._items is None:
+            g = self._g
+            keep = self.diag[g.items[:, 0].to(torch.int64)] == 0
+            self._items = g.items[keep].contiguous()
+            assert self._items.shape[0] == self.n_items
+            self._g = None
+        return self._items
 
 
 def from_coo(rows, cols, vals, n_rows, n_cols, split=DEFAULT_SPLIT, coalesce=True):
diff --git a/include/graphode.h b/include/graphode.h
--- a/include/graphode.h
+++ b/include/graphode.h
@@ -38,6 +38,9 @@
     float*         Y2_colsum;
     float*         cot_out;
     float          cot_out_coef[GODE_MAX_TERMS];
+    const float*   Y2_scale;
+    float*         Y2_scaled;
+    int64_t        n_items_full;
 } gode_spmm_epilogue_t;
 
 int64_t gode_spmm_y2_colsum_rows(int64_t n_items, int64_t n_long, int64_t d);
@@ -84,6 +87,11 @@
                                int32_t groups, float eps, const float* gamma, const float* beta,
                                const float* W, int64_t d_out, int has_time, float t,
                                float* S, float* x_out, void* stream);
+int gode_gn_time_gemm_diag_f32(const gode_lincomb_t* xin , int64_t n_rows, int64_t d_in,
+                               int32_t groups, float eps, const float* gamma, const float* beta,
+                               const float* W, int64_t d_out, int has_time, float t,
+                               float* S, const float* diag, const float* skip, const float* bias, float* K,
+                               int32_t* taken , void* stream);
 int gode_gn_time_gemm_xout_aux_f32(const gode_lincomb_t* xin , int64_t n_rows, int64_t d_in,
                                    int32_t groups, float eps, const float* gamma, const float* beta,
                                    const float* W, int64_t d_out, int has_time, float t,
@@ -269,6 +277,8 @@
     int32_t groups; float eps;
     const float* W;
     const float* b; const float* gamma; const float* beta;
+    const int32_t* at_core_items; int64_t at_n_core; const float* at_diag;
+    const int32_t* a_core_items; int64_t a_n_core; const float* a_diag;
 } gode_gcn_odefunc_t;
 
 typedef struct gode_rk4_workspace {
```

Result: faster. 4.426 steps/s (median of 6 runs) (+4.4%).
